# yifita/iso-points

Hardware: AMD Instinct MI355X
Metric: Mpoints/s full iso-point cycle (project+resample+splat), 1M pts (higher is better)
Workload: dtype f32-class (split-fp16 operands, 2^-22: hidden-layer products from two fp16 parts per f32 operand under exact power-of-two scales, 3 fp16-MFMA passes, f32 accumulate; everything else f32)

## Files before the change

### iso_points_amd/csrc/siren.hip

```cpp
#include <stdlib.h>
#include "siren_common.h"
#include "iso_newton.h"
#include "mlp_common.h"

namespace {

__global__ void k_siren_pack(const float* __restrict__ raw, float* __restrict__ packed,
                             int H, int L) {
  const int64_t total = off_hidden(H, L);
  const int64_t HH = (int64_t)H * H;
  const int NT = H / 16;
  for (int64_t o = (int64_t)blockIdx.x * blockDim.x + threadIdx.x; o < total;
       o += (int64_t)gridDim.x * blockDim.x) {
    float v = 0.f;
    if (o < off_wl(H)) {
      int64_t k = o;
      int c = (int)(k & 3);
      int e = (int)((k >> 2) % (H / 4));
      int g = (int)((k >> 2) / (H / 4));
      int f = 16 * (e >> 2) + 4 * g + (e & 3);
      v = (c < 3) ? raw[f * 3 + c] : raw[(int64_t)H * 3 + f];
    } else if (o < off_bl(H)) {
      int64_t k = o - off_wl(H);
      int e = (int)(k % (H / 4));
      int g = (int)(k / (H / 4));
      int f = 16 * (e >> 2) + 4 * g + (e & 3);
      const int64_t raw_wl = (int64_t)H * 4 + (int64_t)L * (HH + H);
      v = raw[raw_wl + f];
    } else if (o < off_hidden(H, 0)) {
      const int64_t raw_wl = (int64_t)H * 4 + (int64_t)L * (HH + H);
      v = (o == off_bl(H)) ? raw[raw_wl + H] : 0.f;
    } else {
      int64_t k = o - off_hidden(H, 0);
      const int64_t per = H + 2 * HH;
      int l = (int)(k / per);
      int64_t w = k % per;
      const float* Wl = raw + (int64_t)H * 4 + (int64_t)l * (HH + H);
      const float* bl = Wl + HH;
      if (w < H) {
        v = bl[w];
      } else {
        w -= H;
        bool bwd = w >= HH;
        if (bwd) w -= HH;
        int i = (int)(w & 3);
        int lane = (int)((w >> 2) & 63);
        int t = (int)((w >> 8) % NT);
        int q = (int)((w >> 8) / NT);
        int a = 16 * t + (lane & 15);
        int b = 16 * q + 4 * (lane >> 4) + i;
        v = bwd ? Wl[(int64_t)b * H + a]
                : Wl[(int64_t)a * H + b];
      }
    }
    packed[o] = v;
  }
}

#define ISO_GEMM_FWD(img, bias) gemm_pass<NT, true>(img, bias, hL, wbuf, acc, lane, g)
#define ISO_GEMM_BWD(img) gemm_pass<NT, false>(img, nullptr, hL, wbuf, acc, lane, g)

template <int NT, bool CODED>
__global__ __launch_bounds__(256, 2) void k_siren_step(typename SirenArgsOf<CODED>::type a) {
  constexpr int H = NT * 16;
  extern __shared__ __attribute__((aligned(16))) float smem[];
  const int tid = threadIdx.x;
  const int wave = tid >> 6, lane = tid & 63;
  const int g = lane >> 4, j = lane & 15;
  float* hL = smem + wave * (NT * 256);
  float* wbuf = smem + 4 * NT * 256;
  const float* W0img = a.packed + off_w0(H);
  const float* WLimg = a.packed + off_wl(H);
  const float bL = a.packed[off_bl(H)];
  float* stash = a.stash + ((int64_t)blockIdx.x * 4 + wave) * (int64_t)(a.L + 1) * NT * 256;

  const int64_t count = a.count_in ? (int64_t)(*a.count_in) : a.n;
  const int64_t n_tiles = (count + 63) / 64;
  for (int64_t tile = blockIdx.x; tile < n_tiles; tile += gridDim.x) {
    const int64_t slot = tile * 64 + wave * 16 + j;
    const bool valid = slot < count;
    int64_t idx = -1;
    float px = 0.f, py = 0.f, pz = 0.f;
    int row = 0;
    if (valid) {
      idx = a.idx_in ? (int64_t)a.idx_in[slot] : slot;
      px = a.pts[idx * 3]; py = a.pts[idx * 3 + 1]; pz = a.pts[idx * 3 + 2];
      if constexpr (CODED) row = a.code_of ? a.code_of[idx] : 0;
    }
    const f32x4* cb = nullptr;
    if constexpr (CODED) cb = reinterpret_cast<const f32x4*>(a.code_bias + (int64_t)row * H) + g;
    (void)cb;
    float f = 0.f;
    const bool top0 = (a.L == 0);
    for (int e4 = 0; e4 < NT; ++e4) {
      f32x4 h4, s4;
      f32x4 b4 = {0.f, 0.f, 0.f, 0.f};
      if constexpr (CODED) b4 = cb[4 * e4];
#pragma unroll
      for (int i = 0; i < 4; ++i) {
        const f32x4 w = reinterpret_cast<const f32x4*>(W0img)[g * (H / 4) + e4 * 4 + i];
        float z;
        if constexpr (CODED) z = ((w.x * px + w.y * py) + w.z * pz) + b4[i];
        else z = ((w.x * px + w.y * py) + w.z * pz) + w.w;
        float s, c;
        iso_sincos(a.w0 * z, s, c);
        h4[i] = s;
        s4[i] = a.w0 * c;
      }
      if (top0) {
        const f32x4 w4 = reinterpret_cast<const f32x4*>(WLimg)[g * NT + e4];
        f += (w4.x * h4.x + w4.y * h4.y) + (w4.z * h4.z + w4.w * h4.w);
        h4 = (f32x4){w4.x * s4.x, w4.y * s4.y, w4.z * s4.z, w4.w * s4.w};
      }
      reinterpret_cast<f32x4*>(hL)[e4 * 64 + lane] = h4;
      if (!top0) reinterpret_cast<f32x4*>(stash)[e4 * 64 + lane] = s4;
    }
    f32x4 acc[NT];
    for (int l = 0; l < a.L; ++l) {
      const float* base = a.packed + off_hidden(H, l);
      ISO_GEMM_FWD(base + H, base);
      float* st_l = stash + (int64_t)(l + 1) * NT * 256;
      const bool top = (l == a.L - 1);
#pragma unroll
      for (int t = 0; t < NT; ++t) reinterpret_cast<f32x4*>(hL)[t * 64 + lane] = acc[t];
      for (int e4 = 0; e4 < NT; ++e4) {
        const f32x4 z4 = reinterpret_cast<const f32x4*>(hL)[e4 * 64 + lane];
        f32x4 h4, s4;
#pragma unroll
        for (int i = 0; i < 4; ++i) {
          float s, c;
          iso_sincos(a.wh * z4[i], s, c);
          h4[i] = s;
          s4[i] = a.wh * c;
        }
        if (top) {
          const f32x4 w4 = reinterpret_cast<const f32x4*>(WLimg)[g * NT + e4];
          f += (w4.x * h4.x + w4.y * h4.y) + (w4.z * h4.z + w4.w * h4.w);
          h4 = (f32x4){w4.x * s4.x, w4.y * s4.y, w4.z * s4.z, w4.w * s4.w};
          reinterpret_cast<f32x4*>(hL)[e4 * 64 + lane] = h4;
        } else {
          reinterpret_cast<f32x4*>(hL)[e4 * 64 + lane] = h4;
          reinterpret_cast<f32x4*>(st_l)[e4 * 64 + lane] = s4;
        }
      }
    }
    f += __shfl_xor(f, 16);
    f += __shfl_xor(f, 32);
    f += bL;
    for (int l = a.L - 1; l >= 0; --l) {
      const float* base = a.packed + off_hidden(H, l);
      ISO_GEMM_BWD(base + H + (int64_t)H * H);
      const float* st_l = stash + (int64_t)l * NT * 256;
#pragma unroll
      for (int t = 0; t < NT; ++t) {
        const f32x4 s4 = reinterpret_cast<const f32x4*>(st_l)[t * 64 + lane];
        f32x4 gs = {acc[t].x * s4.x, acc[t].y * s4.y, acc[t].z * s4.z, acc[t].w * s4.w};
        reinterpret_cast<f32x4*>(hL)[t * 64 + lane] = gs;
      }
    }
    float gx = 0.f, gy = 0.f, gz = 0.f;
    for (int e4 = 0; e4 < NT; ++e4) {
      const f32x4 a4 = reinterpret_cast<const f32x4*>(hL)[e4 * 64 + lane];
#pragma unroll
      for (int i = 0; i < 4; ++i) {
        const f32x4 w = reinterpret_cast<const f32x4*>(W0img)[g * (H / 4) + e4 * 4 + i];
        gx += w.x * a4[i];
        gy += w.y * a4[i];
        gz += w.z * a4[i];
      }
    }
    gx += __shfl_xor(gx, 16); gx += __shfl_xor(gx, 32);
    gy += __shfl_xor(gy, 16); gy += __shfl_xor(gy, 32);
    gz += __shfl_xor(gz, 16); gz += __shfl_xor(gz, 32);

    bool survive = false;
    if (valid && g == 0) survive = iso_step_finish(a, idx, f, gx, gy, gz);
    if (!a.eval_only && a.do_move) {
      const unsigned long long bal = __ballot(survive);
      if (bal) {
        int base = 0;
        const int leader = __ffsll((long long)bal) - 1;
        if (lane == leader) base = atomicAdd(a.count_out, __popcll(bal));
        base = __shfl(base, leader);
        if (survive) {
          const int rank = __popcll(bal & ((1ull << lane) - 1ull));
          a.idx_out[base + rank] = (int32_t)idx;
        }
      }
    }
    __syncthreads();
  }
}

constexpr int kSirenBlocks = 512;

inline int64_t stash_floats(int H, int L) { return (int64_t)kSirenBlocks * 4 * (L + 1) * H * 16; }

template <int NT, bool CODED>
int launch_step(const typename SirenArgsOf<CODED>::type& a, int blocks, hipStream_t s) {
  const size_t lds = (size_t)(5 * NT * 256) * sizeof(float);
  static bool attr_done = false;
  if (!attr_done) {
    (void)hipFuncSetAttribute(reinterpret_cast<const void*>(&k_siren_step<NT, CODED>),
                        hipFuncAttributeMaxDynamicSharedMemorySize, (int)lds);
    attr_done = true;
  }
  hipLaunchKernelGGL((k_siren_step<NT, CODED>), dim3(blocks), dim3(256), lds, s, a);
  return 0;
}

template <bool CODED>
int dispatch_step(const typename SirenArgsOf<CODED>::type& a, int H, int blocks, hipStream_t s) {
  switch (H / 16) {
    case 4: return launch_step<4, CODED>(a, blocks, s);
    case 8: return launch_step<8, CODED>(a, blocks, s);
    case 16: return launch_step<16, CODED>(a, blocks, s);
    default: return -1;
  }
}

__global__ void k_zero_counts(int32_t* c, int n) {
  int i = blockIdx.x * blockDim.x + threadIdx.x;
  if (i < n) c[i] = 0;
}

bool siren_shape_ok(int H, int L) {
  return (H == 64 || H == 128 || H == 256) && L >= 0 && L <= 8;
}

int g_gemm_mode = -1;
int gemm_mode() {
  if (g_gemm_mode < 0) {
    const char* e = getenv("ISO_SIREN_GEMM");
    g_gemm_mode = (e && (!strcmp(e, "f32") || !strcmp(e, "0"))) ? 0 : 1;
  }
  return g_gemm_mode;
}
bool use_x3(int H, int L) { return gemm_mode() == 1 && siren_x3_supported(H, L); }

int64_t stash_floats_any(int H, int L) {
  int64_t a = stash_floats(H, L);
  int64_t b = siren_x3_supported(H, L) ? siren_x3_stash_floats(H, L) : 0;
  return a > b ? a : b;
}

int run_step(const SirenCodedArgs& a, int H, int64_t n, hipStream_t s) {
  if (use_x3(H, a.L)) return siren_x3_launch(a, H, n, s);
  int64_t tiles = (n + 63) / 64;
  int blocks = (int)(tiles < kSirenBlocks ? tiles : kSirenBlocks);
  return a.code_bias ? dispatch_step<true>(a, H, blocks, s) : dispatch_step<false>(a, H, blocks, s);
}

}

extern "C" int64_t iso_siren_raw_floats(int hidden, int n_hidden) {
  int64_t H = hidden;
  return H * 3 + H + (int64_t)n_hidden * (H * H + H) + H + 1;
}

extern "C" int64_t iso_siren_packed_floats(int hidden, int n_hidden) {
  return siren_packed_total(hidden, n_hidden);
}

extern "C" int iso_siren_set_gemm_mode(int mode) {
  ISO_REQUIRE(mode == 0 || mode == 1, ISO_ERR_INVALID, "iso_siren_set_gemm_mode: mode must be 0 (f32 MFMA) or 1 (split fp16)");
  g_gemm_mode = mode;
  return ISO_OK;
}

extern "C" int iso_siren_get_gemm_mode(void) { return gemm_mode(); }

extern "C" int iso_siren_pack_weights(const float* raw, float* packed, int hidden,
                                      int n_hidden, void* stream) {
  ISO_REQUIRE(siren_shape_ok(hidden, n_hidden), ISO_ERR_UNSUPPORTED,
              "iso_siren_pack_weights: hidden must be 64/128/256 and 0<=n_hidden<=8 (got %d, %d)",
              hidden, n_hidden);
  ISO_REQUIRE(raw && packed, ISO_ERR_INVALID, "iso_siren_pack_weights: null pointer");
  int64_t total = off_hidden(hidden, n_hidden);
  hipLaunchKernelGGL(k_siren_pack, dim3(iso_stream_grid(total, 256)), dim3(256), 0,
                     (hipStream_t)stream, raw, packed, hidden, n_hidden);
  if (hidden % 32 == 0) siren_x3_pack(raw, packed, hidden, n_hidden, (hipStream_t)stream);
  ISO_CHECK_LAUNCH("iso_siren_pack_weights");
  return ISO_OK;
}

static int64_t tail_cap_of(int64_t n) {
  const int64_t blocks = siren_x3_tail_blocks(), tiles = (n + 31) / 32;
  return ((tiles + blocks - 1) / blocks + 1) * 32;
}
static int64_t tail_ints(int64_t n) { return siren_x3_tail_blocks() * (2 * tail_cap_of(n) + 2); }

constexpr int kTileCtrInts = 128;
extern "C" int64_t iso_project_siren_workspace_bytes(int64_t n, int hidden, int n_hidden) {
  if (n < 0) n = 0;
  return stash_floats_any(hidden, n_hidden) * 4 + 2 * n * 4 + tail_ints(n) * 4 + (64 + kTileCtrInts) * 4 + 64;
}

extern "C" int64_t iso_project_siren_counts_offset(int64_t n, int hidden, int n_hidden) {
  if (n < 0) n = 0;
  return stash_floats_any(hidden, n_hidden) * 4 + 2 * n * 4 + tail_ints(n) * 4;
}

static int g_siren_dyn_tiles = -1;
static bool siren_dynamic_tiles_enabled() {
  return g_siren_dyn_tiles != 0;
}
extern "C" int iso_siren_set_drawn_tiles(int on) {
  ISO_REQUIRE(on >= -1 && on <= 1, ISO_ERR_INVALID, "iso_siren_set_drawn_tiles: -1 (default), 0 or 1");
  g_siren_dyn_tiles = on;
  return ISO_OK;
}

static int run_step_split(SirenCodedArgs a, int hidden, int64_t n, hipStream_t s) {
  if (hidden == 256 && !a.fwd_only && use_x3(hidden, a.L)) {
    a.split = 3;
    return run_step(a, hidden, n, s);
  }
  a.split = 0;
  a.tile_ctr = nullptr;
  return run_step(a, hidden, n, s);
}

static int g_tail_from = -1;
static int siren_tail_from(int max_iters) {
  if (g_tail_from == 0) return max_iters + 1;
  if (g_tail_from > 0) return g_tail_from;
  return max_iters >= 6 ? 4 : 2;
}
extern "C" int iso_siren_step_launches(int hidden, int n_hidden, int max_iters) {
  if (max_iters < 0) return 0;
  const bool can_tail = hidden == 256 && use_x3(hidden, n_hidden);
  const int from = can_tail ? siren_tail_from(max_iters) : max_iters + 1;
  return from <= max_iters && from > 0 ? from + 1 : max_iters + 1;
}
extern "C" int iso_siren_set_tail_from(int first_tail_iteration) {
  ISO_REQUIRE(first_tail_iteration >= -1, ISO_ERR_INVALID, "iso_siren_set_tail_from: -1 (default), 0 (never) or an iteration >= 1");
  g_tail_from = first_tail_iteration;
  return ISO_OK;
}

__global__ void k_zero_tail(int32_t* c, int n, int32_t* tc, int m) {
  const int i = blockIdx.x * blockDim.x + threadIdx.x;
  if (i < n) c[i] = 0;
  if (i < m) tc[i] = 0;
}

static int run_iterations(SirenCodedArgs a, int hidden, int64_t n, int max_iters, void* workspace,
                          hipStream_t s, const char* who) {
  float* stash = (float*)workspace;
  int32_t* idxA = (int32_t*)(stash + stash_floats_any(hidden, a.L));
  int32_t* idxB = idxA + n;
  int32_t* tail = idxB + n;
  int32_t* counts = tail + tail_ints(n);
  const int blocks = siren_x3_tail_blocks();
  const int64_t cap = tail_cap_of(n);
  int32_t* tail_counts = tail + (int64_t)blocks * 2 * cap;
  const bool can_tail = hidden == 256 && !a.dirs && !a.fwd_only && use_x3(hidden, a.L);
  const int tail_from = can_tail ? siren_tail_from(max_iters) : max_iters + 1;
  int32_t* tile_ctr = counts + 64;
  hipLaunchKernelGGL(k_zero_tail, dim3((2 * blocks + 255) / 256), dim3(256), 0, s, counts, 64 + kTileCtrInts, tail_counts,
                     tail_from <= max_iters ? 2 * blocks : 0);
  const bool dyn_tiles = siren_dynamic_tiles_enabled() && 2 * (max_iters + 1) <= kTileCtrInts;
  a.stash = stash; a.n = n; a.eval_only = 0; a.sdf_out = a.dirs ? a.sdf_out : nullptr; a.grad_out = nullptr;
  for (int it = 0; it <= max_iters; ++it) {
    a.idx_in = (it == 0) ? nullptr : ((it & 1) ? idxA : idxB);
    a.count_in = (it == 0) ? nullptr : counts + it;
    a.idx_out = (it & 1) ? idxB : idxA;
    a.count_out = counts + it + 1;
    a.do_move = (it < max_iters) ? 1 : 0;
    a.tile_ctr = dyn_tiles ? tile_ctr + 2 * it : nullptr;
    if (it >= tail_from && it > 0) {
      a.tail_lists = tail; a.tail_counts = tail_counts; a.iter_counts = counts; a.tail_cap = (int)cap;
      a.it_first = it; a.it_last = max_iters;
      ISO_REQUIRE(siren_x3_launch_tail(a, hidden, s) == 0, ISO_ERR_UNSUPPORTED, "%s: no tail kernel for hidden size %d", who, hidden);
      break;
    }
    ISO_REQUIRE(run_step_split(a, hidden, n, s) == 0, ISO_ERR_UNSUPPORTED, "%s: unsupported hidden size %d", who, hidden);
  }
  return ISO_OK;
}

__global__ void k_siren_fold_codes(const float* __restrict__ w0c, const float* __restrict__ b0,
                                   const float* __restrict__ codes, float* __restrict__ table, int H, int Hp, int C,
                                   int64_t U) {
  const int64_t total = U * Hp;
  for (int64_t o = (int64_t)blockIdx.x * blockDim.x + threadIdx.x; o < total; o += (int64_t)gridDim.x * blockDim.x) {
    const int64_t u = o / Hp;
    const int f = (int)(o - u * Hp);
    float v = 0.f;
    if (f < H) {
      double acc = (double)b0[f];
      const float* wr = w0c + (int64_t)f * C;
      const float* cu = codes + u * C;
      for (int k = 0; k < C; ++k) acc = fma((double)wr[k], (double)cu[k], acc);
      v = (float)acc;
    }
    table[o] = v;
  }
}

extern "C" int iso_siren_fold_codes(const float* w0c, const float* b0, const float* codes, float* table, int hidden,
                                    int padded_hidden, int c_dim, int64_t n_codes, void* stream) {
  ISO_REQUIRE(hidden >= 1 && padded_hidden >= hidden && c_dim >= 1 && n_codes >= 0, ISO_ERR_INVALID,
              "iso_siren_fold_codes: bad sizes (hidden %d, padded %d, c_dim %d, codes %lld)", hidden, padded_hidden,
              c_dim, (long long)n_codes);
  if (n_codes == 0) return ISO_OK;
  ISO_REQUIRE(w0c && b0 && codes && table, ISO_ERR_INVALID, "iso_siren_fold_codes: null pointer");
  const int64_t total = n_codes * padded_hidden;
  hipLaunchKernelGGL(k_siren_fold_codes, dim3(iso_stream_grid(total, 256)), dim3(256), 0, (hipStream_t)stream, w0c, b0,
                     codes, table, hidden, padded_hidden, c_dim, n_codes);
  ISO_CHECK_LAUNCH("iso_siren_fold_codes");
  return ISO_OK;
}

static int project_siren(const float* pts_in, float* pts_out, float* normals_out, uint8_t* mask_out, int64_t n,
                         const float* packed, int hidden, int n_hidden, float omega_first, float omega_hidden,
                         int max_iters, float tol, void* workspace, int64_t workspace_bytes, void* stream,
                         const float* code_bias, const int32_t* code_of) {
  ISO_REQUIRE(siren_shape_ok(hidden, n_hidden), ISO_ERR_UNSUPPORTED,
              "iso_project_siren: hidden must be 64/128/256 and 0<=n_hidden<=8 (got %d, %d)",
              hidden, n_hidden);
  ISO_REQUIRE(n >= 0 && max_iters >= 0 && max_iters <= 60, ISO_ERR_INVALID,
              "iso_project_siren: bad n / max_iters (max 60)");
  if (n == 0) return ISO_OK;
  ISO_REQUIRE(n < (1ll << 31), ISO_ERR_UNSUPPORTED, "iso_project_siren: n must fit int32");
  ISO_REQUIRE(pts_in && pts_out && normals_out && mask_out && packed && workspace,
              ISO_ERR_INVALID, "iso_project_siren: null pointer");
  ISO_REQUIRE(workspace_bytes >= iso_project_siren_workspace_bytes(n, hidden, n_hidden),
              ISO_ERR_WORKSPACE, "iso_project_siren: workspace too small");
  hipStream_t s = (hipStream_t)stream;
  if (pts_out != pts_in)
    (void)hipMemcpyAsync(pts_out, pts_in, (size_t)n * 12, hipMemcpyDeviceToDevice, s);
  SirenCodedArgs a;
  a.pts = pts_out; a.normals = normals_out; a.mask = mask_out;
  a.packed = packed; a.L = n_hidden;
  a.w0 = omega_first; a.wh = omega_hidden; a.tol = tol;
  a.code_bias = code_bias; a.code_of = code_of;
  int rc = run_iterations(a, hidden, n, max_iters, workspace, s, "iso_project_siren");
  if (rc != ISO_OK) return rc;
  ISO_CHECK_LAUNCH("iso_project_siren");
  return ISO_OK;
}

extern "C" int iso_project_siren(const float* pts_in, float* pts_out, float* normals_out,
                                 uint8_t* mask_out, int64_t n, const float* packed,
                                 int hidden, int n_hidden, float omega_first,
                                 float omega_hidden, int max_iters, float tol,
                                 void* workspace, int64_t workspace_bytes, void* stream) {
  return project_siren(pts_in, pts_out, normals_out, mask_out, n, packed, hidden, n_hidden, omega_first, omega_hidden,
                       max_iters, tol, workspace, workspace_bytes, stream, nullptr, nullptr);
}

extern "C" int iso_project_siren_coded(const float* pts_in, float* pts_out, float* normals_out,
                                       uint8_t* mask_out, int64_t n, const float* packed,
                                       int hidden, int n_hidden, float omega_first,
                                       float omega_hidden, int max_iters, float tol,
                                       void* workspace, int64_t workspace_bytes, void* stream,
                                       const float* code_bias, const int32_t* code_of, int64_t n_codes) {
  ISO_REQUIRE(code_bias && n_codes >= 1 && (code_of || n_codes == 1), ISO_ERR_INVALID,
              "iso_project_siren_coded: needs a bias table of n_codes >= 1 rows (and code_of when n_codes > 1)");
  return project_siren(pts_in, pts_out, normals_out, mask_out, n, packed, hidden, n_hidden, omega_first, omega_hidden,
                       max_iters, tol, workspace, workspace_bytes, stream, code_bias, code_of);
}

static int trace_siren(const float* ray0, const float* dirs, float* pts_out, float* sdf_out, uint8_t* mask_out,
                       int64_t n, const float* packed, int hidden, int n_hidden, float omega_first, float omega_hidden,
                       float alpha, float bound, int max_iters, float tol, void* workspace, int64_t workspace_bytes,
                       void* stream, const float* code_bias, const int32_t* code_of) {
  ISO_REQUIRE(siren_shape_ok(hidden, n_hidden), ISO_ERR_UNSUPPORTED,
              "iso_trace_siren: hidden must be 64/128/256 and 0<=n_hidden<=8 (got %d, %d)",
              hidden, n_hidden);
  ISO_REQUIRE(n >= 0 && max_iters >= 0 && max_iters <= 60, ISO_ERR_INVALID,
              "iso_trace_siren: bad n / max_iters (max 60)");
  if (n == 0) return ISO_OK;
  ISO_REQUIRE(n < (1ll << 31), ISO_ERR_UNSUPPORTED, "iso_trace_siren: n must fit int32");
  ISO_REQUIRE(ray0 && dirs && pts_out && sdf_out && mask_out && packed && workspace,
              ISO_ERR_INVALID, "iso_trace_siren: null pointer");
  ISO_REQUIRE(workspace_bytes >= iso_project_siren_workspace_bytes(n, hidden, n_hidden),
              ISO_ERR_WORKSPACE, "iso_trace_siren: workspace too small");
  hipStream_t s = (hipStream_t)stream;
  if (pts_out != ray0)
    (void)hipMemcpyAsync(pts_out, ray0, (size_t)n * 12, hipMemcpyDeviceToDevice, s);
  SirenCodedArgs a;
  a.pts = pts_out; a.normals = nullptr; a.mask = mask_out; a.sdf_out = sdf_out;
  a.packed = packed; a.L = n_hidden;
  a.w0 = omega_first; a.wh = omega_hidden;
  a.dirs = dirs; a.alpha = alpha; a.bound = bound;
  a.tol = 0.1f * tol;
  a.tol_valid = tol;
  a.fwd_only = 1;
  a.code_bias = code_bias; a.code_of = code_of;
  int rc = run_iterations(a, hidden, n, max_iters, workspace, s, "iso_trace_siren");
  if (rc != ISO_OK) return rc;
  ISO_CHECK_LAUNCH("iso_trace_siren");
  return ISO_OK;
}

extern "C" int iso_trace_siren(const float* ray0, const float* dirs, float* pts_out, float* sdf_out,
                               uint8_t* mask_out, int64_t n, const float* packed, int hidden,
                               int n_hidden, float omega_first, float omega_hidden, float alpha,
                               float bound, int max_iters, float tol, void* workspace,
                               int64_t workspace_bytes, void* stream) {
  return trace_siren(ray0, dirs, pts_out, sdf_out, mask_out, n, packed, hidden, n_hidden, omega_first, omega_hidden,
                     alpha, bound, max_iters, tol, workspace, workspace_bytes, stream, nullptr, nullptr);
}

extern "C" int iso_trace_siren_coded(const float* ray0, const float* dirs, float* pts_out, float* sdf_out,
                                     uint8_t* mask_out, int64_t n, const float* packed, int hidden,
                                     int n_hidden, float omega_first, float omega_hidden, float alpha,
                                     float bound, int max_iters, float tol, void* workspace,
                                     int64_t workspace_bytes, void* stream,
                                     const float* code_bias, const int32_t* code_of, int64_t n_codes) {
  ISO_REQUIRE(code_bias && n_codes >= 1 && (code_of || n_codes == 1), ISO_ERR_INVALID,
              "iso_trace_siren_coded: needs a bias table of n_codes >= 1 rows (and code_of when n_codes > 1)");
  return trace_siren(ray0, dirs, pts_out, sdf_out, mask_out, n, packed, hidden, n_hidden, omega_first, omega_hidden,
                     alpha, bound, max_iters, tol, workspace, workspace_bytes, stream, code_bias, code_of);
}

static int siren_sdf_grad(const float* pts, float* sdf_out, float* grad_out, int64_t n, const float* packed,
                          int hidden, int n_hidden, float omega_first, float omega_hidden, void* workspace,
                          int64_t workspace_bytes, void* stream, const float* code_bias, const int32_t* code_of) {
  ISO_REQUIRE(siren_shape_ok(hidden, n_hidden), ISO_ERR_UNSUPPORTED,
              "iso_siren_sdf_grad: hidden must be 64/128/256 and 0<=n_hidden<=8 (got %d, %d)",
              hidden, n_hidden);
  ISO_REQUIRE(n >= 0, ISO_ERR_INVALID, "iso_siren_sdf_grad: n < 0");
  ISO_REQUIRE(n < (1ll << 31), ISO_ERR_UNSUPPORTED, "iso_siren_sdf_grad: n must fit int32");
  if (n == 0) return ISO_OK;
  ISO_REQUIRE(pts && sdf_out && packed && workspace, ISO_ERR_INVALID,
              "iso_siren_sdf_grad: null pointer");
  ISO_REQUIRE(workspace_bytes >= stash_floats_any(hidden, n_hidden) * 4, ISO_ERR_WORKSPACE,
              "iso_siren_sdf_grad: workspace too small");
  SirenCodedArgs a;
  a.pts = const_cast<float*>(pts); a.normals = nullptr; a.mask = nullptr;
  a.sdf_out = sdf_out; a.grad_out = grad_out;
  a.idx_in = nullptr; a.count_in = nullptr; a.idx_out = nullptr; a.count_out = nullptr;
  a.packed = packed; a.stash = (float*)workspace; a.n = n; a.L = n_hidden;
  a.w0 = omega_first; a.wh = omega_hidden; a.tol = 0.f; a.do_move = 0; a.eval_only = 1;
  a.fwd_only = grad_out ? 0 : 1;
  a.code_bias = code_bias; a.code_of = code_of;
  if (hidden == 256 && !a.fwd_only && siren_dynamic_tiles_enabled() &&
      workspace_bytes >= iso_project_siren_workspace_bytes(n, hidden, n_hidden)) {
    int32_t* ctr = (int32_t*)((char*)workspace + iso_project_siren_counts_offset(n, hidden, n_hidden)) + 64;
    hipLaunchKernelGGL(k_zero_counts, dim3(1), dim3(64), 0, (hipStream_t)stream, ctr, 2);
    a.tile_ctr = ctr;
  }
  ISO_REQUIRE(run_step_split(a, hidden, n, (hipStream_t)stream) == 0, ISO_ERR_UNSUPPORTED,
              "iso_siren_sdf_grad: unsupported hidden size %d", hidden);
  ISO_CHECK_LAUNCH("iso_siren_sdf_grad");
  return ISO_OK;
}

extern "C" int iso_siren_sdf_grad(const float* pts, float* sdf_out, float* grad_out,
                                  int64_t n, const float* packed, int hidden,
                                  int n_hidden, float omega_first, float omega_hidden,
                                  void* workspace, int64_t workspace_bytes, void* stream) {
  return siren_sdf_grad(pts, sdf_out, grad_out, n, packed, hidden, n_hidden, omega_first, omega_hidden, workspace,
                        workspace_bytes, stream, nullptr, nullptr);
}

extern "C" int iso_siren_sdf_grad_coded(const float* pts, float* sdf_out, float* grad_out,
                                        int64_t n, const float* packed, int hidden,
                                        int n_hidden, float omega_first, float omega_hidden,
                                        void* workspace, int64_t workspace_bytes, void* stream,
                                        const float* code_bias, const int32_t* code_of, int64_t n_codes) {
  ISO_REQUIRE(code_bias && n_codes >= 1 && (code_of || n_codes == 1), ISO_ERR_INVALID,
              "iso_siren_sdf_grad_coded: needs a bias table of n_codes >= 1 rows (and code_of when n_codes > 1)");
  return siren_sdf_grad(pts, sdf_out, grad_out, n, packed, hidden, n_hidden, omega_first, omega_hidden, workspace,
                        workspace_bytes, stream, code_bias, code_of);
}
```

### iso_points_amd/csrc/siren_common.h

```cpp
#pragma once
#include "iso_common.h"

struct SirenArgs {
  float* pts;
  float* normals;
  uint8_t* mask;
  float* sdf_out;
  float* grad_out;
  const int32_t* idx_in;
  const int32_t* count_in;
  int32_t* idx_out;
  int32_t* count_out;
  const float* packed;
  float* stash;
  int64_t n;
  int L;
  float w0, wh, tol;
  int do_move;
  int eval_only;
  const float* dirs = nullptr;
  float alpha = 1.f, bound = 0.f, tol_valid = 0.f;
  int fwd_only = 0;
  int64_t cnt_lo = -1, cnt_hi = INT64_MAX;
  int small_tiles = 0;
  int split = 0;
  int big_blocks = 0;
  int32_t* tail_lists = nullptr;
  int32_t* tail_counts = nullptr;
  int32_t* iter_counts = nullptr;
  int tail_cap = 0, it_first = 0, it_last = 0;
  int32_t* tile_ctr = nullptr;
  int draw_first = 0;
  int ps_guard = 0;
};

struct SirenCodedArgs : SirenArgs {
  const float* code_bias = nullptr;
  const int32_t* code_of = nullptr;
};
template <bool CODED> struct SirenArgsOf { using type = SirenArgs; };
template <> struct SirenArgsOf<true> { using type = SirenCodedArgs; };

__host__ __device__ inline int64_t siren_split_point(int64_t count) {
  const int64_t big = 256 * 96, small = 256 * 32;
  const int64_t full = count / big * big, rem = count - full;
  if (rem == 0) return count;
  return (rem + small - 1) / small <= 2 ? full : count;
}

__host__ __device__ inline int64_t off_w0(int H) { (void)H; return 0; }
__host__ __device__ inline int64_t off_wl(int H) { return 4 * (int64_t)H; }
__host__ __device__ inline int64_t off_bl(int H) { return 5 * (int64_t)H; }
__host__ __device__ inline int64_t off_hidden(int H, int l) {
  return 5 * (int64_t)H + 4 + (int64_t)l * ((int64_t)H + 2 * (int64_t)H * H);
}

__host__ __device__ inline int x3_feat(int s, int kappa) {
  return 32 * (s >> 1) + 16 * (s & 1) + 8 * ((kappa & 7) >> 2) + 4 * (kappa >> 3) + (kappa & 3);
}
__host__ __device__ inline int64_t x3_base(int H, int L) { return off_hidden(H, L); }
__host__ __device__ inline int64_t x3_off_w0(int H, int L) { return x3_base(H, L); }
__host__ __device__ inline int64_t x3_off_wl(int H, int L) { return x3_base(H, L) + 4 * (int64_t)H; }
__host__ __device__ inline int64_t x3_off_layer(int H, int L, int l) {
  return x3_base(H, L) + 5 * (int64_t)H + (int64_t)l * (int64_t)H;
}
constexpr int kX16Header = 24;
__host__ __device__ inline int64_t x16_base(int H, int L) { return x3_off_layer(H, L, L); }
__host__ __device__ inline int64_t x16_off_layer(int H, int L, int l) { return x16_base(H, L) + kX16Header + (int64_t)l * H * H; }
__host__ __device__ inline int64_t x16_off_bw(int H, int L, int l) { return x16_off_layer(H, L, L) + (int64_t)l * H * H; }
__host__ __device__ inline int64_t siren_packed_total(int H, int L) { return x16_off_bw(H, L, L); }

bool siren_x3_supported(int H, int L);
int64_t siren_x3_stash_floats(int H, int L);
void siren_x3_pack(const float* raw, float* packed, int H, int L, hipStream_t s);
int siren_x3_launch(const SirenCodedArgs& a, int H, int64_t n_upper, hipStream_t s);
int siren_x3_tail_blocks();
int siren_x3_launch_tail(const SirenCodedArgs& a, int H, hipStream_t s);
constexpr int64_t kPsMinList = 3 * 256 * 128;
__host__ __device__ inline bool siren_ps_takes(int64_t count, int L, const float* hdr , float wh) {
  if (count < kPsMinList) return false;
  float r = 0.f;
  for (int l = 0; l < L; ++l) r = hdr[17 + l] > r ? hdr[17 + l] : r;
  return (wh * r) * 1.01f < 1.0e4f;
}
```

### iso_points_amd/csrc/siren_x3.hip

```cpp
#include <stdlib.h>
#include <type_traits>
#include "siren_common.h"
#include "iso_newton.h"
#include "mlp_common.h"

#include "mfma_split.h"

constexpr int kAD = 3;

namespace {

__device__ __forceinline__ void x3_sin_wcos8(float w_in, float w, const float (&z)[8], float (&s)[8], float (&c)[8]) {
  iso_sin_wcos8(w_in, w, z, s, c);
}


__global__ void k_siren_pack_x3(const float* __restrict__ raw, float* __restrict__ packed, int H, int L) {
  const int64_t base = x3_base(H, L), total = x16_base(H, L);
  const int64_t HH = (int64_t)H * H;
  const float* b0 = raw + (int64_t)H * 3;
  const float* WL = raw + (int64_t)H * 4 + (int64_t)L * (HH + H);
  for (int64_t o = base + (int64_t)blockIdx.x * blockDim.x + threadIdx.x; o < total;
       o += (int64_t)gridDim.x * blockDim.x) {
    const int64_t rel = o - base;
    auto feat_of = [](int64_t ko) { return x3_feat((int)(ko >> 4), 8 * (int)((ko >> 3) & 1) + (int)(ko & 7)); };
    if (rel < 4 * (int64_t)H) {
      const int f = feat_of(rel >> 2), c = (int)(rel & 3);
      packed[o] = (c < 3) ? raw[f * 3 + c] : b0[f];
    } else if (rel < 5 * (int64_t)H) {
      packed[o] = WL[feat_of(rel - 4 * (int64_t)H)];
    } else {
      const int64_t r2 = rel - 5 * (int64_t)H;
      const int l = (int)(r2 / H);
      const float* Wl = raw + (int64_t)H * 4 + (int64_t)l * (HH + H);
      packed[o] = Wl[HH + feat_of(r2 % H)];
    }
  }
}

__global__ void k_siren_wscale(const float* __restrict__ raw, float* __restrict__ packed, int H, int L) {
  __shared__ float s_m[256];
  const int l = blockIdx.x;
  const int64_t HH = (int64_t)H * H;
  const float* Wl = raw + (int64_t)H * 4 + (int64_t)l * (HH + H);
  float m = 0.f, cs = 0.f;
  for (int f = threadIdx.x; f < H; f += 256) {
    float t = 0.f;
#pragma unroll 32
    for (int k = 0; k < H; ++k) {
      const float a = fabsf(Wl[(int64_t)k * H + f]);
      m = (a == a && a > m) ? a : m;
      t += a;
    }
    cs = fmaxf(cs, t);
  }
  s_m[threadIdx.x] = m;
  __syncthreads();
  for (int o = 128; o > 0; o >>= 1) {
    if ((int)threadIdx.x < o) s_m[threadIdx.x] = fmaxf(s_m[threadIdx.x], s_m[threadIdx.x + o]);
    __syncthreads();
  }
  if (threadIdx.x == 0) {
    float mx = s_m[0];
    int e = 0;
    float sc = 1.0f;
    if (mx > 0.f && mx < 3.0e38f) {
      (void)frexpf(mx, &e);
      int k = 10 - e;
      k = k > 100 ? 100 : (k < -100 ? -100 : k);
      sc = ldexpf(1.0f, k);
    }
    packed[x16_base(H, L) + l] = sc;
  }
  __syncthreads();
  s_m[threadIdx.x] = cs;
  __syncthreads();
  for (int o = 128; o > 0; o >>= 1) {
    if ((int)threadIdx.x < o) s_m[threadIdx.x] = fmaxf(s_m[threadIdx.x], s_m[threadIdx.x + o]);
    __syncthreads();
  }
  if (threadIdx.x == 0) packed[x16_base(H, L) + 8 + l] = s_m[0];
  if (l == 0) {
    __syncthreads();
    const float* WLh = raw + (int64_t)H * 4 + (int64_t)L * (HH + H);
    float mh = 0.f;
    for (int f = threadIdx.x; f < H; f += 256) mh = fmaxf(mh, fabsf(WLh[f]));
    s_m[threadIdx.x] = mh;
    __syncthreads();
    for (int o = 128; o > 0; o >>= 1) {
      if ((int)threadIdx.x < o) s_m[threadIdx.x] = fmaxf(s_m[threadIdx.x], s_m[threadIdx.x + o]);
      __syncthreads();
    }
    if (threadIdx.x == 0) packed[x16_base(H, L) + 16] = s_m[0];
  }
}

__global__ void k_siren_pack_f16(const float* __restrict__ raw, float* __restrict__ packed, int H, int L) {
  const int64_t HH = (int64_t)H * H;
  const int NTO = H / 32;
  const int64_t total = 2 * (int64_t)L * HH;
  for (int64_t o = (int64_t)blockIdx.x * blockDim.x + threadIdx.x; o < total; o += (int64_t)gridDim.x * blockDim.x) {
    const bool bwd = o >= (int64_t)L * HH;
    const int l = (int)((o / HH) % L);
    const int64_t q = o % HH;
    const float* Wl = raw + (int64_t)H * 4 + (int64_t)l * (HH + H);
    const float sc = packed[x16_base(H, L) + l];
    const int d = (int)(q & 3), lane = (int)((q >> 2) & 63);
    const int64_t blk = q >> 8;
    const int part = (int)(blk & 1);
    const int To = (int)((blk >> 1) % NTO), s = (int)(blk / (2 * NTO));
    const int fo = 32 * To + (lane & 31);
    f32x2 v;
#pragma unroll
    for (int u = 0; u < 2; ++u) {
      const int fi = x3_feat(s, 8 * (lane >> 5) + 2 * d + u);
      v[u] = (bwd ? Wl[(int64_t)fi * H + fo] : Wl[(int64_t)fo * H + fi]) * sc;
    }
    const f16x2 h = __builtin_convertvector(v, f16x2);
    const f16x2 lo = __builtin_convertvector(v - __builtin_convertvector(h, f32x2), f16x2);
    reinterpret_cast<unsigned*>(packed + x16_off_layer(H, L, 0))[o] =
        part == 0 ? __builtin_bit_cast(unsigned, h) : __builtin_bit_cast(unsigned, lo);
  }
}

template <int H, int NW, int NB>
struct X3Shape {
  static constexpr int NS = H / 16;
  static constexpr int NTO = H / 32;
  static constexpr int TW = NTO / NW;
  static constexpr int SL = 2 * TW;
  static constexpr int NG = SL * NB;
  static constexpr int P = 32 * NB;
  static constexpr size_t kActBytes = (size_t)NS * NB * kAP * 1024;
  static constexpr size_t kRedBytes = (size_t)NW * P * 16;
  static constexpr size_t kPtsBytes = (size_t)P * 16;
  static constexpr int kLdsGroupsFit = (int)((163840 - (kActBytes + kRedBytes + kPtsBytes)) / ((size_t)NW * 2048));
  static constexpr int LG = kLdsGroupsFit < NG ? kLdsGroupsFit : NG;
  static constexpr size_t kLds = kActBytes + kRedBytes + kPtsBytes + (size_t)NW * LG * 2048;
  static constexpr int64_t kStashPerWg(int L) { return (int64_t)NW * (L > 1 ? L : 1) * NG * 512; }
  static_assert(NTO % NW == 0 && TW >= 1, "features must split evenly over the waves");
};

template <int H>
__device__ __forceinline__ void x3_code_bias8(const float* table, int row, int s, int h, float (&b)[8]) {
  const f32x4* t = reinterpret_cast<const f32x4*>(table + (int64_t)row * H + 16 * s + 4 * h);
  const f32x4 lo = t[0], hi = t[2];
#pragma unroll
  for (int e = 0; e < 4; ++e) { b[e] = lo[e]; b[4 + e] = hi[e]; }
}

template <int H, int NW, int NB, bool FWD, bool CODED>
__device__ __forceinline__ void x3_step_body(const typename SirenArgsOf<CODED>::type& a, const int bid, const int nblk,
                                             const int sid) {
  using S = X3Shape<H, NW, NB>;
  constexpr int NS = S::NS, NTO = S::NTO, TW = S::TW, SL = S::SL, NG = S::NG, P = S::P;
  extern __shared__ __attribute__((aligned(16))) unsigned char smem_raw[];
  u32x4* act = reinterpret_cast<u32x4*>(smem_raw);
  f32x4* red = reinterpret_cast<f32x4*>(smem_raw + S::kActBytes);
  f32x4* ptl = reinterpret_cast<f32x4*>(smem_raw + S::kActBytes + S::kRedBytes);
  constexpr int LG = S::LG;
  const int tid = threadIdx.x;
  const int w = __builtin_amdgcn_readfirstlane(tid >> 6);
  const int lane = tid & 63, h = lane >> 5, j = lane & 31;
  u32x4* own = act + (size_t)(SL * w) * NB * kAP * 64 + lane;
  u32x4* park = own + (size_t)(kAP - 2) * NG * 64;
  constexpr bool IL = (NW == 8);
  const int L = a.L;
  const float* X = a.packed + x3_base(H, L);
  const f32x4* W0u = reinterpret_cast<const f32x4*>(X) + SL * w * 16;
  const float* WLu = X + 4 * H + SL * w * 16;
  const int h8 = h * 8;
  const float bL = a.packed[off_bl(H)];
  f32x4* stash = reinterpret_cast<f32x4*>(a.stash) +
                 ((int64_t)sid * NW + w) * (int64_t)(L > 1 ? L : 1) * NG * 128;
  f32x4* lst = reinterpret_cast<f32x4*>(smem_raw + S::kActBytes + S::kRedBytes + S::kPtsBytes) + w * (LG * 128) + lane;

  constexpr int FP = 2, BP = 2;
  auto fwd_img = [&](int l) { return reinterpret_cast<const u32x4*>(a.packed + x16_off_layer(H, L, l)) + (TW * w * 2) * 64; };
  auto rev_img = [&](int l) { return reinterpret_cast<const u32x4*>(a.packed + x16_off_bw(H, L, l)) + (TW * w * 2) * 64; };
  auto fwd_scale = [&](int l) { return kActScale * a.packed[x16_base(H, L) + l]; };
  float* redm = reinterpret_cast<float*>(red);
  float bscale[NB];
  float amax[NB];
  auto put_amax = [&](int buf) {
#pragma unroll
    for (int n = 0; n < NB; ++n) {
      const float m = __builtin_fmaxf(amax[n], __shfl_xor(amax[n], 32));
      if (h == 0) redm[(buf * P + 32 * n + j) * NW + w] = m;
    }
  };
  u32x4 A[4][TW][3];
  x3_prefetch_a<kAD, TW, NTO, FP>(A, fwd_img(0), 0, lane);

  const int64_t total = a.count_in ? (int64_t)__hip_atomic_load(a.count_in, __ATOMIC_RELAXED, __HIP_MEMORY_SCOPE_AGENT) : a.n;
  if (total <= a.cnt_lo || total > a.cnt_hi) return;
  if (a.ps_guard && H == 256 && siren_ps_takes(total, L, a.packed + x16_base(H, L), a.wh)) return;
  const int64_t cut = a.split ? siren_split_point(total) : total;
  const int64_t slot0 = a.split == 2 ? cut : 0;
  const int64_t count = a.split == 1 ? cut : total;
  const int64_t n_tiles = (count - slot0 + P - 1) / P;
  __shared__ int s_next_tile, s_first_tile;
  int nidx[NB];
  float npx[NB], npy[NB], npz[NB];
  int nrow[NB];
  auto fetch_idx = [&](int64_t t) {
    int j_e = j;
    asm volatile("" : "+v"(j_e));
#pragma unroll
    for (int n = 0; n < NB; ++n) {
      const int64_t slot = slot0 + t * P + 32 * n + j_e;
      nidx[n] = -1;
      if (t < n_tiles && slot < count) nidx[n] = a.idx_in ? a.idx_in[slot] : (int)slot;
    }
  };
  auto fetch_pts = [&]() {
#pragma unroll
    for (int n = 0; n < NB; ++n) {
      npx[n] = npy[n] = npz[n] = 0.f;
      if constexpr (CODED) nrow[n] = 0;
      if (nidx[n] >= 0) {
        const int64_t idx = nidx[n];
        npx[n] = a.pts[idx * 3]; npy[n] = a.pts[idx * 3 + 1]; npz[n] = a.pts[idx * 3 + 2];
        if constexpr (CODED) nrow[n] = a.code_of ? a.code_of[idx] : 0;
      }
    }
  };
  int64_t first_tile = bid;
  if (!FWD && a.tile_ctr != nullptr && a.draw_first) {
    if (tid == 0) s_first_tile = atomicAdd(a.tile_ctr, 1);
    __syncthreads();
    first_tile = s_first_tile;
  }
  fetch_idx(first_tile);
  fetch_pts();
  const bool dyn = !FWD && a.tile_ctr != nullptr;
  const int draw_base = a.draw_first ? 0 : nblk;
  int64_t next_tile = 0;
  for (int64_t tile = first_tile; tile < n_tiles; tile = next_tile) {
    float px[NB], py[NB], pz[NB];
    int row[NB];
    int j_e = j;
    asm volatile("" : "+v"(j_e));
#pragma unroll
    for (int n = 0; n < NB; ++n) {
      px[n] = npx[n]; py[n] = npy[n]; pz[n] = npz[n];
      if constexpr (CODED) row[n] = nrow[n];
      if constexpr (!FWD) {
        if constexpr (CODED) {
          if (w == 0 && h == 0) ptl[32 * n + j_e] = (f32x4){px[n], py[n], pz[n], __int_as_float(row[n])};
        } else {
          if (w == 0 && h == 0) ptl[32 * n + j_e] = (f32x4){px[n], py[n], pz[n], 0.f};
        }
      }
    }
    for (int sl = 0; sl < SL; ++sl) {
      f32x4 wv[8];
#pragma unroll
      for (int e = 0; e < 8; ++e) wv[e] = W0u[sl * 16 + h8 + e];
#pragma unroll
      for (int n = 0; n < NB; ++n) {
        float zz[8], hv[8], sv[8];
        if constexpr (CODED) {
          float bz[8];
          x3_code_bias8<H>(a.code_bias, row[n], SL * w + sl, h, bz);
#pragma unroll
          for (int e = 0; e < 8; ++e) zz[e] = ((wv[e].x * px[n] + wv[e].y * py[n]) + wv[e].z * pz[n]) + bz[e];
        } else {
#pragma unroll
          for (int e = 0; e < 8; ++e) zz[e] = ((wv[e].x * px[n] + wv[e].y * py[n]) + wv[e].z * pz[n]) + wv[e].w;
        }
        x3_sin_wcos8(a.w0, a.w0, zz, hv, sv);
        const int k = sl * NB + n;
        {
          u32x4 p0, p1;
          split8_f16(hv, p0, p1);
          own[(k * kAP + 0) * 64] = p0; own[(k * kAP + 1) * 64] = p1;
        }
        (void)sv;
      }
    }
    __syncthreads();

    f32x16 acc[TW][NB];
    float fpart[NB];
#pragma unroll
    for (int n = 0; n < NB; ++n) fpart[n] = 0.f;
    for (int l = 0; l < L; ++l) {
      const float* lay = a.packed + x3_off_layer(H, L, l);
      const u32x4* img = fwd_img(l);
      const float zscale = fwd_scale(l);
      const float w_in = a.wh / zscale;
      if (l + 1 < L || FWD) {
        gemm_x3<kAD, TW, NB, NTO, NS, kBias, IL, FP, FP>(img, lay, act + lane, acc, w, 0, A,
                                                         l + 1 < L ? fwd_img(l + 1) : fwd_img(0), 0, lane, zscale);
      } else {
        gemm_x3<kAD, TW, NB, NTO, NS, kBias, IL, FP, BP>(img, lay, act + lane, acc, w, 0, A, rev_img(L - 1), 0, lane,
                                                         zscale);
      }
      __syncthreads();
      const bool top = (l == L - 1);
      f32x4* st_l = stash + (int64_t)l * NG * 128;
      const bool lds_slot = (l == 0);
      const float seed_scale = x3_scale_for(a.packed[x16_base(H, L) + 16] * a.wh * 1.01f);
      if (top) {
#pragma unroll
        for (int n = 0; n < NB; ++n) { amax[n] = 0.f; bscale[n] = seed_scale; }
      }
      auto act_group = [&](int k, int n, int sl, const float (&zz)[8], float& fp) {
        float hv[8], sv[8];
        x3_sin_wcos8(w_in, a.wh, zz, hv, sv);
        if (top) {
          const f32x4 wl0 = *reinterpret_cast<const f32x4*>(WLu + sl * 16 + h8);
          const f32x4 wl1 = *reinterpret_cast<const f32x4*>(WLu + sl * 16 + h8 + 4);
          const float f0 = (wl0.x * hv[0] + wl0.y * hv[1]) + (wl0.z * hv[2] + wl0.w * hv[3]);
          const float f1 = (wl1.x * hv[4] + wl1.y * hv[5]) + (wl1.z * hv[6] + wl1.w * hv[7]);
          fp += f0 + f1;
          if constexpr (FWD) return;
#pragma unroll
          for (int e = 0; e < 4; ++e) { hv[e] = wl0[e] * sv[e]; hv[4 + e] = wl1[e] * sv[4 + e]; }
          float m = amax[n];
#pragma unroll
          for (int e = 0; e < 8; e += 2) m = __builtin_fmaxf(m, __builtin_fmaxf(__builtin_fabsf(hv[e]), __builtin_fabsf(hv[e + 1])));
          amax[n] = m;
          u32x4 p0, p1;
          split8_f16(hv, p0, p1, seed_scale);
          own[(k * kAP + 0) * 64] = p0; own[(k * kAP + 1) * 64] = p1;
          return;
        } else {
          if constexpr (!FWD) {
            if (k < LG && lds_slot) {
              lst[(k * 2 + 0) * 64] = (f32x4){sv[0], sv[1], sv[2], sv[3]};
              lst[(k * 2 + 1) * 64] = (f32x4){sv[4], sv[5], sv[6], sv[7]};
            } else {
              st_l[(k * 2 + 0) * 64 + lane] = (f32x4){sv[0], sv[1], sv[2], sv[3]};
              st_l[(k * 2 + 1) * 64 + lane] = (f32x4){sv[4], sv[5], sv[6], sv[7]};
            }
          }
        }
        u32x4 p0, p1;
        split8_f16(hv, p0, p1);
        own[(k * kAP + 0) * 64] = p0; own[(k * kAP + 1) * 64] = p1;
      };
      if constexpr (NG <= 8) {
#pragma unroll
        for (int t = 0; t < TW; ++t)
#pragma unroll
          for (int p = 0; p < 2; ++p)
#pragma unroll
            for (int n = 0; n < NB; ++n) {
              float zz[8];
#pragma unroll
              for (int e = 0; e < 8; ++e) zz[e] = acc[t][n][8 * p + e];
              act_group((2 * t + p) * NB + n, n, 2 * t + p, zz, fpart[n]);
              __builtin_amdgcn_sched_barrier(0);
            }
      } else {
#pragma unroll
        for (int t = 0; t < TW; ++t)
#pragma unroll
          for (int n = 0; n < NB; ++n)
#pragma unroll
            for (int p = 0; p < 2; ++p) {
              const int k = (2 * t + p) * NB + n;
              const f32x16& v = acc[t][n];
              park[(k * 2 + 0) * 64] = as_u32x4((f32x4){v[8 * p], v[8 * p + 1], v[8 * p + 2], v[8 * p + 3]});
              park[(k * 2 + 1) * 64] = as_u32x4((f32x4){v[8 * p + 4], v[8 * p + 5], v[8 * p + 6], v[8 * p + 7]});
            }
        for (int sl = 0; sl < SL; ++sl) {
          f32x4 z[NB][2];
#pragma unroll
          for (int n = 0; n < NB; ++n) {
            z[n][0] = as_f32x4(park[((sl * NB + n) * 2 + 0) * 64]);
            z[n][1] = as_f32x4(park[((sl * NB + n) * 2 + 1) * 64]);
          }
#pragma unroll
          for (int n = 0; n < NB; ++n) {
            float zz[8];
#pragma unroll
            for (int e = 0; e < 8; ++e) zz[e] = z[n][e >> 2][e & 3];
            act_group(sl * NB + n, n, sl, zz, fpart[n]);
          }
        }
      }
      if constexpr (!FWD) { if (top) put_amax(0); }
      __syncthreads();
    }
    float gx[NB], gy[NB], gz[NB];
#pragma unroll
    for (int n = 0; n < NB; ++n) gx[n] = gy[n] = gz[n] = 0.f;
    int mbuf = 0;
    auto get_amax = [&](float (&Mp)[NB]) {
#pragma unroll
      for (int n = 0; n < NB; ++n) {
        float m = 0.f;
#pragma unroll
        for (int ww = 0; ww < NW; ++ww) m = __builtin_fmaxf(m, redm[(mbuf * P + 32 * n + j) * NW + ww]);
        Mp[n] = m;
      }
    };
    for (int l = FWD ? 0 : L - 1; l >= 1; --l) {
      const u32x4* img = rev_img(l);
      const f32x4* st_l = stash + (int64_t)(l - 1) * NG * 128;
      f32x4 sv[NG][2];
      auto ld_stash = [&]() {
#pragma unroll
        for (int k = 0; k < NG; ++k) {
          if (k < LG && l == 1) {
            sv[k][0] = lst[(k * 2) * 64]; sv[k][1] = lst[(k * 2 + 1) * 64];
          } else {
            sv[k][0] = st_l[(k * 2) * 64 + lane]; sv[k][1] = st_l[(k * 2 + 1) * 64 + lane];
          }
        }
      };
      float Mp[NB];
      get_amax(Mp);
      gemm_x3<kAD, TW, NB, NTO, NS, kZero, IL, BP, BP>(img, nullptr, act + lane, acc, w, 0, A, rev_img(l - 1), 0, lane);
      ld_stash();
      __syncthreads();
      float inv[NB], nscale[NB];
      {
        const float iw = 1.0f / a.packed[x16_base(H, L) + l];
        const float grow = a.packed[x16_base(H, L) + 8 + l] * a.wh * 1.01f;
#pragma unroll
        for (int n = 0; n < NB; ++n) {
          inv[n] = iw / bscale[n];
          nscale[n] = x3_scale_for(Mp[n] * grow);
          amax[n] = 0.f;
        }
      }
#pragma unroll
      for (int t = 0; t < TW; ++t)
#pragma unroll
        for (int p = 0; p < 2; ++p) {
#pragma unroll
          for (int n = 0; n < NB; ++n) {
            const int k = (2 * t + p) * NB + n;
            float av[8];
#pragma unroll
            for (int e = 0; e < 8; ++e) av[e] = (acc[t][n][8 * p + e] * inv[n]) * sv[k][e >> 2][e & 3];
            float m = amax[n];
#pragma unroll
            for (int e = 0; e < 8; e += 2) m = __builtin_fmaxf(m, __builtin_fmaxf(__builtin_fabsf(av[e]), __builtin_fabsf(av[e + 1])));
            amax[n] = m;
            u32x4 p0, p1;
            split8_f16(av, p0, p1, nscale[n]);
            own[(k * kAP + 0) * 64] = p0; own[(k * kAP + 1) * 64] = p1;
          }
        }
#pragma unroll
      for (int n = 0; n < NB; ++n) bscale[n] = nscale[n];
      put_amax(mbuf ^ 1);
      mbuf ^= 1;
      __syncthreads();
    }
    if constexpr (!FWD) {
      int drawn = 0;
      if (dyn && tid == 0) drawn = draw_base + atomicAdd(a.tile_ctr, 1);
      gemm_x3<kAD, TW, NB, NTO, NS, kZero, IL, BP, FP>(rev_img(0), nullptr, act + lane, acc, w, 0, A, fwd_img(0), 0, lane);
      if (dyn && tid == 0) s_next_tile = drawn;
      __syncthreads();
      next_tile = dyn ? (int64_t)s_next_tile : tile + nblk;
      fetch_idx(next_tile);
      float inv[NB];
      {
        const float iw = 1.0f / a.packed[x16_base(H, L)];
#pragma unroll
        for (int n = 0; n < NB; ++n) inv[n] = iw / bscale[n];
      }
      f32x4 q[NB];
#pragma unroll
      for (int n = 0; n < NB; ++n) q[n] = ptl[32 * n + j];
#pragma unroll
      for (int t = 0; t < TW; ++t)
#pragma unroll
        for (int p = 0; p < 2; ++p) {
          f32x4 wv[8];
#pragma unroll
          for (int e = 0; e < 8; ++e) wv[e] = W0u[(2 * t + p) * 16 + h8 + e];
#pragma unroll
          for (int n = 0; n < NB; ++n) {
            float zz[8], cv[8];
            if constexpr (CODED) {
              float bz[8];
              x3_code_bias8<H>(a.code_bias, __float_as_int(q[n].w), SL * w + 2 * t + p, h, bz);
#pragma unroll
              for (int e = 0; e < 8; ++e) zz[e] = ((wv[e].x * q[n].x + wv[e].y * q[n].y) + wv[e].z * q[n].z) + bz[e];
            } else {
#pragma unroll
              for (int e = 0; e < 8; ++e) zz[e] = ((wv[e].x * q[n].x + wv[e].y * q[n].y) + wv[e].z * q[n].z) + wv[e].w;
            }
            iso_wcos8(a.w0, a.w0, zz, cv);
#pragma unroll
            for (int e = 0; e < 8; ++e) {
              const float av = (acc[t][n][8 * p + e] * inv[n]) * cv[e];
              gx[n] += wv[e].x * av;
              gy[n] += wv[e].y * av;
              gz[n] += wv[e].z * av;
            }
            __builtin_amdgcn_sched_barrier(0);
          }
        }
    } else {
      next_tile = tile + nblk;
      fetch_idx(next_tile);
    }
#pragma unroll
    for (int n = 0; n < NB; ++n) {
      float f = fpart[n] + __shfl_xor(fpart[n], 32);
      float x = gx[n] + __shfl_xor(gx[n], 32);
      float y = gy[n] + __shfl_xor(gy[n], 32);
      float z = gz[n] + __shfl_xor(gz[n], 32);
      if (h == 0) red[w * P + 32 * n + j] = (f32x4){f, x, y, z};
    }
    int tid_e = tid, lane_e = lane;
    asm volatile("" : "+v"(tid_e), "+v"(lane_e));
    int eidx = -1;
    f32x4 qe = {0.f, 0.f, 0.f, 0.f};
    {
      const int64_t slot = slot0 + tile * P + tid_e;
      if (tid_e < P && slot < count) {
        eidx = a.idx_in ? a.idx_in[slot] : (int)slot;
        if constexpr (!FWD) qe = ptl[tid_e];
      }
      fetch_pts();
    }
    __syncthreads();
    bool survive = false;
    int64_t idx = -1;
    {
      const int64_t slot = slot0 + tile * P + tid_e;
      if (tid_e < P && slot < count) {
        f32x4 r = red[tid_e];
#pragma unroll
        for (int ww = 1; ww < NW; ++ww) {
          const f32x4 q = red[ww * P + tid_e];
          r.x += q.x; r.y += q.y; r.z += q.z; r.w += q.w;
        }
        const float f = r.x + bL;
        idx = eidx;
        if constexpr (!FWD) survive = iso_step_finish<SirenArgs, true>(a, idx, f, r.y, r.z, r.w, qe.x, qe.y, qe.z);
        else survive = iso_step_finish(a, idx, f, r.y, r.z, r.w);
      }
    }
    if (!a.eval_only && a.do_move) {
      const unsigned long long bal = __ballot(survive);
      if (bal) {
        int base = 0;
        const int leader = __ffsll((long long)bal) - 1;
        if (lane_e == leader) base = atomicAdd(a.count_out, __popcll(bal));
        base = __shfl(base, leader);
        if (survive) {
          const int rank = __popcll(bal & ((1ull << lane_e) - 1ull));
          a.idx_out[base + rank] = (int32_t)idx;
        }
      }
    }
  }
}

template <int H, int NW, int NB, int MINB, bool FWD, bool CODED>
__global__ __launch_bounds__(64 * NW, MINB) void k_siren_step_x3(typename SirenArgsOf<CODED>::type a) {
  x3_step_body<H, NW, NB, FWD, CODED>(a, (int)blockIdx.x, (int)gridDim.x, (int)blockIdx.x);
}

template <int H, int NW, int NB, int MINB, bool CODED>
__global__ __launch_bounds__(64 * NW, MINB) void k_siren_step_x3_both(typename SirenArgsOf<CODED>::type a) {
  const bool big = (int)blockIdx.x < a.big_blocks;
  const int small_blocks = (int)gridDim.x - a.big_blocks;
  if (big) {
    typename SirenArgsOf<CODED>::type b = a;
    b.split = 1;
    x3_step_body<H, NW, NB, false, CODED>(b, (int)blockIdx.x, a.big_blocks, (int)blockIdx.x);
  }
  if (!big || a.tile_ctr != nullptr) {
    if (big) __syncthreads();
    typename SirenArgsOf<CODED>::type b = a;
    b.split = 2;
    if (a.tile_ctr) b.tile_ctr = a.tile_ctr + 1;
    const bool joint = a.tile_ctr != nullptr;
    b.draw_first = joint ? 1 : 0;
    const int bid = big ? small_blocks + (int)blockIdx.x : (int)blockIdx.x - a.big_blocks;
    const int nblk = joint ? small_blocks + a.big_blocks : small_blocks;
    if (big) b.stash = a.stash + (int64_t)blockIdx.x * X3Shape<H, NW, NB>::kStashPerWg(a.L);
    else b.stash = a.stash + (int64_t)a.big_blocks * X3Shape<H, NW, NB>::kStashPerWg(a.L);
    x3_step_body<H, NW, 1, false, CODED>(b, bid, nblk, big ? 0 : bid);
  }
}

template <int H, int NW, int MINB, bool CODED>
__global__ __launch_bounds__(64 * NW, MINB) void k_siren_tail_x3(typename SirenArgsOf<CODED>::type a) {
  const int b = blockIdx.x, nblk = gridDim.x;
  int32_t* lists = a.tail_lists + (int64_t)b * 2 * a.tail_cap;
  int32_t* cnts = a.tail_counts + b * 2;
  typename SirenArgsOf<CODED>::type r = a;
  r.split = 0; r.small_tiles = 1; r.cnt_lo = -1; r.cnt_hi = INT64_MAX; r.tile_ctr = nullptr;
  r.idx_out = lists; r.count_out = cnts;
  r.do_move = a.it_first < a.it_last ? 1 : 0;
  x3_step_body<H, NW, 1, false, CODED>(r, b, nblk, b);
  int cur = 0;
  for (int it = a.it_first + 1; it <= a.it_last; ++it) {
    __syncthreads();
    const int m = __hip_atomic_load(&cnts[cur], __ATOMIC_RELAXED, __HIP_MEMORY_SCOPE_AGENT);
    if (m == 0) break;
    if (threadIdx.x == 0) {
      __hip_atomic_store(&cnts[cur ^ 1], 0, __ATOMIC_RELAXED, __HIP_MEMORY_SCOPE_AGENT);
      if (a.iter_counts) atomicAdd(&a.iter_counts[it], m);
    }
    __syncthreads();
    r.idx_in = lists + (int64_t)cur * a.tail_cap; r.count_in = cnts + cur;
    r.idx_out = lists + (int64_t)(cur ^ 1) * a.tail_cap; r.count_out = cnts + (cur ^ 1);
    r.do_move = it < a.it_last ? 1 : 0;
    x3_step_body<H, NW, 1, false, CODED>(r, 0, 1, b);
    cur ^= 1;
  }
  __syncthreads();
  if (threadIdx.x == 0) { cnts[0] = 0; cnts[1] = 0; }
}

template <int H, int NW, int NB, int MINB, bool FWD, bool CODED>
int launch_x3(const typename SirenArgsOf<CODED>::type& a, int64_t n_upper, hipStream_t s) {
  using S = X3Shape<H, NW, NB>;
  static bool attr_done = false;
  if (!attr_done) {
    (void)hipFuncSetAttribute(reinterpret_cast<const void*>(&k_siren_step_x3<H, NW, NB, MINB, FWD, CODED>),
                              hipFuncAttributeMaxDynamicSharedMemorySize, (int)S::kLds);
    attr_done = true;
  }
  const int64_t tiles = (n_upper + S::P - 1) / S::P;
  const int64_t cap = 256 * MINB;
  const int blocks = (int)(tiles < cap ? (tiles < 1 ? 1 : tiles) : cap);
  hipLaunchKernelGGL((k_siren_step_x3<H, NW, NB, MINB, FWD, CODED>), dim3(blocks), dim3(64 * NW), S::kLds, s, a);
  return 0;
}

template <int H, int NW, int NB, int MINB, bool CODED>
int launch_x3_both(typename SirenArgsOf<CODED>::type a, int64_t n_upper, hipStream_t s) {
  using SB = X3Shape<H, NW, NB>;
  using SS = X3Shape<H, NW, 1>;
  constexpr size_t lds = SB::kLds > SS::kLds ? SB::kLds : SS::kLds;
  static bool attr_done = false;
  if (!attr_done) {
    (void)hipFuncSetAttribute(reinterpret_cast<const void*>(&k_siren_step_x3_both<H, NW, NB, MINB, CODED>),
                              hipFuncAttributeMaxDynamicSharedMemorySize, (int)lds);
    attr_done = true;
  }
  const int64_t cap = 256 * MINB;
  const int64_t tb = (n_upper + SB::P - 1) / SB::P, ts = (n_upper + SS::P - 1) / SS::P;
  a.big_blocks = (int)(tb < cap ? (tb < 1 ? 1 : tb) : cap);
  const int small_blocks = (int)(ts < cap ? (ts < 1 ? 1 : ts) : cap);
  hipLaunchKernelGGL((k_siren_step_x3_both<H, NW, NB, MINB, CODED>), dim3(a.big_blocks + small_blocks), dim3(64 * NW), lds, s, a);
  return 0;
}

}

constexpr int kNW256 = 8;
constexpr int kMinB256 = 1;
constexpr int kNB256 = 3;
constexpr int kMinB128 = 1;
bool siren_x3_supported(int H, int L) { return (H == 256 || H == 128) && L >= 1 && L <= 8; }

int64_t siren_x3_stash_floats(int H, int L) {
  if (H == 256) {
    return 256 * kMinB256 * (X3Shape<256, kNW256, kNB256>::kStashPerWg(L) + X3Shape<256, kNW256, 1>::kStashPerWg(L));
  }
  if (H == 128) return 256 * kMinB128 * X3Shape<128, 4, 3>::kStashPerWg(L);
  return 0;
}

void siren_x3_pack(const float* raw, float* packed, int H, int L, hipStream_t s) {
  const int64_t words = x16_base(H, L) - x3_base(H, L);
  hipLaunchKernelGGL(k_siren_pack_x3, dim3(iso_stream_grid(words, 256)), dim3(256), 0, s, raw, packed, H, L);
  if (L > 0) {
    hipLaunchKernelGGL(k_siren_wscale, dim3(L), dim3(256), 0, s, raw, packed, H, L);
    hipLaunchKernelGGL(k_siren_pack_f16, dim3(iso_stream_grid(2 * (int64_t)L * H * H, 256)), dim3(256), 0, s, raw, packed, H, L);
  }
}

int siren_x3_tail_blocks() { return 256 * kMinB256; }

template <bool CODED>
static int launch_tail(const typename SirenArgsOf<CODED>::type& a, hipStream_t s) {
  using SS = X3Shape<256, kNW256, 1>;
  static bool attr_done = false;
  if (!attr_done) {
    (void)hipFuncSetAttribute(reinterpret_cast<const void*>(&k_siren_tail_x3<256, kNW256, kMinB256, CODED>),
                              hipFuncAttributeMaxDynamicSharedMemorySize, (int)SS::kLds);
    attr_done = true;
  }
  hipLaunchKernelGGL((k_siren_tail_x3<256, kNW256, kMinB256, CODED>), dim3(siren_x3_tail_blocks()), dim3(64 * kNW256), SS::kLds, s, a);
  return 0;
}

int siren_x3_launch_tail(const SirenCodedArgs& a, int H, hipStream_t s) {
  if (H != 256) return -1;
  return a.code_bias ? launch_tail<true>(a, s) : launch_tail<false>(a, s);
}

template <bool CODED>
static int launch_any(const typename SirenArgsOf<CODED>::type& a, int H, int64_t n_upper, hipStream_t s) {
  if (a.split == 3 && H == 256 && !a.fwd_only) return launch_x3_both<256, kNW256, kNB256, kMinB256, CODED>(a, n_upper, s);
  if (a.fwd_only) {
    if (H == 256) return launch_x3<256, kNW256, kNB256, kMinB256, true, CODED>(a, n_upper, s);
    if (H == 128) return launch_x3<128, 4, 3, kMinB128, true, CODED>(a, n_upper, s);
  }
  if constexpr (!CODED) {
    if (H == 256) return launch_x3<256, kNW256, kNB256, kMinB256, false, false>(a, n_upper, s);
  }
  if (H == 128) return launch_x3<128, 4, 3, kMinB128, false, CODED>(a, n_upper, s);
  return -1;
}

int siren_x3_launch(const SirenCodedArgs& a, int H, int64_t n_upper, hipStream_t s) {
  return a.code_bias ? launch_any<true>(a, H, n_upper, s) : launch_any<false>(a, H, n_upper, s);
}
```

### iso_points_amd/csrc/splat.hip

```cpp
#include <float.h>
#include "iso_common.h"
#include "splat_frame.h"
#include "pca_eig.h"

#pragma clang fp contract(off)

struct ZScale;
struct ZRider {
  const float* gz; int64_t n;
  ZScale* zs; int blocks;
  const long long* acc; float* grad; int terms_log2;
};
__device__ void z_absmax_body(const float* __restrict__ gz, int64_t n, ZScale* __restrict__ zs, int block, int nblocks);
__device__ void z_finish_body(const long long* __restrict__ acc, const ZScale* __restrict__ zs, const int64_t* __restrict__ first,
                              const int64_t* __restrict__ num, int n_clouds, float* __restrict__ grad, int terms_log2,
                              int block, int nblocks);

namespace {

__device__ __forceinline__ float esqrt_arg(float x) {
  float a = fabsf(x);
  return a < 1e-17f ? 1e-17f : a;
}

__global__ void k_view_flags(const float* __restrict__ pts, const float* __restrict__ nrm,
                             const float* __restrict__ views, int32_t* __restrict__ flags,
                             int64_t P, float znear, float zfar, int backface) {
  const int n = blockIdx.y;
  const float* V = views + n * 16;
  for (int64_t i = (int64_t)blockIdx.x * blockDim.x + threadIdx.x; i < P;
       i += (int64_t)gridDim.x * blockDim.x) {
    float x = pts[i * 3], y = pts[i * 3 + 1], z = pts[i * 3 + 2];
    float zv = ((x * V[2] + y * V[6]) + z * V[10]) + V[14];
    bool ok = (zv >= znear) && (zv <= zfar);
    if (backface) {
      float nx = nrm[i * 3], ny = nrm[i * 3 + 1], nz = nrm[i * 3 + 2];
      float nzv = (nx * V[2] + ny * V[6]) + nz * V[10];
      ok = ok && (nzv < 0.f);
    }
    flags[(int64_t)n * P + i] = ok ? 1 : 0;
  }
}

__global__ void k_compact_rows(const float* __restrict__ in, const int32_t* __restrict__ flags,
                               const int32_t* __restrict__ off, float* __restrict__ out,
                               int64_t P, int64_t total, int U) {
  for (int64_t e = (int64_t)blockIdx.x * blockDim.x + threadIdx.x; e < total;
       e += (int64_t)gridDim.x * blockDim.x) {
    if (flags[e]) {
      const float* s = in + (e % P) * U;
      float* d = out + (int64_t)off[e] * U;
      for (int u = 0; u < U; ++u) d[u] = s[u];
    }
  }
}

__global__ void k_vrk_h(const float* __restrict__ dists ,
                        const int64_t* __restrict__ first, const int64_t* __restrict__ num,
                        const int64_t* __restrict__ cloud_num, float* __restrict__ h, int64_t pmax) {
  const int n = blockIdx.y;
  const int64_t len = num[n];
  const int64_t clen = cloud_num ? cloud_num[n] : len;
  for (int64_t i = (int64_t)blockIdx.x * blockDim.x + threadIdx.x; i < len;
       i += (int64_t)gridDim.x * blockDim.x) {
    const float* d = dists + ((int64_t)n * pmax + i) * 7;
    float m = -FLT_MAX;
#pragma unroll
    for (int k = 1; k < 7; ++k) {
      float v = (clen < 7) ? 1e-3f : d[k];
      m = fmaxf(m, v);
    }
    float hv = 0.5f * m;
    hv = fminf(fmaxf(hv, 5e-5f), 0.01f);
    h[first[n] + i] = hv;
  }
}

struct SetupOut {
  float* ndc;
  float* ellipse;
  float* cutoff;
  float* radii;
  float* scaler;
};

struct SetupRes { float ndc[3], el[3], rad[2], scaler; };

__device__ __forceinline__ SetupRes splat_setup_point(float x, float y, float z, float nx, float ny, float nz,
                                                      float hk, const float* __restrict__ V,
                                                      const float* __restrict__ M, int S, float sigma,
                                                      float cutoffC) {
  const float xv = ((x * M[0] + y * M[4]) + z * M[8]) + M[12];
  const float yv = ((x * M[1] + y * M[5]) + z * M[9]) + M[13];
  const float t = ((x * M[3] + y * M[7]) + z * M[11]) + M[15];
  const float zv = ((x * V[2] + y * V[6]) + z * V[10]) + V[14];
  const float t2 = iso_eps_denom(t * t, 1e-17f);
  const float td = iso_eps_denom(t, 1e-17f);
  const float j00 = 1.0f / td;
  const float j30 = -1.0f / t2 * xv, j31 = -1.0f / t2 * yv;
  float w0[3], w1[3];
#pragma unroll
  for (int r = 0; r < 3; ++r) {
    w0[r] = M[r * 4 + 0] * j00 + M[r * 4 + 3] * j30;
    w1[r] = M[r * 4 + 1] * j00 + M[r * 4 + 3] * j31;
  }
  float ex = 0.f, ey = 0.f, ez = 0.f;
  const float ax = fabsf(nx), ay = fabsf(ny), az = fabsf(nz);
  if (ax <= ay && ax <= az) ex = 1.f; else if (ay <= az) ey = 1.f; else ez = 1.f;
  const float mx = nx + ex, my = ny + ey, mz = nz + ez;
  float ux = ny * mz - nz * my, uy = nz * mx - nx * mz, uz = nx * my - ny * mx;
  float un = sqrtf((ux * ux + uy * uy) + uz * uz);
  un = un > 1e-12f ? un : 1e-12f;
  ux /= un; uy /= un; uz /= un;
  float vx = ny * uz - nz * uy, vy = nz * ux - nx * uz, vz = nx * uy - ny * ux;
  float vn = sqrtf((vx * vx + vy * vy) + vz * vz);
  vn = vn > 1e-12f ? vn : 1e-12f;
  vx /= vn; vy /= vn; vz /= vn;
  const float m00 = (ux * w0[0] + uy * w0[1]) + uz * w0[2];
  const float m01 = (ux * w1[0] + uy * w1[1]) + uz * w1[2];
  const float m10 = (vx * w0[0] + vy * w0[1]) + vz * w0[2];
  const float m11 = (vx * w1[0] + vy * w1[1]) + vz * w1[2];
  const float ps = 2.0f / (float)S;
  const float lp = sigma * (ps * ps);
  const float g00 = hk * (m00 * m00 + m10 * m10) + lp;
  const float g01 = hk * (m00 * m01 + m10 * m11);
  const float g11 = hk * (m01 * m01 + m11 * m11) + lp;
  const float detM = m00 * m11 - m01 * m10;
  const float fro = (m00 * m00 + m10 * m10) + (m01 * m01 + m11 * m11);
  const float detG = (hk * hk) * (detM * detM) + (lp * hk * fro + lp * lp);
  const float a = g11 / detG, c = g00 / detG, b = (-g01 / detG) + (-g01 / detG);
  const float den = iso_eps_denom(4.0f * a * c - b * b, 1e-17f);
  SetupRes o;
  o.rad[1] = sqrtf(esqrt_arg(4.0f * a * cutoffC / den));
  o.rad[0] = sqrtf(esqrt_arg(4.0f * c * cutoffC / den));
  o.scaler = fabsf(detM) / iso_eps_denom(sqrtf(esqrt_arg(detG * 4.0f * 3.14159265358979323846f * 3.14159265358979323846f)), 1e-17f);
  o.ndc[0] = xv / t; o.ndc[1] = yv / t; o.ndc[2] = zv;
  o.el[0] = a; o.el[1] = b; o.el[2] = c;
  return o;
}

__device__ __forceinline__ void splat_tangent_frame(float nx, float ny, float nz, float& ux, float& uy, float& uz,
                                                    float& vx, float& vy, float& vz) {
  float ex = 0.f, ey = 0.f, ez = 0.f;
  const float ax = fabsf(nx), ay = fabsf(ny), az = fabsf(nz);
  if (ax <= ay && ax <= az) ex = 1.f; else if (ay <= az) ey = 1.f; else ez = 1.f;
  const float mx = nx + ex, my = ny + ey, mz = nz + ez;
  ux = ny * mz - nz * my;
  uy = nz * mx - nx * mz;
  uz = nx * my - ny * mx;
  float un = sqrtf((ux * ux + uy * uy) + uz * uz);
  un = un > 1e-12f ? un : 1e-12f;
  ux /= un; uy /= un; uz /= un;
  vx = ny * uz - nz * uy;
  vy = nz * ux - nx * uz;
  vz = nx * uy - ny * ux;
  float vn = sqrtf((vx * vx + vy * vy) + vz * vz);
  vn = vn > 1e-12f ? vn : 1e-12f;
  vx /= vn; vy /= vn; vz /= vn;
}

__global__ void k_tangent_frame(const float* __restrict__ nrm, int64_t n, float* __restrict__ u, float* __restrict__ v) {
  for (int64_t i = (int64_t)blockIdx.x * blockDim.x + threadIdx.x; i < n; i += (int64_t)gridDim.x * blockDim.x) {
    float ux, uy, uz, vx, vy, vz;
    splat_tangent_frame(nrm[i * 3], nrm[i * 3 + 1], nrm[i * 3 + 2], ux, uy, uz, vx, vy, vz);
    u[i * 3] = ux; u[i * 3 + 1] = uy; u[i * 3 + 2] = uz;
    v[i * 3] = vx; v[i * 3 + 1] = vy; v[i * 3 + 2] = vz;
  }
}

struct SetupProj { float xv, yv, t, zv, w0[3], w1[3]; };

__device__ __forceinline__ SetupProj splat_setup_project(float x, float y, float z, const float* __restrict__ V,
                                                         const float* __restrict__ M) {
  SetupProj pj;
  pj.xv = ((x * M[0] + y * M[4]) + z * M[8]) + M[12];
  pj.yv = ((x * M[1] + y * M[5]) + z * M[9]) + M[13];
  pj.t = ((x * M[3] + y * M[7]) + z * M[11]) + M[15];
  pj.zv = ((x * V[2] + y * V[6]) + z * V[10]) + V[14];
  const float t2 = iso_eps_denom(pj.t * pj.t, 1e-17f);
  const float td = iso_eps_denom(pj.t, 1e-17f);
  const float j00 = 1.0f / td;
  const float j30 = -1.0f / t2 * pj.xv, j31 = -1.0f / t2 * pj.yv;
#pragma unroll
  for (int r = 0; r < 3; ++r) {
    pj.w0[r] = M[r * 4 + 0] * j00 + M[r * 4 + 3] * j30;
    pj.w1[r] = M[r * 4 + 1] * j00 + M[r * 4 + 3] * j31;
  }
  return pj;
}

__device__ __forceinline__ SetupRes splat_setup_frame(const SetupProj& pj, float ux, float uy, float uz, float vx, float vy,
                                                      float vz, float c1, float c2, int S, float sigma, float cutoffC) {
  const float* w0 = pj.w0;
  const float* w1 = pj.w1;
  const float m00 = (ux * w0[0] + uy * w0[1]) + uz * w0[2];
  const float m01 = (ux * w1[0] + uy * w1[1]) + uz * w1[2];
  const float m10 = (vx * w0[0] + vy * w0[1]) + vz * w0[2];
  const float m11 = (vx * w1[0] + vy * w1[1]) + vz * w1[2];
  const float ps = 2.0f / (float)S;
  const float lp = sigma * (ps * ps);
  const float hk = c1;
  float g00 = hk * (m00 * m00 + m10 * m10) + lp;
  float g01 = hk * (m00 * m01 + m10 * m11);
  float g11 = hk * (m01 * m01 + m11 * m11) + lp;
  const float detM = m00 * m11 - m01 * m10;
  const float fro = (m00 * m00 + m10 * m10) + (m01 * m01 + m11 * m11);
  float detG = (hk * hk) * (detM * detM) + (lp * hk * fro + lp * lp);
  {
    const bool same = c1 == c2;
    const float a00 = (c1 * (m00 * m00) + c2 * (m10 * m10)) + lp;
    const float a01 = c1 * (m00 * m01) + c2 * (m10 * m11);
    const float a11 = (c1 * (m01 * m01) + c2 * (m11 * m11)) + lp;
    const float adet = (c1 * c2) * (detM * detM) +
                       (lp * (c1 * (m00 * m00 + m01 * m01) + c2 * (m10 * m10 + m11 * m11)) + lp * lp);
    g00 = same ? g00 : a00;
    g01 = same ? g01 : a01;
    g11 = same ? g11 : a11;
    detG = same ? detG : adet;
  }
  const float a = g11 / detG, c = g00 / detG, b = (-g01 / detG) + (-g01 / detG);
  const float den = iso_eps_denom(4.0f * a * c - b * b, 1e-17f);
  SetupRes o;
  o.rad[1] = sqrtf(esqrt_arg(4.0f * a * cutoffC / den));
  o.rad[0] = sqrtf(esqrt_arg(4.0f * c * cutoffC / den));
  o.scaler = fabsf(detM) / iso_eps_denom(sqrtf(esqrt_arg(detG * 4.0f * 3.14159265358979323846f * 3.14159265358979323846f)), 1e-17f);
  o.ndc[0] = pj.xv / pj.t; o.ndc[1] = pj.yv / pj.t; o.ndc[2] = pj.zv;
  o.el[0] = a; o.el[1] = b; o.el[2] = c;
  return o;
}

__global__ void k_splat_setup(const float* __restrict__ pts, const float* __restrict__ nrm,
                              const float* __restrict__ h, const int64_t* __restrict__ first,
                              const int64_t* __restrict__ num, const float* __restrict__ views,
                              const float* __restrict__ projs, int S, float sigma, float cutoffC,
                              SetupOut o) {
  const int n = blockIdx.y;
  const float* V = views + n * 16;
  const float* M = projs + n * 16;
  const int64_t len = num[n], base = first[n];
  for (int64_t i = (int64_t)blockIdx.x * blockDim.x + threadIdx.x; i < len;
       i += (int64_t)gridDim.x * blockDim.x) {
    const int64_t p = base + i;
    const SetupRes r = splat_setup_point(pts[p * 3], pts[p * 3 + 1], pts[p * 3 + 2], nrm[p * 3], nrm[p * 3 + 1],
                                         nrm[p * 3 + 2], h[p], V, M, S, sigma, cutoffC);
    o.ndc[p * 3] = r.ndc[0]; o.ndc[p * 3 + 1] = r.ndc[1]; o.ndc[p * 3 + 2] = r.ndc[2];
    o.ellipse[p * 3] = r.el[0]; o.ellipse[p * 3 + 1] = r.el[1]; o.ellipse[p * 3 + 2] = r.el[2];
    o.cutoff[p] = cutoffC;
    o.radii[p * 2] = r.rad[0]; o.radii[p * 2 + 1] = r.rad[1];
    o.scaler[p] = r.scaler;
  }
}

__global__ void k_splat_setup_vrk(const float* __restrict__ pts, const float* __restrict__ frames,
                                  const float* __restrict__ curv, const int64_t* __restrict__ first,
                                  const int64_t* __restrict__ num, const float* __restrict__ views,
                                  const float* __restrict__ projs, int S, float sigma, float cutoffC, SetupOut o) {
  const int n = blockIdx.y;
  const float* V = views + n * 16;
  const float* M = projs + n * 16;
  const int64_t len = num[n], base = first[n];
  for (int64_t i = (int64_t)blockIdx.x * blockDim.x + threadIdx.x; i < len;
       i += (int64_t)gridDim.x * blockDim.x) {
    const int64_t p = base + i;
    const float* f = frames + p * 9;
    const SetupProj pj = splat_setup_project(pts[p * 3], pts[p * 3 + 1], pts[p * 3 + 2], V, M);
    const SetupRes r = splat_setup_frame(pj, f[1], f[4], f[7], f[2], f[5], f[8], curv[p * 3 + 1], curv[p * 3 + 2], S, sigma,
                                         cutoffC);
    o.ndc[p * 3] = r.ndc[0]; o.ndc[p * 3 + 1] = r.ndc[1]; o.ndc[p * 3 + 2] = r.ndc[2];
    o.ellipse[p * 3] = r.el[0]; o.ellipse[p * 3 + 1] = r.el[1]; o.ellipse[p * 3 + 2] = r.el[2];
    o.cutoff[p] = cutoffC;
    o.radii[p * 2] = r.rad[0]; o.radii[p * 2 + 1] = r.rad[1];
    o.scaler[p] = r.scaler;
  }
}

constexpr int kVrkK = 8;
__global__ void __launch_bounds__(256) k_splat_setup_aniso(const float* __restrict__ pts, const int64_t* __restrict__ idx,
                                                           int64_t p_stride, const int64_t* __restrict__ first,
                                                           const int64_t* __restrict__ num,
                                                           const float* __restrict__ views,
                                                           const float* __restrict__ projs, int S, float sigma,
                                                           float cutoffC, SetupOut o) {
  const int n = blockIdx.y;
  const float* V = views + n * 16;
  const float* M = projs + n * 16;
  const int64_t base = first[n];
  const int64_t len = min(num[n], p_stride);
  const float* cloud = pts + base * 3;
  for (int64_t i = (int64_t)blockIdx.x * blockDim.x + threadIdx.x; i < len;
       i += (int64_t)gridDim.x * blockDim.x) {
    const int64_t p = base + i;
    float l[3], v[3][3];
    pca_neighbourhood_eig(cloud, idx + ((int64_t)n * p_stride + i) * kVrkK, kVrkK, len, l, v);
    const SetupProj pj = splat_setup_project(pts[p * 3], pts[p * 3 + 1], pts[p * 3 + 2], V, M);
    const SetupRes r = splat_setup_frame(pj, v[0][1], v[1][1], v[2][1], v[0][2], v[1][2], v[2][2], l[1], l[2], S, sigma,
                                         cutoffC);
    o.ndc[p * 3] = r.ndc[0]; o.ndc[p * 3 + 1] = r.ndc[1]; o.ndc[p * 3 + 2] = r.ndc[2];
    o.ellipse[p * 3] = r.el[0]; o.ellipse[p * 3 + 1] = r.el[1]; o.ellipse[p * 3 + 2] = r.el[2];
    o.cutoff[p] = cutoffC;
    o.radii[p * 2] = r.rad[0]; o.radii[p * 2 + 1] = r.rad[1];
    o.scaler[p] = r.scaler;
  }
}

constexpr int kHSlices = 64;
constexpr int kHBlock = 256;
__global__ void __launch_bounds__(kHBlock) k_vrk_h_partial(const float* __restrict__ dists ,
                                                           const int64_t* __restrict__ num, int64_t p_stride, int64_t pmax,
                                                           double* __restrict__ part) {
  __shared__ double s_sum[kHBlock];
  const int n = blockIdx.y, s = blockIdx.x;
  const int64_t clen = num[n];
  const int64_t len = min(max(clen, (int64_t)0), p_stride);
  const int64_t chunk = (pmax + kHSlices - 1) / kHSlices;
  const int64_t lo = s * chunk, hi = min(lo + chunk, pmax);
  double acc = 0.0;
  for (int64_t i = lo + threadIdx.x; i < hi; i += kHBlock) {
    float m = -1.0f;
    if (clen < 7) {
// ... 923 lines not shown
    cc[k] = i < tiles ? count_of(tile_of(i)) : 0;
  }
  auto visit = [&](auto&& f) {
#pragma unroll
    for (int k = 0; k < 4; ++k) {
      const int i = threadIdx.x + k * (int)blockDim.x;
      if (i < tiles) f(i, tile_of(i), cc[k]);
    }
    for (int i = threadIdx.x + 4 * (int)blockDim.x; i < tiles; i += blockDim.x) f(i, tile_of(i), count_of(tile_of(i)));
  };
  if (threadIdx.x == 0) s_slots = 0;
  __syncthreads();
  {
    int mine = 0;
    visit([&](int, int, int c) { mine += c; });
    mine = wave_sum_i(mine);
    if ((threadIdx.x & 63) == 0 && mine) atomicAdd(&s_slots, mine);
  }
  __syncthreads();
  if (threadIdx.x == 0) {
    int sl0 = (s_slots / target_items + 255) / 256 * 256;
    s_slice = sl0 < 256 ? 256 : (sl0 > kSlice ? kSlice : sl0);
  }
  __syncthreads();
  for (int round = 0; round < 16; ++round) {
    if (threadIdx.x == 0) s_slots = 0;
    __syncthreads();
    const int sl = s_slice;
    int mine = 0;
    visit([&](int, int, int c) { if (2 * c > 3 * sl) mine += (c + sl - 1) / sl; });
    mine = wave_sum_i(mine);
    if ((threadIdx.x & 63) == 0 && mine) atomicAdd(&s_slots, mine);
    __syncthreads();
    const bool fits = s_slots <= max_slots;
    __syncthreads();
    if (fits) break;
    if (threadIdx.x == 0) s_slice = sl * 2;
    __syncthreads();
  }
  const int sl = s_slice;
  auto slices_of = [&](int c) { return (2 * c > 3 * sl && max_slots > 0) ? (c + sl - 1) / sl : 1; };
  if (threadIdx.x < 64) hist[threadIdx.x] = 0;
  if (threadIdx.x == 0) { s_slots = 0; s_heavy = 0; }
  __syncthreads();
  auto bucket_of = [&](int c) { return min(c >> 6, 63); };
  visit([&](int, int tile, int c) {
    const int ns = slices_of(c);
    if (ns > 1) {
      const int b0 = atomicAdd(&s_slots, ns);
      heavy[atomicAdd(&s_heavy, 1)] = make_int4(tile, b0, ns, 0);
      for (int k = 0; k < ns; ++k) items[b0 + k] = make_int4(tile, k, ns, b0 + k);
    } else {
      atomicAdd(&hist[bucket_of(c)], 1);
    }
  });
  __syncthreads();
  if (threadIdx.x == 0) {
    int run = s_slots;
    for (int b = 63; b >= 0; --b) { base[b] = run; run += hist[b]; }
    counters[0] = run;
    counters[1] = s_heavy;
  }
  __syncthreads();
  visit([&](int, int tile, int c) {
    if (slices_of(c) == 1) items[atomicAdd(&base[bucket_of(c)], 1)] = make_int4(tile, 0, 1, 0);
  });
}
__global__ __launch_bounds__(1024) void k_tile_items(const int32_t* __restrict__ tile_off, Frame F, int ty_begin,
                                                     int ty_rows, int n_clouds, int max_slots, int target_items,
                                                     int4* __restrict__ items, int4* __restrict__ heavy,
                                                     int32_t* __restrict__ counters) {
  tile_items_body(tile_off, F, ty_begin, ty_rows, n_clouds, max_slots, target_items, items, heavy, counters);
}

template <int KMAX, bool KFULL = false>
__global__ __launch_bounds__(256) void k_raster_merge(const int4* __restrict__ heavy, const int32_t* __restrict__ counters,
                                                      const float* __restrict__ scratch, Frame F, int K_arg,
                                                      float depth_thres, int32_t* __restrict__ idx_out,
                                                      float* __restrict__ zbuf_out, float* __restrict__ q_out,
                                                      float* __restrict__ occ_out, CompositeArgs ca) {
  const int K = KFULL ? KMAX : K_arg;
  const int nh = counters[1];
  for (int hI = blockIdx.x; hI < nh; hI += gridDim.x) {
    const int4 hv = heavy[hI];
    const int tile = hv.x;
    const int tx = tile % F.Tx, ty = (tile / F.Tx) % F.Ty, n = tile / (F.Tx * F.Ty);
    const int lx = threadIdx.x % TILE, ly = threadIdx.x / TILE;
    const int xi = tx * TILE + lx, yi = ty * TILE + ly;
    PixK<KMAX> best;
    best.init();
    for (int sI = 0; sI < hv.z; ++sI) {
      const float* sc = scratch + (int64_t)(hv.y + sI) * 3 * KMAX * 256;
      float zz[KMAX], qq[KMAX];
      int ii[KMAX];
#pragma unroll
      for (int j = 0; j < KMAX; ++j) {
        zz[j] = sc[j * 256 + threadIdx.x];
        qq[j] = sc[(KMAX + j) * 256 + threadIdx.x];
        ii[j] = __float_as_int(sc[(2 * KMAX + j) * 256 + threadIdx.x]);
      }
      if (sI == 0) {
#pragma unroll
        for (int j = 0; j < KMAX; ++j) { best.z[j] = zz[j]; best.q[j] = qq[j]; best.id[j] = ii[j]; }
      } else {
#pragma unroll
        for (int j = 0; j < KMAX; ++j)
          if (j < K && zz[j] < FLT_MAX) best.push_q(zz[j], ii[j], qq[j], K);
      }
    }
    if (xi >= F.W || yi >= F.H) continue;
    const int yo = F.H - 1 - yi, xo = F.W - 1 - xi;
    const int64_t pix = ((int64_t)n * F.H + yo) * F.W + xo;
    const float z0 = best.z[0];
    const bool hit = z0 < FLT_MAX;
    occ_out[pix] = hit ? 1.0f : 0.0f;
#pragma unroll
    for (int j = 0; j < KMAX; ++j) {
      if (j < K) {
        const bool ok = best.z[j] < FLT_MAX && !((best.z[j] - z0) > depth_thres);
        idx_out[pix * K + j] = ok ? best.id[j] : -1;
        zbuf_out[pix * K + j] = ok ? best.z[j] : -1.0f;
        q_out[pix * K + j] = ok ? best.q[j] : -1.0f;
        if (ok && ca.vis) ca.vis[best.id[j]] = 1;
      }
    }
    if (ca.scaler) composite_pixel<KMAX>(best, K, z0, depth_thres, hit, ca, pix);
  }
}

template <int K>
__global__ __launch_bounds__(256) void k_composite_k(const int32_t* __restrict__ idx, const float* __restrict__ qv,
                                                     const float* __restrict__ occ, const float* __restrict__ scaler,
                                                     const float* __restrict__ feat, int C, int norm, float eps,
                                                     int64_t npix, float* __restrict__ frag_scaler, float* __restrict__ out) {
  const int64_t i = (int64_t)blockIdx.x * blockDim.x + threadIdx.x;
  if (i >= npix) return;
  int p[K];
  float q[K];
#pragma unroll
  for (int v = 0; v < K / 4; ++v) {
    const int4 a = reinterpret_cast<const int4*>(idx + i * K)[v];
    const float4 b = reinterpret_cast<const float4*>(qv + i * K)[v];
    p[4 * v] = a.x; p[4 * v + 1] = a.y; p[4 * v + 2] = a.z; p[4 * v + 3] = a.w;
    q[4 * v] = b.x; q[4 * v + 1] = b.y; q[4 * v + 2] = b.z; q[4 * v + 3] = b.w;
  }
  float s[K], f[K][3];
#pragma unroll
  for (int k = 0; k < K; ++k) {
    const int64_t pc = p[k] >= 0 ? p[k] : 0;
    s[k] = p[k] >= 0 ? scaler[pc] : 0.f;
#pragma unroll
    for (int c = 0; c < 3; ++c) f[k][c] = (c < C && p[k] >= 0) ? feat[pc * C + c] : 0.f;
  }
  float sw = 0.f, acc[3] = {0.f, 0.f, 0.f};
#pragma unroll
  for (int k = 0; k < K; ++k) {
    if (p[k] >= 0) {
      const float w = expf(-0.5f * q[k]) * s[k];
#pragma unroll
      for (int c = 0; c < 3; ++c) if (c < C) acc[c] += w * f[k][c];
      sw += w;
    }
  }
  if (frag_scaler) {
#pragma unroll
    for (int v = 0; v < K / 4; ++v)
      reinterpret_cast<float4*>(frag_scaler + i * K)[v] = make_float4(s[4 * v], s[4 * v + 1], s[4 * v + 2], s[4 * v + 3]);
  }
  float d = 1.0f;
  if (norm) d = sw > eps ? sw : eps;
#pragma unroll
  for (int c = 0; c < 3; ++c) if (c < C) out[i * (C + 1) + c] = norm ? acc[c] / d : acc[c];
  out[i * (C + 1) + C] = occ[i];
}

__global__ void k_composite(const int32_t* __restrict__ idx, const float* __restrict__ qv,
                            const float* __restrict__ occ, const float* __restrict__ scaler,
                            const float* __restrict__ feat, int K, int C, int norm, float eps,
                            int64_t npix, float* __restrict__ frag_scaler ,
                            float* __restrict__ out) {
  for (int64_t i = (int64_t)blockIdx.x * blockDim.x + threadIdx.x; i < npix;
       i += (int64_t)gridDim.x * blockDim.x) {
    float sw = 0.f;
    float acc[8];
    for (int c = 0; c < C; ++c) acc[c] = 0.f;
    for (int k = 0; k < K; ++k) {
      const int p = idx[i * K + k];
      float s = 0.f, w = 0.f;
      if (p >= 0) {
        s = scaler[p];
        w = expf(-0.5f * qv[i * K + k]) * s;
        for (int c = 0; c < C; ++c) acc[c] += w * feat[(int64_t)p * C + c];
        sw += w;
      }
      if (frag_scaler) frag_scaler[i * K + k] = s;
    }
    float d = 1.0f;
    if (norm) d = sw > eps ? sw : eps;
    for (int c = 0; c < C; ++c) out[i * (C + 1) + c] = norm ? acc[c] / d : acc[c];
    out[i * (C + 1) + C] = occ[i];
  }
}

__global__ void k_composite_backward(const int32_t* __restrict__ idx, const float* __restrict__ qv,
                                     const float* __restrict__ scaler, const float* __restrict__ feat,
                                     const float* __restrict__ grad_img, int K, int C, int norm, float eps, int64_t npix,
                                     float* __restrict__ grad_feat, float* __restrict__ grad_q,
                                     float* __restrict__ grad_scaler, float* __restrict__ grad_occ) {
  for (int64_t i = (int64_t)blockIdx.x * blockDim.x + threadIdx.x; i < npix; i += (int64_t)gridDim.x * blockDim.x) {
    float g[8], acc[8];
#pragma unroll
    for (int c = 0; c < 8; ++c) { g[c] = c < C ? grad_img[i * (C + 1) + c] : 0.f; acc[c] = 0.f; }
    if (grad_occ) grad_occ[i] = grad_img[i * (C + 1) + C];
    float sw = 0.f;
    for (int k = 0; k < K; ++k) {
      const int p = idx[i * K + k];
      if (p >= 0) {
        const float w = expf(-0.5f * qv[i * K + k]) * scaler[p];
#pragma unroll
        for (int c = 0; c < 8; ++c) if (c < C) acc[c] += w * feat[(int64_t)p * C + c];
        sw += w;
      }
    }
    const float d = norm ? (sw > eps ? sw : eps) : 1.0f;
    const bool through = norm && sw > eps;
    float go = 0.f;
#pragma unroll
    for (int c = 0; c < 8; ++c) if (c < C) go += g[c] * (acc[c] / d);
    for (int k = 0; k < K; ++k) {
      const int p = idx[i * K + k];
      float gq = 0.f;
      if (p >= 0) {
        const float e = expf(-0.5f * qv[i * K + k]);
        const float sc = scaler[p];
        const float w = e * sc;
        float gw = 0.f;
#pragma unroll
        for (int c = 0; c < 8; ++c)
          if (c < C) {
            const float f = feat[(int64_t)p * C + c];
            gw += g[c] * f;
            if (grad_feat && g[c] != 0.f) atomicAdd(&grad_feat[(int64_t)p * C + c], g[c] * w / d);
          }
        gw = (gw - (through ? go : 0.f)) / d;
        gq = -0.5f * w * gw;
        if (grad_scaler && gw != 0.f) atomicAdd(&grad_scaler[p], e * gw);
      }
      if (grad_q) grad_q[i * K + k] = gq;
    }
  }
}

__global__ void k_mark_visible(const int32_t* __restrict__ idx0, int K, int64_t npix,
                               uint8_t* __restrict__ visible, int64_t view_stride = 0) {
  const int32_t* __restrict__ idx = idx0 + (int64_t)blockIdx.y * view_stride * K;
  if ((K & 3) == 0 && ((uintptr_t)idx & 15) == 0) {
    const int4* __restrict__ idx4 = reinterpret_cast<const int4*>(idx);
    const int64_t nq = npix * (K / 4);
    for (int64_t i = (int64_t)blockIdx.x * blockDim.x + threadIdx.x; i < nq; i += (int64_t)gridDim.x * blockDim.x) {
      const int4 p = idx4[i];
      if (p.x >= 0) visible[p.x] = 1;
      if (p.y >= 0) visible[p.y] = 1;
      if (p.z >= 0) visible[p.z] = 1;
      if (p.w >= 0) visible[p.w] = 1;
    }
    return;
  }
  for (int64_t i = (int64_t)blockIdx.x * blockDim.x + threadIdx.x; i < npix;
       i += (int64_t)gridDim.x * blockDim.x) {
    if (idx[i * K] < 0) continue;
    for (int k = 0; k < K; ++k) {
      const int p = idx[i * K + k];
      if (p >= 0) visible[p] = 1;
    }
  }
}

__global__ void k_zbuf_scatter(const int32_t* __restrict__ idx, const float* __restrict__ gz,
                               int K, int64_t npix, float* __restrict__ z_grad) {
  for (int64_t i = (int64_t)blockIdx.x * blockDim.x + threadIdx.x; i < npix;
       i += (int64_t)gridDim.x * blockDim.x) {
    for (int k = 0; k < K; ++k) {
      const float g = gz[i * K + k];
      if (g == 0.0f) continue;
      const int p = idx[i * K + k];
      if (p < 0) break;
      atomicAdd(&z_grad[p], g);
    }
  }
}

constexpr int GB = 8;
struct BlkGeo { int NBx, NBy, NB2x, NB2y; };
static inline BlkGeo make_blk(int H, int W) {
  BlkGeo g;
  g.NBx = (W + GB - 1) / GB; g.NBy = (H + GB - 1) / GB; g.NB2x = (g.NBx + 7) / 8; g.NB2y = (g.NBy + 7) / 8;
  return g;
}

__global__ __launch_bounds__(256) void k_grad_maps(const float* __restrict__ grad_occ, Frame F, BlkGeo G, int N,
                                                   unsigned long long* __restrict__ pixmask ,
                                                   uint8_t* __restrict__ rowbytes ,
                                                   uint8_t* __restrict__ blk2 ,
                                                   int32_t* __restrict__ clear_a, int n_clear_a,
                                                   int32_t* __restrict__ clear_b, int n_clear_b) {
  if (blockIdx.x == 0) {
    if ((int)threadIdx.x < n_clear_a) clear_a[threadIdx.x] = 0;
    if (clear_b && (int)threadIdx.x < n_clear_b) clear_b[threadIdx.x] = 0;
  }
  const int lane = threadIdx.x & 63;
  const int64_t total = (int64_t)N * G.NB2x * G.NB2y;
  for (int64_t sb = (int64_t)blockIdx.x * 4 + (threadIdx.x >> 6); sb < total; sb += (int64_t)gridDim.x * 4) {
    const int sx = sb % G.NB2x, sy = (sb / G.NB2x) % G.NB2y, n = sb / ((int64_t)G.NB2x * G.NB2y);
    const int bx = sx * 8 + (lane & 7), by = sy * 8 + (lane >> 3);
    unsigned long long m = 0ull;
    if (bx < G.NBx && by < G.NBy) {
      const int x0 = bx * GB, x1 = min(F.W, x0 + GB);
      for (int y = by * GB; y < min(F.H, (by + 1) * GB); ++y) {
        const float* row = grad_occ + ((int64_t)n * F.H + y) * F.W;
        unsigned bits = 0u;
        if (x1 - x0 == GB && (((uintptr_t)(row + x0)) & 15) == 0) {
          const float4 a = *reinterpret_cast<const float4*>(row + x0), c = *reinterpret_cast<const float4*>(row + x0 + 4);
          bits = (unsigned)(a.x != 0.f) | ((unsigned)(a.y != 0.f) << 1) | ((unsigned)(a.z != 0.f) << 2) | ((unsigned)(a.w != 0.f) << 3) |
                 ((unsigned)(c.x != 0.f) << 4) | ((unsigned)(c.y != 0.f) << 5) | ((unsigned)(c.z != 0.f) << 6) | ((unsigned)(c.w != 0.f) << 7);
        } else {
          for (int x = x0; x < x1; ++x) bits |= (unsigned)(row[x] != 0.0f) << (x - x0);
        }
        m |= (unsigned long long)bits << (8 * (y - by * GB));
      }
      pixmask[((int64_t)n * G.NBy + by) * G.NBx + bx] = m;
    }
    const unsigned long long bal = __ballot(m != 0ull);
    if ((lane & 7) == 0 && by < G.NBy) rowbytes[((int64_t)n * G.NBy + by) * G.NB2x + sx] = (uint8_t)((bal >> (8 * (lane >> 3))) & 0xffull);
    if (lane == 0) blk2[sb] = bal ? 1 : 0;
  }
}



__device__ __forceinline__ bool out_range(float c, float r, int n, float e, int m, int& lo, int& hi) {
  int a, b;
  if (!pixel_range(c, r, n, e, m, a, b)) return false;
  lo = n - 1 - b;
  hi = n - 1 - a;
  return true;
}

__device__ __forceinline__ void occ_term(float g, float dx, float dy, float rx, float ry, float sx,
                                         float sy, float r2, int rect_mode, float radii_s, float& gx,
                                         float& gy) {
  if (g == 0.0f) return;
  const float dist2 = dx * dx + dy * dy;
  bool outside;
  if (rect_mode) {
    if (fabsf(dx) > sx || fabsf(dy) > sy) return;
    outside = (fabsf(dx) > sx / radii_s) || (fabsf(dy) > sy / radii_s);
  } else {
    if (dist2 > r2) return;
    outside = (fabsf(dx) > rx) || (fabsf(dy) > ry);
  }
  if (g > 0.0f && outside) return;
  const float denom = iso_eps_denom(dist2, 1e-10f);
  gx += dx / denom * g;
  gy += dy / denom * g;
}

__global__ __launch_bounds__(256) void k_splat_backward(
    const float* __restrict__ pts, const float* __restrict__ radii,
    const uint8_t* __restrict__ visible, const float* __restrict__ rs,
    const int64_t* __restrict__ first, const int64_t* __restrict__ num,
    const uint8_t* __restrict__ blk2, BlkGeo G, Frame F, int rect_mode, float radii_s,
    int32_t* __restrict__ heavy, int32_t* __restrict__ heavy_count, float* __restrict__ grad,
    long long* __restrict__ zacc ,
    ZRider rider, int own_blocks) {
  if ((int)blockIdx.x >= own_blocks) {
    if (blockIdx.y == 0) z_absmax_body(rider.gz, rider.n, rider.zs, blockIdx.x - own_blocks, rider.blocks);
    return;
  }
  const int n = blockIdx.y;
  const int64_t len = num[n], base = first[n];
  const float r = rect_mode ? 0.f : rs[n];
  const int lane = threadIdx.x & 63, wv = threadIdx.x >> 6;
  __shared__ int s_wcnt[4][4], s_base;
  const int64_t span = (int64_t)own_blocks * 1024;
  for (int64_t i0 = (int64_t)blockIdx.x * 1024; i0 < len; i0 += span) {
    bool is_heavy[4];
    int64_t pp[4];
    unsigned long long bal[4];
#pragma unroll
    for (int k = 0; k < 4; ++k) {
      const int64_t i = i0 + k * 256 + threadIdx.x;
      is_heavy[k] = false;
      pp[k] = -1;
      if (i < len) {
        const int64_t p = base + i;
        pp[k] = p;
        const float px = pts[p * 3], py = pts[p * 3 + 1], pz = pts[p * 3 + 2];
        const float rx = radii[p * 2], ry = radii[p * 2 + 1];
        const bool vis = (!visible || visible[p]);
        grad[p * 3] = 0.f; grad[p * 3 + 1] = 0.f; grad[p * 3 + 2] = 0.f;
        if (zacc) zacc[p] = 0;
        const float sx = rect_mode ? rx * radii_s : r, sy = rect_mode ? ry * radii_s : r;
        if (vis && !(pz < 0.f || fabsf(py) > F.ey || fabsf(px) > F.ex) && sx > 0.f && sy > 0.f) {
          int x0, x1, y0, y1;
          if (out_range(px, sx, F.W, F.ex, F.m, x0, x1) && out_range(py, sy, F.H, F.ey, F.m, y0, y1)) {
            for (int sy2 = y0 / 64; sy2 <= y1 / 64 && !is_heavy[k]; ++sy2)
              for (int sx2 = x0 / 64; sx2 <= x1 / 64; ++sx2)
                if (blk2[((int64_t)n * G.NB2y + sy2) * G.NB2x + sx2]) { is_heavy[k] = true; break; }
          }
        }
      }
      bal[k] = __ballot(is_heavy[k]);
      if (lane == 0) s_wcnt[k][wv] = __popcll(bal[k]);
    }
    __syncthreads();
    if (threadIdx.x == 0) {
      int tot = 0;
#pragma unroll
      for (int q = 0; q < 16; ++q) tot += s_wcnt[q >> 2][q & 3];
      s_base = tot ? atomicAdd(heavy_count, tot) : 0;
    }
    __syncthreads();
    int b0 = s_base;
#pragma unroll
    for (int k = 0; k < 4; ++k) {
#pragma unroll
      for (int q = 0; q < 4; ++q) {
        if (q == wv && is_heavy[k]) heavy[b0 + __popcll(bal[k] & ((1ull << lane) - 1ull))] = (int32_t)pp[k];
        b0 += s_wcnt[k][q];
      }
    }
    __syncthreads();
  }
}

__global__ __launch_bounds__(256) void k_splat_backward_heavy(
    const float* __restrict__ pts, const float* __restrict__ radii, const float* __restrict__ rs,
    const int64_t* __restrict__ first, const int64_t* __restrict__ num, int n_clouds,
    const float* __restrict__ grad_occ, const unsigned long long* __restrict__ pixmask,
    const uint8_t* __restrict__ rowbytes, BlkGeo G, Frame F,
    int rect_mode, float radii_s, const int32_t* __restrict__ heavy,
    const int32_t* __restrict__ heavy_count, float* __restrict__ grad, ZRider rider, int own_blocks) {
  if ((int)blockIdx.x >= own_blocks) {
    z_finish_body(rider.acc, rider.zs, first, num, n_clouds, rider.grad, rider.terms_log2, blockIdx.x - own_blocks, rider.blocks);
    return;
  }
  const int count = *heavy_count;
  constexpr int LP = 8;
  const int j = threadIdx.x & (LP - 1);
  unsigned long long diag = 0ull;
  for (int ry = 0; ry < 8; ++ry) diag |= 1ull << (8 * ry + ((j - ry) & 7));
  for (int w = (blockIdx.x * blockDim.x + threadIdx.x) / LP; w < (count + 63) / 64 * 64; w += own_blocks * blockDim.x / LP) {
    const bool live = w < count;
    const int64_t p = live ? heavy[w] : 0;
    int n = 0;
    for (int c = 1; c < n_clouds; ++c) if (p >= first[c]) n = c;
    const float r = rect_mode ? 0.f : rs[n], r2 = r * r;
    const float px = pts[p * 3], py = pts[p * 3 + 1];
    const float rx = radii[p * 2], ry = radii[p * 2 + 1];
    const float sx = rect_mode ? rx * radii_s : r, sy = rect_mode ? ry * radii_s : r;
    int x0, x1, y0, y1;
    float gx = 0.f, gy = 0.f;
    if (live && out_range(px, sx, F.W, F.ex, F.m, x0, x1) && out_range(py, sy, F.H, F.ey, F.m, y0, y1)) {
      const float* __restrict__ gimg = grad_occ + (int64_t)n * F.H * F.W;
      const int bx0 = x0 / GB, bx1 = x1 / GB, by0 = y0 / GB, by1 = y1 / GB;
      constexpr int RY = 4;
      for (int cx = bx0 >> 3; cx <= bx1 >> 3; cx += 4) {
        const int ka = max(bx0 - cx * 8, 0), kb = min(bx1 - cx * 8, 31);
        const unsigned colwin = (0xffffffffu >> (31 - kb)) & (0xffffffffu << ka);
        for (int byc = by0; byc <= by1; byc += RY) {
          unsigned fl[RY];
#pragma unroll
          for (int t = 0; t < RY; ++t) {
            fl[t] = 0u;
            if (byc + t <= by1) {
              const uint8_t* rp = rowbytes + ((int64_t)n * G.NBy + byc + t) * G.NB2x + cx;
              unsigned wv;
              __builtin_memcpy(&wv, rp, 4);
              fl[t] = wv & colwin;
            }
          }
#pragma unroll
          for (int t = 0; t < RY; ++t) {
            const int by = byc + t;
            unsigned flags = fl[t];
            if (!flags) continue;
            const int ra = max(y0 - by * GB, 0), rb = min(y1 - by * GB, GB - 1);
            const unsigned long long rowsel = (rb == 7 ? ~0ull : ((1ull << (8 * (rb + 1))) - 1ull)) & ~((1ull << (8 * ra)) - 1ull);
            while (flags) {
              const int k = __ffs((int)flags) - 1;
              flags &= flags - 1;
              const int bx = cx * 8 + k;
              const int ca = max(x0 - bx * GB, 0), cb = min(x1 - bx * GB, GB - 1);
              const unsigned long long colsel = (unsigned long long)((0xffu >> (7 - cb)) & (0xffu << ca)) * 0x0101010101010101ull;
              const unsigned long long win = rowsel & colsel;
              unsigned long long m = pixmask[((int64_t)n * G.NBy + by) * G.NBx + bx] & win;
              if (m == win && bx * GB + GB <= F.W && (F.W & 3) == 0 && (((uintptr_t)gimg) & 15) == 0) {
                if (j >= ra && j <= rb) {
                  const int yo = by * GB + j;
                  const float4* rowp = reinterpret_cast<const float4*>(gimg + (int64_t)yo * F.W + bx * GB);
                  const float4 ga = rowp[0], gb = rowp[1];
                  const float gv[8] = {ga.x, ga.y, ga.z, ga.w, gb.x, gb.y, gb.z, gb.w};
                  const float dy = ndc_y(F.H - 1 - yo, F) - py;
#pragma unroll
                  for (int rxx = 0; rxx < GB; ++rxx)
                    if (rxx >= ca && rxx <= cb)
                      occ_term(gv[rxx], ndc_x(F.W - 1 - (bx * GB + rxx), F) - px, dy, rx, ry, sx, sy, r2, rect_mode, radii_s, gx, gy);
                }
                continue;
              }
              m &= diag;
              while (m) {
                const int b = __ffsll((long long)m) - 1;
                m &= m - 1;
                const int yo = by * GB + (b >> 3), xo = bx * GB + (b & 7);
                const float g = gimg[(int64_t)yo * F.W + xo];
                occ_term(g, ndc_x(F.W - 1 - xo, F) - px, ndc_y(F.H - 1 - yo, F) - py, rx, ry, sx, sy, r2, rect_mode, radii_s, gx, gy);
              }
            }
          }
        }
      }
    }
#pragma unroll
    for (int o = 1; o < LP; o <<= 1) {
      gx += __shfl_xor(gx, o);
      gy += __shfl_xor(gy, o);
    }
    if (live && j == 0) { grad[p * 3] = gx; grad[p * 3 + 1] = gy; }
  }
}

constexpr int kRselBins = 2048;
constexpr int kRselShift[3] = {21, 10, 0};
constexpr int kRselBits[3] = {11, 11, 10};

__device__ bool rsel_resolve(const unsigned* __restrict__ hist, int n, int n_clouds, int passes, unsigned& prefix,
                             long long& k, long long& cnt, long long* s_w , long long* s_pub ) {
  prefix = 0u; k = 0; cnt = 0;
  const int t = threadIdx.x, lane = t & 63, w = t >> 6;
  for (int q = 0; q < passes; ++q) {
    const unsigned* hq = hist + ((int64_t)q * n_clouds + n) * kRselBins;
    long long v[8], sum = 0;
#pragma unroll
    for (int e = 0; e < 8; ++e) { v[e] = hq[t * 8 + e]; sum += v[e]; }
    long long inc = sum;
#pragma unroll
    for (int o = 1; o < 64; o <<= 1) { const long long u = __shfl_up(inc, o); if (lane >= o) inc += u; }
    if (lane == 63) s_w[w] = inc;
    __syncthreads();
    long long base = 0, tot = 0;
#pragma unroll
    for (int j = 0; j < 4; ++j) { if (j < w) base += s_w[j]; tot += s_w[j]; }
    if (q == 0) { cnt = tot; k = tot > 0 ? (tot - 1) / 2 : 0; }
    if (cnt == 0) { __syncthreads(); return false; }
    long long ex = base + inc - sum;
    if (k >= ex && k < ex + sum) {
      int bsel = 0;
#pragma unroll
      for (int e = 0; e < 8; ++e) { if (k >= ex + v[e] && e < 7 && bsel == e) { ex += v[e]; bsel = e + 1; } }
      s_pub[0] = t * 8 + bsel; s_pub[1] = ex;
    }
    __syncthreads();
    prefix |= ((unsigned)s_pub[0]) << kRselShift[q];
    k -= s_pub[1];
    __syncthreads();
  }
  return true;
}

template <int PASS>
__global__ __launch_bounds__(256) void k_rsel_hist(const float* __restrict__ radii,
                                                   const uint8_t* __restrict__ visible,
                                                   const int64_t* __restrict__ first,
                                                   const int64_t* __restrict__ num,
                                                   unsigned* __restrict__ hist ) {
  __shared__ unsigned lh[kRselBins];
  __shared__ long long s_w[4], s_pub[2];
  const int n = blockIdx.y, n_clouds = gridDim.y;
  unsigned prefix = 0u;
  long long k, cnt;
  if (PASS > 0 && !rsel_resolve(hist, n, n_clouds, PASS, prefix, k, cnt, s_w, s_pub)) return;
  for (int j = threadIdx.x; j < kRselBins; j += 256) lh[j] = 0u;
  __syncthreads();
  constexpr int shift = kRselShift[PASS];
  constexpr unsigned dmask = (1u << kRselBits[PASS]) - 1u;
  const unsigned hi_mask = PASS == 0 ? 0u : (0xffffffffu << (shift + kRselBits[PASS]));
  const int64_t len = num[n], base = first[n];
  for (int64_t i = (int64_t)blockIdx.x * blockDim.x + threadIdx.x; i < len;
       i += (int64_t)gridDim.x * blockDim.x) {
    const int64_t p = base + i;
    if (!visible[p]) continue;
    const float2 r2 = *reinterpret_cast<const float2*>(radii + p * 2);
    const unsigned k0 = __float_as_uint(r2.x), k1 = __float_as_uint(r2.y);
    if ((k0 & hi_mask) == prefix) atomicAdd(&lh[(k0 >> shift) & dmask], 1u);
    if ((k1 & hi_mask) == prefix) atomicAdd(&lh[(k1 >> shift) & dmask], 1u);
  }
  __syncthreads();
  unsigned* hp = hist + ((int64_t)PASS * n_clouds + n) * kRselBins;
  for (int j = threadIdx.x; j < kRselBins; j += 256)
    if (lh[j]) atomicAdd(&hp[j], lh[j]);
}

__global__ __launch_bounds__(256) void k_rsel_final(unsigned* __restrict__ hist, int n_clouds, float radii_s,
                                                    float* __restrict__ out) {
  __shared__ long long s_w[4], s_pub[2];
  const int n = blockIdx.x;
  if (n >= n_clouds) return;
  unsigned prefix;
  long long k, cnt;
  const bool any = rsel_resolve(hist, n, n_clouds, 3, prefix, k, cnt, s_w, s_pub);
  if (threadIdx.x == 0) out[n] = any ? __uint_as_float(prefix) * radii_s : 0.0f;
  __syncthreads();
  for (int q = 0; q < 3; ++q)
    for (int j = threadIdx.x; j < kRselBins; j += 256) hist[((int64_t)q * n_clouds + n) * kRselBins + j] = 0u;
}

}

extern "C" int iso_splat_view_flags(const float* points, const float* normals,
                                    const float* views, int32_t* flags, int64_t P, int n_views,
                                    float znear, float zfar, int backface_culling, void* stream) {
  ISO_REQUIRE(P >= 0 && n_views >= 0, ISO_ERR_INVALID, "iso_splat_view_flags: bad sizes");
  if (P == 0 || n_views == 0) return ISO_OK;
  ISO_REQUIRE(points && views && flags && (normals || !backface_culling), ISO_ERR_INVALID,
              "iso_splat_view_flags: null pointer");
  int gx = iso_div_up(P, 256); if (gx > 4096) gx = 4096;
  hipLaunchKernelGGL(k_view_flags, dim3(gx, n_views), dim3(256), 0, (hipStream_t)stream, points,
                     normals, views, flags, P, znear, zfar, backface_culling);
  ISO_CHECK_LAUNCH("iso_splat_view_flags");
  return ISO_OK;
}

extern "C" int iso_compact_rows(const float* in, const int32_t* flags, const int32_t* offsets,
                                float* out, int64_t P, int64_t total, int U, void* stream) {
  ISO_REQUIRE(P >= 0 && total >= 0 && U >= 0, ISO_ERR_INVALID, "iso_compact_rows: bad sizes");
  if (total == 0 || U == 0) return ISO_OK;
  ISO_REQUIRE(in && flags && offsets && out && P > 0, ISO_ERR_INVALID, "iso_compact_rows: null pointer");
  hipLaunchKernelGGL(k_compact_rows, dim3(iso_stream_grid(total, 256)), dim3(256), 0,
                     (hipStream_t)stream, in, flags, offsets, out, P, total, U);
  ISO_CHECK_LAUNCH("iso_compact_rows");
  return ISO_OK;
}

extern "C" int iso_splat_vrk_h(const float* dists, const int64_t* first_idx, const int64_t* num_pts,
                               const int64_t* cloud_num_pts, float* h, int n_clouds,
                               int64_t p_stride, void* stream) {
  ISO_REQUIRE(n_clouds >= 0 && p_stride >= 0, ISO_ERR_INVALID, "iso_splat_vrk_h: bad sizes");
  if (n_clouds == 0 || p_stride == 0) return ISO_OK;
  ISO_REQUIRE(dists && first_idx && num_pts && h, ISO_ERR_INVALID, "iso_splat_vrk_h: null pointer");
  int gx = iso_div_up(p_stride, 256); if (gx > 4096) gx = 4096;
  hipLaunchKernelGGL(k_vrk_h, dim3(gx, n_clouds), dim3(256), 0, (hipStream_t)stream, dists,
                     first_idx, num_pts, cloud_num_pts, h, p_stride);
  ISO_CHECK_LAUNCH("iso_splat_vrk_h");
  return ISO_OK;
}

extern "C" int iso_splat_setup(const float* points, const float* normals, const float* h,
                               const int64_t* first_idx, const int64_t* num_pts,
                               const float* views, const float* projs, int n_views,
                               int64_t max_pts, int image_size, float sigma, float cutoff,
                               float* ndc_out, float* ellipse_out, float* cutoff_out,
                               float* radii_out, float* scaler_out, void* stream) {
  ISO_REQUIRE(n_views >= 0 && max_pts >= 0 && image_size > 0, ISO_ERR_INVALID, "iso_splat_setup: bad sizes");
  if (n_views == 0 || max_pts == 0) return ISO_OK;
  ISO_REQUIRE(points && normals && h && first_idx && num_pts && views && projs && ndc_out &&
                  ellipse_out && cutoff_out && radii_out && scaler_out,
              ISO_ERR_INVALID, "iso_splat_setup: null pointer");
  SetupOut o{ndc_out, ellipse_out, cutoff_out, radii_out, scaler_out};
  int gx = iso_div_up(max_pts, 256); if (gx > 4096) gx = 4096;
  hipLaunchKernelGGL(k_splat_setup, dim3(gx, n_views), dim3(256), 0, (hipStream_t)stream, points,
                     normals, h, first_idx, num_pts, views, projs, image_size, sigma, cutoff, o);
  ISO_CHECK_LAUNCH("iso_splat_setup");
  return ISO_OK;
}

extern "C" int64_t iso_splat_vrk_h_global_work_bytes(int n_clouds) {
  return n_clouds > 0 ? (int64_t)n_clouds * kHSlices * (int64_t)sizeof(double) : 0;
}

extern "C" int iso_splat_vrk_h_global(const float* dists, const int64_t* first_idx, const int64_t* num_pts, float* h,
                                      int n_clouds, int64_t p_stride, int64_t padded_len, void* work, void* stream) {
  ISO_REQUIRE(n_clouds >= 0 && p_stride >= 0 && padded_len >= p_stride, ISO_ERR_INVALID,
              "iso_splat_vrk_h_global: bad sizes (padded_len must be >= p_stride)");
  if (n_clouds == 0 || p_stride == 0) return ISO_OK;
  ISO_REQUIRE(dists && first_idx && num_pts && h && work, ISO_ERR_INVALID, "iso_splat_vrk_h_global: null pointer");
  hipLaunchKernelGGL(k_vrk_h_partial, dim3(kHSlices, n_clouds), dim3(kHBlock), 0, (hipStream_t)stream, dists, num_pts,
                     p_stride, padded_len, (double*)work);
  ISO_CHECK_LAUNCH("iso_splat_vrk_h_global (partial sums)");
  int gx = iso_div_up(p_stride, 256); if (gx > 4096) gx = 4096;
  hipLaunchKernelGGL(k_vrk_h_finish, dim3(gx, n_clouds), dim3(256), 0, (hipStream_t)stream, (const double*)work, first_idx,
                     num_pts, padded_len, h);
  ISO_CHECK_LAUNCH("iso_splat_vrk_h_global");
  return ISO_OK;
}

extern "C" int iso_splat_tangent_frame(const float* normals, int64_t n, float* u_out, float* v_out, void* stream) {
  ISO_REQUIRE(n >= 0, ISO_ERR_INVALID, "iso_splat_tangent_frame: bad sizes");
  if (n == 0) return ISO_OK;
  ISO_REQUIRE(normals && u_out && v_out, ISO_ERR_INVALID, "iso_splat_tangent_frame: null pointer");
  hipLaunchKernelGGL(k_tangent_frame, dim3(iso_stream_grid(n, 256)), dim3(256), 0, (hipStream_t)stream, normals, n, u_out,
                     v_out);
  ISO_CHECK_LAUNCH("iso_splat_tangent_frame");
  return ISO_OK;
}

extern "C" int iso_splat_setup_vrk(const float* points, const float* frames, const float* curvature,
                                   const int64_t* first_idx, const int64_t* num_pts, const float* views, const float* projs,
                                   int n_views, int64_t max_pts, int image_size, float sigma, float cutoff, float* ndc_out,
                                   float* ellipse_out, float* cutoff_out, float* radii_out, float* scaler_out, void* stream) {
  ISO_REQUIRE(n_views >= 0 && max_pts >= 0 && image_size > 0, ISO_ERR_INVALID, "iso_splat_setup_vrk: bad sizes");
  if (n_views == 0 || max_pts == 0) return ISO_OK;
  ISO_REQUIRE(points && frames && curvature && first_idx && num_pts && views && projs && ndc_out && ellipse_out &&
                  cutoff_out && radii_out && scaler_out,
              ISO_ERR_INVALID, "iso_splat_setup_vrk: null pointer");
  SetupOut o{ndc_out, ellipse_out, cutoff_out, radii_out, scaler_out};
  int gx = iso_div_up(max_pts, 256); if (gx > 4096) gx = 4096;
  hipLaunchKernelGGL(k_splat_setup_vrk, dim3(gx, n_views), dim3(256), 0, (hipStream_t)stream, points, frames, curvature,
                     first_idx, num_pts, views, projs, image_size, sigma, cutoff, o);
  ISO_CHECK_LAUNCH("iso_splat_setup_vrk");
  return ISO_OK;
}

extern "C" int iso_splat_setup_aniso(const float* points, const int64_t* knn_idx, int64_t p_stride,
                                     const int64_t* first_idx, const int64_t* num_pts, const float* views,
                                     const float* projs, int n_views, int image_size, float sigma, float cutoff,
                                     float* ndc_out, float* ellipse_out, float* cutoff_out, float* radii_out,
                                     float* scaler_out, void* stream) {
  ISO_REQUIRE(n_views >= 0 && p_stride >= 0 && image_size > 0, ISO_ERR_INVALID, "iso_splat_setup_aniso: bad sizes");
  if (n_views == 0 || p_stride == 0) return ISO_OK;
  ISO_REQUIRE(points && knn_idx && first_idx && num_pts && views && projs && ndc_out && ellipse_out && cutoff_out &&
                  radii_out && scaler_out,
              ISO_ERR_INVALID, "iso_splat_setup_aniso: null pointer");
  SetupOut o{ndc_out, ellipse_out, cutoff_out, radii_out, scaler_out};
  int gx = iso_div_up(p_stride, 256); if (gx > 4096) gx = 4096;
  hipLaunchKernelGGL(k_splat_setup_aniso, dim3(gx, n_views), dim3(256), 0, (hipStream_t)stream, points, knn_idx, p_stride,
                     first_idx, num_pts, views, projs, image_size, sigma, cutoff, o);
  ISO_CHECK_LAUNCH("iso_splat_setup_aniso");
  return ISO_OK;
}

extern "C" int64_t iso_splat_front_workspace_bytes(int64_t n_points) {
  if (n_points < 0) n_points = 0;
  const int64_t n_chunks = (n_points + kChunk - 1) / kChunk;
  return 8 * 4 * (n_chunks + 1) + 8 * 4 * (4 * n_chunks + 4);
}

// ... 243 lines not shown
  }
  bool items_done = false;
  if (max_pts > 0) {
    ISO_REQUIRE(points && ellipse && cutoff && radii, ISO_ERR_INVALID, "iso_splat_forward: null pointer");
    items_done = launch_bin<true>(points, radii, first_idx, num_pts, n_clouds, max_pts, F, tile_row_begin,
                                  tile_row_end, tile_cursor, tile_off, pairs, pair_capacity, overflow_flag, s,
                                  TileItemsJob{ty_rows, n_clouds, max_slots, kTargetItems, items, heavy, counters});
  }
  if (K > 32) {
    hipLaunchKernelGGL(k_tile_order, dim3(1), dim3(1024), 0, s, tile_off, F, tile_row_begin, ty_rows, n_clouds, tile_cursor);
    hipLaunchKernelGGL(k_raster_deep, dim3(tiles), dim3(256), 0, s, points, ellipse, cutoff, radii, tile_cursor, tile_off, pairs,
                       pair_capacity, F, K, depth_merging_thres, idx_out, zbuf_out, qvalue_out, occ_out, ca);
    ISO_CHECK_LAUNCH("iso_splat_forward");
    return ISO_OK;
  }
  if (items) {
    if (!items_done)
      hipLaunchKernelGGL(k_tile_items, dim3(1), dim3(1024), 0, s, tile_off, F, tile_row_begin, ty_rows, n_clouds, max_slots,
                         kTargetItems, items, heavy, counters);
  } else {
    hipLaunchKernelGGL(k_tile_order, dim3(1), dim3(1024), 0, s, tile_off, F, tile_row_begin, ty_rows, n_clouds,
                       tile_cursor);
  }
#define ISO_LAUNCH_R(KM_)                                                                            \
  if (K == KM_)                                                                                      \
    hipLaunchKernelGGL((k_raster<KM_, true>), dim3(tiles + max_slots), dim3(256), 0, s, points, ellipse, cutoff, radii, \
                       tile_cursor, items, counters, scratch, tile_off, pairs, pair_capacity, F,                \
                       K, depth_merging_thres, idx_out, zbuf_out, qvalue_out, occ_out, ca);             \
  else                                                                                               \
    hipLaunchKernelGGL((k_raster<KM_>), dim3(tiles + max_slots), dim3(256), 0, s, points, ellipse, cutoff, radii, \
                       tile_cursor, items, counters, scratch, tile_off, pairs, pair_capacity, F,                \
                       K, depth_merging_thres, idx_out, zbuf_out, qvalue_out, occ_out, ca);             \
  if (items && K == KM_)                                                                              \
    hipLaunchKernelGGL((k_raster_merge<KM_, true>), dim3(tiles < 1024 ? tiles : 1024), dim3(256), 0, s, heavy, counters, scratch, \
                       F, K, depth_merging_thres, idx_out, zbuf_out, qvalue_out, occ_out, ca);              \
  else if (items)                                                                                     \
    hipLaunchKernelGGL(k_raster_merge<KM_>, dim3(tiles < 1024 ? tiles : 1024), dim3(256), 0, s, heavy, counters, scratch, \
                       F, K, depth_merging_thres, idx_out, zbuf_out, qvalue_out, occ_out, ca)
  if (K <= 4) { ISO_LAUNCH_R(4); }
  else if (K <= 8) { ISO_LAUNCH_R(8); }
  else if (K <= 16) { ISO_LAUNCH_R(16); }
  else { ISO_LAUNCH_R(32); }
#undef ISO_LAUNCH_R
  ISO_CHECK_LAUNCH("iso_splat_forward");
  return ISO_OK;
}

extern "C" int iso_splat_forward(const float* points, const float* ellipse, const float* cutoff,
                                 const float* radii, const int64_t* first_idx,
                                 const int64_t* num_pts, int n_clouds, int64_t max_pts,
                                 float depth_merging_thres, int image_size, int image_width, int points_per_pixel,
                                 int tile_row_begin, int tile_row_end, int32_t* tile_cursor,
                                 const int32_t* tile_off, int32_t* pairs,
                                 int64_t pair_capacity, int32_t* overflow_flag, int32_t* idx_out,
                                 float* zbuf_out, float* qvalue_out, float* occ_out, void* workspace,
                                 int64_t workspace_bytes, void* stream) {
  CompositeArgs ca{nullptr, nullptr, nullptr, 0, 0, 0.f, nullptr};
  return splat_forward_impl(ca, points, ellipse, cutoff, radii, first_idx, num_pts, n_clouds, max_pts, depth_merging_thres,
                            image_size, image_width, points_per_pixel, tile_row_begin, tile_row_end, tile_cursor, tile_off, pairs,
                            pair_capacity, overflow_flag, idx_out, zbuf_out, qvalue_out, occ_out, workspace,
                            workspace_bytes, stream);
}

extern "C" int iso_splat_render(const float* points, const float* ellipse, const float* cutoff,
                                const float* radii, const int64_t* first_idx,
                                const int64_t* num_pts, int n_clouds, int64_t max_pts,
                                float depth_merging_thres, int image_size, int image_width, int points_per_pixel,
                                int tile_row_begin, int tile_row_end, int32_t* tile_cursor,
                                const int32_t* tile_off, int32_t* pairs,
                                int64_t pair_capacity, int32_t* overflow_flag, int32_t* idx_out,
                                float* zbuf_out, float* qvalue_out, float* occ_out, void* workspace,
                                int64_t workspace_bytes, const float* scaler, const float* features, int channels,
                                int norm_weighted, float eps, float* image_out, void* stream) {
  return iso_splat_render_visible(points, ellipse, cutoff, radii, first_idx, num_pts, n_clouds, max_pts, depth_merging_thres,
                                  image_size, image_width, points_per_pixel, tile_row_begin, tile_row_end, tile_cursor, tile_off,
                                  pairs, pair_capacity, overflow_flag, idx_out, zbuf_out, qvalue_out, occ_out, workspace,
                                  workspace_bytes, scaler, features, channels, norm_weighted, eps, image_out, nullptr, stream);
}

extern "C" int iso_splat_render_visible(const float* points, const float* ellipse, const float* cutoff,
                                        const float* radii, const int64_t* first_idx,
                                        const int64_t* num_pts, int n_clouds, int64_t max_pts,
                                        float depth_merging_thres, int image_size, int image_width, int points_per_pixel,
                                        int tile_row_begin, int tile_row_end, int32_t* tile_cursor,
                                        const int32_t* tile_off, int32_t* pairs,
                                        int64_t pair_capacity, int32_t* overflow_flag, int32_t* idx_out,
                                        float* zbuf_out, float* qvalue_out, float* occ_out, void* workspace,
                                        int64_t workspace_bytes, const float* scaler, const float* features, int channels,
                                        int norm_weighted, float eps, float* image_out, uint8_t* visible_out, void* stream) {
  ISO_REQUIRE(channels >= 0 && channels <= 8, ISO_ERR_UNSUPPORTED, "iso_splat_render: channels must be <= 8");
  ISO_REQUIRE(scaler && image_out && (features || channels == 0), ISO_ERR_INVALID, "iso_splat_render: null pointer");
  CompositeArgs ca{scaler, features, image_out, channels, norm_weighted, eps, visible_out};
  return splat_forward_impl(ca, points, ellipse, cutoff, radii, first_idx, num_pts, n_clouds, max_pts, depth_merging_thres,
                            image_size, image_width, points_per_pixel, tile_row_begin, tile_row_end, tile_cursor, tile_off, pairs,
                            pair_capacity, overflow_flag, idx_out, zbuf_out, qvalue_out, occ_out, workspace,
                            workspace_bytes, stream);
}

extern "C" int iso_rasterize_coarse(const float* points, const float* radii, const int64_t* first_idx,
                                    const int64_t* num_pts, int n_clouds, int image_size, int bin_size,
                                    int max_points_per_bin, int32_t* bin_points_out, int32_t* overflow_out, void* stream) {
  ISO_REQUIRE(n_clouds >= 0 && image_size > 0 && bin_size > 0 && max_points_per_bin >= 0, ISO_ERR_INVALID,
              "iso_rasterize_coarse: bad sizes");
  const int B = 1 + (image_size - 1) / bin_size;
  if (n_clouds == 0 || max_points_per_bin == 0) return ISO_OK;
  ISO_REQUIRE(points && radii && first_idx && num_pts && bin_points_out && overflow_out, ISO_ERR_INVALID,
              "iso_rasterize_coarse: null pointer");
  hipLaunchKernelGGL(k_coarse_bins, dim3(B * B, n_clouds), dim3(256), 0, (hipStream_t)stream, points, radii, first_idx,
                     num_pts, image_size, bin_size, B, max_points_per_bin, bin_points_out, overflow_out);
  ISO_CHECK_LAUNCH("iso_rasterize_coarse");
  return ISO_OK;
}

extern "C" int iso_rasterize_fine(const float* points, const float* ellipse, const float* cutoff, const float* radii,
                                  int64_t n_points, const int32_t* bin_points, int n_clouds, int max_points_per_bin,
                                  float depth_merging_thres, int image_size, int bin_size, int points_per_pixel,
                                  int32_t* idx_out, float* zbuf_out, float* qvalue_out, float* occ_out, void* stream) {
  ISO_REQUIRE(n_clouds >= 0 && image_size > 0 && bin_size > 0 && max_points_per_bin >= 0 && n_points >= 0, ISO_ERR_INVALID,
              "iso_rasterize_fine: bad sizes");
  ISO_REQUIRE(points_per_pixel >= 1 && points_per_pixel <= 150, ISO_ERR_UNSUPPORTED,
              "iso_rasterize_fine: points_per_pixel must be in [1,150] (rasterization_utils.cuh:18), got %d", points_per_pixel);
  if (n_clouds == 0) return ISO_OK;
  ISO_REQUIRE(idx_out && zbuf_out && qvalue_out && occ_out && (max_points_per_bin == 0 || bin_points) &&
                  (n_points == 0 || (points && ellipse && cutoff && radii)),
              ISO_ERR_INVALID, "iso_rasterize_fine: null pointer");
  const Frame F = make_frame(image_size, image_size);
  const int B = 1 + (image_size - 1) / bin_size;
  const int64_t npix = (int64_t)n_clouds * image_size * image_size;
  const int K = points_per_pixel;
  hipStream_t s = (hipStream_t)stream;
#define ISO_FINE(KM_)                                                                                               \
  hipLaunchKernelGGL(k_fine_bins<KM_>, dim3(iso_stream_grid(npix, 256)), dim3(256), 0, s, points, ellipse, cutoff, radii, \
                     bin_points, n_clouds, B, max_points_per_bin, bin_size, F, K, depth_merging_thres, n_points, idx_out,  \
                     zbuf_out, qvalue_out, occ_out)
  if (K <= 4) ISO_FINE(4);
  else if (K <= 8) ISO_FINE(8);
  else if (K <= 16) ISO_FINE(16);
  else if (K <= 32) ISO_FINE(32);
  else
    hipLaunchKernelGGL(k_fine_bins_deep, dim3(iso_stream_grid(npix, 256)), dim3(256), 0, s, points, ellipse, cutoff, radii,
                       bin_points, n_clouds, B, max_points_per_bin, bin_size, F, K, depth_merging_thres, n_points, idx_out,
                       zbuf_out, qvalue_out, occ_out);
#undef ISO_FINE
  ISO_CHECK_LAUNCH("iso_rasterize_fine");
  return ISO_OK;
}

namespace {
__global__ __launch_bounds__(256) void k_gather_neg_idx(const float* __restrict__ values, const int32_t* __restrict__ idx,
                                                        int64_t n, float* __restrict__ out) {
  const int64_t i0 = ((int64_t)blockIdx.x * 256 + threadIdx.x) * 4;
  if (i0 + 3 < n) {
    const int4 k = *reinterpret_cast<const int4*>(idx + i0);
    float4 r;
    r.x = k.x >= 0 ? values[k.x] : 0.f;
    r.y = k.y >= 0 ? values[k.y] : 0.f;
    r.z = k.z >= 0 ? values[k.z] : 0.f;
    r.w = k.w >= 0 ? values[k.w] : 0.f;
    *reinterpret_cast<float4*>(out + i0) = r;
  } else {
    for (int64_t i = i0; i < n; ++i) { const int k = idx[i]; out[i] = k >= 0 ? values[k] : 0.f; }
  }
}
}

extern "C" int iso_gather_neg_idx(const float* values, const int32_t* idx, int64_t n, float* out, void* stream) {
  ISO_REQUIRE(n >= 0, ISO_ERR_INVALID, "iso_gather_neg_idx: bad size");
  if (n == 0) return ISO_OK;
  ISO_REQUIRE(values && idx && out, ISO_ERR_INVALID, "iso_gather_neg_idx: null pointer");
  ISO_REQUIRE((((uintptr_t)idx | (uintptr_t)out) & 15) == 0, ISO_ERR_INVALID, "iso_gather_neg_idx: idx / out must be 16-byte aligned");
  hipLaunchKernelGGL(k_gather_neg_idx, dim3((unsigned)((n + 1023) / 1024)), dim3(256), 0, (hipStream_t)stream, values, idx, n, out);
  ISO_CHECK_LAUNCH("iso_gather_neg_idx");
  return ISO_OK;
}

extern "C" int iso_splat_composite(const int32_t* idx, const float* qvalue, const float* occ,
                                   const float* scaler, const float* features, int64_t n_pixels,
                                   int points_per_pixel, int channels, int norm_weighted, float eps,
                                   float* frag_scaler_out, float* image_out, void* stream) {
  ISO_REQUIRE(channels >= 0 && channels <= 8, ISO_ERR_UNSUPPORTED, "iso_splat_composite: channels must be <= 8");
  ISO_REQUIRE(n_pixels >= 0 && points_per_pixel >= 1, ISO_ERR_INVALID, "iso_splat_composite: bad sizes");
  if (n_pixels == 0) return ISO_OK;
  ISO_REQUIRE(idx && qvalue && occ && scaler && image_out && (features || channels == 0),
              ISO_ERR_INVALID, "iso_splat_composite: null pointer");
  const bool aligned = (((uintptr_t)idx | (uintptr_t)qvalue | (uintptr_t)frag_scaler_out) & 15) == 0;
  if (aligned && channels <= 3 && points_per_pixel == 8)
    hipLaunchKernelGGL(k_composite_k<8>, dim3((unsigned)((n_pixels + 255) / 256)), dim3(256), 0, (hipStream_t)stream, idx, qvalue,
                       occ, scaler, features, channels, norm_weighted, eps, n_pixels, frag_scaler_out, image_out);
  else if (aligned && channels <= 3 && points_per_pixel == 4)
    hipLaunchKernelGGL(k_composite_k<4>, dim3((unsigned)((n_pixels + 255) / 256)), dim3(256), 0, (hipStream_t)stream, idx, qvalue,
                       occ, scaler, features, channels, norm_weighted, eps, n_pixels, frag_scaler_out, image_out);
  else
  hipLaunchKernelGGL(k_composite, dim3(iso_stream_grid(n_pixels, 256)), dim3(256), 0,
                     (hipStream_t)stream, idx, qvalue, occ, scaler, features, points_per_pixel,
                     channels, norm_weighted, eps, n_pixels, frag_scaler_out, image_out);
  ISO_CHECK_LAUNCH("iso_splat_composite");
  return ISO_OK;
}

extern "C" int iso_splat_composite_backward(const int32_t* idx, const float* qvalue, const float* scaler,
                                            const float* features, const float* grad_image, int64_t n_pixels,
                                            int points_per_pixel, int channels, int norm_weighted, float eps,
                                            float* grad_features, float* grad_qvalue, float* grad_scaler,
                                            float* grad_occ, void* stream) {
  ISO_REQUIRE(channels >= 0 && channels <= 8, ISO_ERR_UNSUPPORTED, "iso_splat_composite_backward: channels must be <= 8");
  ISO_REQUIRE(n_pixels >= 0 && points_per_pixel >= 1, ISO_ERR_INVALID, "iso_splat_composite_backward: bad sizes");
  if (n_pixels == 0) return ISO_OK;
  ISO_REQUIRE(idx && qvalue && scaler && grad_image && (features || channels == 0), ISO_ERR_INVALID,
              "iso_splat_composite_backward: null pointer");
  hipLaunchKernelGGL(k_composite_backward, dim3(iso_stream_grid(n_pixels, 256)), dim3(256), 0, (hipStream_t)stream, idx,
                     qvalue, scaler, features, grad_image, points_per_pixel, channels, norm_weighted, eps, n_pixels,
                     grad_features, grad_qvalue, grad_scaler, grad_occ);
  ISO_CHECK_LAUNCH("iso_splat_composite_backward");
  return ISO_OK;
}

extern "C" int iso_splat_mark_visible(const int32_t* idx, int64_t n_pixels, int points_per_pixel,
                                      uint8_t* visible, void* stream) {
  ISO_REQUIRE(n_pixels >= 0 && points_per_pixel >= 1, ISO_ERR_INVALID, "iso_splat_mark_visible: bad sizes");
  if (n_pixels == 0) return ISO_OK;
  ISO_REQUIRE(idx && visible, ISO_ERR_INVALID, "iso_splat_mark_visible: null pointer");
  hipLaunchKernelGGL(k_mark_visible, dim3(iso_stream_grid(n_pixels, 256)), dim3(256), 0,
                     (hipStream_t)stream, idx, points_per_pixel, n_pixels, visible);
  ISO_CHECK_LAUNCH("iso_splat_mark_visible");
  return ISO_OK;
}

extern "C" int64_t iso_splat_median_radius_workspace_bytes(int n_clouds) {
  if (n_clouds < 0) n_clouds = 0;
  return (int64_t)n_clouds * 3 * kRselBins * 4 + 64;
}

extern "C" int iso_splat_median_radius(const float* radii, const uint8_t* visible,
                                       const int64_t* first_idx, const int64_t* num_pts,
                                       int n_clouds, int64_t max_pts, float radii_s,
                                       void* workspace, int64_t workspace_bytes,
                                       float* search_radius_out, void* stream) {
  ISO_REQUIRE(n_clouds >= 0 && max_pts >= 0, ISO_ERR_INVALID, "iso_splat_median_radius: bad sizes");
  if (n_clouds == 0) return ISO_OK;
  ISO_REQUIRE(first_idx && num_pts && workspace && search_radius_out && (max_pts == 0 || (radii && visible)),
              ISO_ERR_INVALID, "iso_splat_median_radius: null pointer");
  ISO_REQUIRE(workspace_bytes >= iso_splat_median_radius_workspace_bytes(n_clouds), ISO_ERR_WORKSPACE,
              "iso_splat_median_radius: workspace too small");
  ISO_REQUIRE(((uintptr_t)radii & 7) == 0, ISO_ERR_INVALID, "iso_splat_median_radius: radii must be 8-byte aligned");
  hipStream_t s = (hipStream_t)stream;
  unsigned* hist = (unsigned*)workspace;
  int gx = iso_div_up(max_pts > 0 ? max_pts : 1, 256 * 8);
  if (gx > 512) gx = 512;
  if (max_pts > 0) {
    hipLaunchKernelGGL(k_rsel_hist<0>, dim3(gx, n_clouds), dim3(256), 0, s, radii, visible, first_idx, num_pts, hist);
    hipLaunchKernelGGL(k_rsel_hist<1>, dim3(gx, n_clouds), dim3(256), 0, s, radii, visible, first_idx, num_pts, hist);
    hipLaunchKernelGGL(k_rsel_hist<2>, dim3(gx, n_clouds), dim3(256), 0, s, radii, visible, first_idx, num_pts, hist);
  }
  hipLaunchKernelGGL(k_rsel_final, dim3(n_clouds), dim3(256), 0, s, hist, n_clouds, radii_s, search_radius_out);
  ISO_CHECK_LAUNCH("iso_splat_median_radius");
  return ISO_OK;
}

extern "C" int64_t iso_splat_median_pass_words(int n_clouds) { return (int64_t)(n_clouds < 0 ? 0 : n_clouds) * kRselBins; }

extern "C" int iso_splat_median_pass(int pass, const float* radii, const uint8_t* visible, const int64_t* first_idx,
                                     const int64_t* num_pts, int n_clouds, int64_t max_pts, void* workspace,
                                     int64_t workspace_bytes, void* stream) {
  ISO_REQUIRE(pass >= 0 && pass <= 2 && n_clouds >= 0 && max_pts >= 0, ISO_ERR_INVALID, "iso_splat_median_pass: bad arguments");
  if (n_clouds == 0 || max_pts == 0) return ISO_OK;
  ISO_REQUIRE(radii && visible && first_idx && num_pts && workspace, ISO_ERR_INVALID, "iso_splat_median_pass: null pointer");
  ISO_REQUIRE(workspace_bytes >= iso_splat_median_radius_workspace_bytes(n_clouds), ISO_ERR_WORKSPACE,
              "iso_splat_median_pass: workspace too small");
  hipStream_t s = (hipStream_t)stream;
  unsigned* hist = (unsigned*)workspace;
  int gx = iso_div_up(max_pts, 256 * 8);
  if (gx > 512) gx = 512;
  if (pass == 0) hipLaunchKernelGGL(k_rsel_hist<0>, dim3(gx, n_clouds), dim3(256), 0, s, radii, visible, first_idx, num_pts, hist);
  else if (pass == 1) hipLaunchKernelGGL(k_rsel_hist<1>, dim3(gx, n_clouds), dim3(256), 0, s, radii, visible, first_idx, num_pts, hist);
  else hipLaunchKernelGGL(k_rsel_hist<2>, dim3(gx, n_clouds), dim3(256), 0, s, radii, visible, first_idx, num_pts, hist);
  ISO_CHECK_LAUNCH("iso_splat_median_pass");
  return ISO_OK;
}

extern "C" int iso_splat_median_final(void* workspace, int n_clouds, float radii_s, float* search_radius_out, void* stream) {
  ISO_REQUIRE(n_clouds >= 0 && (n_clouds == 0 || (workspace && search_radius_out)), ISO_ERR_INVALID,
              "iso_splat_median_final: bad arguments");
  if (n_clouds == 0) return ISO_OK;
  hipLaunchKernelGGL(k_rsel_final, dim3(n_clouds), dim3(256), 0, (hipStream_t)stream, (unsigned*)workspace, n_clouds, radii_s,
                     search_radius_out);
  ISO_CHECK_LAUNCH("iso_splat_median_final");
  return ISO_OK;
}

extern "C" int iso_splat_zbuf_backward(const int32_t* idx, const float* grad_zbuf,
                                       int64_t n_pixels, int points_per_pixel, float* z_grad,
                                       void* stream) {
  ISO_REQUIRE(n_pixels >= 0 && points_per_pixel >= 1, ISO_ERR_INVALID, "iso_splat_zbuf_backward: bad sizes");
  if (n_pixels == 0) return ISO_OK;
  ISO_REQUIRE(idx && grad_zbuf && z_grad, ISO_ERR_INVALID, "iso_splat_zbuf_backward: null pointer");
  hipLaunchKernelGGL(k_zbuf_scatter, dim3(iso_stream_grid(n_pixels, 256)), dim3(256), 0,
                     (hipStream_t)stream, idx, grad_zbuf, points_per_pixel, n_pixels, z_grad);
  ISO_CHECK_LAUNCH("iso_splat_zbuf_backward");
  return ISO_OK;
}

struct ZScale { unsigned max_bits; int exp2; };

__device__ void z_absmax_body(const float* __restrict__ gz, int64_t n, ZScale* __restrict__ zs, int block, int nblocks) {
  __shared__ unsigned sm[4];
  unsigned m = 0u;
  const int64_t n4 = n / 4;
  const uint4* g4 = reinterpret_cast<const uint4*>(gz);
  const int64_t stride = (int64_t)nblocks * blockDim.x;
  int64_t i = (int64_t)block * blockDim.x + threadIdx.x;
  for (; i + 3 * stride < n4; i += 4 * stride) {
    const uint4 v0 = g4[i], v1 = g4[i + stride], v2 = g4[i + 2 * stride], v3 = g4[i + 3 * stride];
    const unsigned a = max(max(v0.x & 0x7fffffffu, v0.y & 0x7fffffffu), max(v0.z & 0x7fffffffu, v0.w & 0x7fffffffu));
    const unsigned b = max(max(v1.x & 0x7fffffffu, v1.y & 0x7fffffffu), max(v1.z & 0x7fffffffu, v1.w & 0x7fffffffu));
    const unsigned c = max(max(v2.x & 0x7fffffffu, v2.y & 0x7fffffffu), max(v2.z & 0x7fffffffu, v2.w & 0x7fffffffu));
    const unsigned d = max(max(v3.x & 0x7fffffffu, v3.y & 0x7fffffffu), max(v3.z & 0x7fffffffu, v3.w & 0x7fffffffu));
    m = max(m, max(max(a, b), max(c, d)));
  }
  for (; i < n4; i += stride) {
    const uint4 v = g4[i];
    const unsigned a = max(v.x & 0x7fffffffu, v.y & 0x7fffffffu), b = max(v.z & 0x7fffffffu, v.w & 0x7fffffffu);
    m = max(m, max(a, b));
  }
  for (int64_t t = n4 * 4 + (int64_t)block * blockDim.x + threadIdx.x; t < n; t += stride)
    m = max(m, __float_as_uint(gz[t]) & 0x7fffffffu);
#pragma unroll
  for (int o = 32; o > 0; o >>= 1) m = max(m, (unsigned)__shfl_xor((int)m, o));
  if ((threadIdx.x & 63) == 0) sm[threadIdx.x >> 6] = m;
  __syncthreads();
  if (threadIdx.x == 0) {
    m = max(max(sm[0], sm[1]), max(sm[2], sm[3]));
    if (m) atomicMax(&zs->max_bits, m);
  }
}

__global__ __launch_bounds__(256) void k_z_absmax(const float* __restrict__ gz0, int64_t n, ZScale* __restrict__ zs,
                                                  int64_t view_stride = 0) {
  z_absmax_body(gz0 + (int64_t)blockIdx.y * view_stride, n, zs, blockIdx.x, gridDim.x);
}

__device__ __forceinline__ int z_exponent(unsigned max_bits, int terms_log2) {
  int e = 0;
  if (max_bits != 0u && max_bits < 0x7f800000u) {
    int ex;
    (void)frexpf(__uint_as_float(max_bits), &ex);
    e = 61 - terms_log2 - ex;
  }
  return e;
}
__global__ void k_z_scale(ZScale* zs, int terms_log2) { zs->exp2 = z_exponent(zs->max_bits, terms_log2); }

__device__ __forceinline__ void z_scatter_one(int p, float g, int e, long long* __restrict__ acc) {
  if (g == 0.0f) return;
  if (g != g || fabsf(g) > 3.0e38f) {
    atomicMax(&acc[p], 1ll << 62);
    return;
  }
  const long long q = __double2ll_rn(ldexp((double)g, e));
  atomicAdd(reinterpret_cast<unsigned long long*>(&acc[p]), (unsigned long long)q);
}

__global__ void k_z_scatter(const int32_t* __restrict__ idx0, const float* __restrict__ gz0, int K, int64_t npix,
                            const ZScale* __restrict__ zs, long long* __restrict__ acc, int64_t view_stride = 0,
                            int terms_log2 = -1) {
  const int32_t* __restrict__ idx = idx0 + (int64_t)blockIdx.y * view_stride * K;
  const float* __restrict__ gz = gz0 + (int64_t)blockIdx.y * view_stride * K;
  const int e = terms_log2 >= 0 ? z_exponent(zs->max_bits, terms_log2) : zs->exp2;
  if ((K & 3) == 0 && (((uintptr_t)idx | (uintptr_t)gz) & 15) == 0) {
    const int4* __restrict__ idx4 = reinterpret_cast<const int4*>(idx);
    const float4* __restrict__ gz4 = reinterpret_cast<const float4*>(gz);
    const int64_t nq = npix * (K / 4);
    for (int64_t i = (int64_t)blockIdx.x * blockDim.x + threadIdx.x; i < nq; i += (int64_t)gridDim.x * blockDim.x) {
      const float4 g = gz4[i];
      if (g.x == 0.0f && g.y == 0.0f && g.z == 0.0f && g.w == 0.0f) continue;
      const int4 p = idx4[i];
      if (p.x < 0) continue;
      z_scatter_one(p.x, g.x, e, acc);
      if (p.y >= 0) z_scatter_one(p.y, g.y, e, acc);
      if (p.z >= 0) z_scatter_one(p.z, g.z, e, acc);
      if (p.w >= 0) z_scatter_one(p.w, g.w, e, acc);
    }
    return;
  }
  for (int64_t i = (int64_t)blockIdx.x * blockDim.x + threadIdx.x; i < npix; i += (int64_t)gridDim.x * blockDim.x) {
    for (int k = 0; k < K; ++k) {
      const int p = idx[i * K + k];
      if (p < 0) break;
      z_scatter_one(p, gz[i * K + k], e, acc);
    }
  }
}

__global__ void k_z_finish(const long long* __restrict__ acc, const ZScale* __restrict__ zs, int64_t n,
                           float* __restrict__ grad, int terms_log2 = -1) {
  const int e = terms_log2 >= 0 ? z_exponent(zs->max_bits, terms_log2) : zs->exp2;
  for (int64_t p = (int64_t)blockIdx.x * blockDim.x + threadIdx.x; p < n; p += (int64_t)gridDim.x * blockDim.x) {
    const long long a = acc[p];
    float z = (float)ldexp((double)a, -e);
    if (a >= (1ll << 61) || a <= -(1ll << 61)) z = __builtin_nanf("");
    grad[p * 3 + 2] = z;
  }
}

__device__ void z_finish_body(const long long* __restrict__ acc, const ZScale* __restrict__ zs, const int64_t* __restrict__ first,
                              const int64_t* __restrict__ num, int n_clouds, float* __restrict__ grad, int terms_log2,
                              int block, int nblocks) {
  const int e = z_exponent(zs->max_bits, terms_log2);
  for (int c = 0; c < n_clouds; ++c) {
    const int64_t len = num[c], base = first[c];
    for (int64_t i = (int64_t)block * blockDim.x + threadIdx.x; i < len; i += (int64_t)nblocks * blockDim.x) {
      const int64_t p = base + i;
      const long long a = acc[p];
      float z = (float)ldexp((double)a, -e);
      if (a >= (1ll << 61) || a <= -(1ll << 61)) z = __builtin_nanf("");
      grad[p * 3 + 2] = z;
    }
  }
}

__global__ void k_z_finish_clouds(const long long* __restrict__ acc, const ZScale* __restrict__ zs,
                                  const int64_t* __restrict__ first, const int64_t* __restrict__ num,
                                  float* __restrict__ grad, int terms_log2) {
  z_finish_body(acc, zs, first + blockIdx.y, num + blockIdx.y, 1, grad, terms_log2, blockIdx.x, gridDim.x);
}

static int64_t bwd_maps_bytes(int n_clouds, int image_size, int image_width) {
  const BlkGeo G = make_blk(image_size, image_width > 0 ? image_width : image_size);
  return (((int64_t)n_clouds * ((int64_t)G.NBx * G.NBy * 8 + (int64_t)G.NB2x * G.NBy + (int64_t)G.NB2x * G.NB2y)) + 63) / 64 * 64;
}
extern "C" int64_t iso_splat_backward_workspace_bytes(int n_clouds, int image_size, int image_width,
                                                      int64_t total_points) {
  if (total_points < 0) total_points = 0;
  return bwd_maps_bytes(n_clouds, image_size, image_width) + 64 + (4 * total_points + 15) / 16 * 16 + 16 + 8 * total_points;
}

extern "C" int iso_splat_backward(const float* points, const float* radii, const uint8_t* visible,
                                  const float* search_radius, const int64_t* first_idx,
                                  const int64_t* num_pts, int n_clouds, int64_t max_pts,
                                  const float* grad_occ, const int32_t* idx,
                                  const float* grad_zbuf, int image_size, int image_width, int points_per_pixel,
                                  int rect_mode, float radii_s, int64_t total_points,
                                  void* workspace, int64_t workspace_bytes, float* grad_points,
                                  void* stream) {
  ISO_REQUIRE(n_clouds >= 0 && max_pts >= 0 && image_size > 0, ISO_ERR_INVALID, "iso_splat_backward: bad sizes");
  if (n_clouds == 0 || max_pts == 0) return ISO_OK;
  ISO_REQUIRE(points && radii && (search_radius || rect_mode) && first_idx && num_pts && grad_occ &&
                  grad_points && workspace && (!grad_zbuf || idx),
              ISO_ERR_INVALID, "iso_splat_backward: null pointer");
  ISO_REQUIRE(workspace_bytes >= iso_splat_backward_workspace_bytes(n_clouds, image_size, image_width, total_points),
              ISO_ERR_WORKSPACE, "iso_splat_backward: workspace too small");
  const Frame F = make_frame(image_size, image_width > 0 ? image_width : image_size);
  const BlkGeo G = make_blk(F.H, F.W);
  ISO_REQUIRE(F.H <= 2048 && F.W <= 2048, ISO_ERR_UNSUPPORTED, "iso_splat_backward: image sides must be <= 2048");
  hipStream_t s = (hipStream_t)stream;
  unsigned long long* pixmask = (unsigned long long*)workspace;
  uint8_t* rowbytes = (uint8_t*)(pixmask + (int64_t)n_clouds * G.NBx * G.NBy);
  uint8_t* blk2 = rowbytes + (int64_t)n_clouds * G.NB2x * G.NBy;
  int32_t* heavy_count = (int32_t*)((uint8_t*)workspace + bwd_maps_bytes(n_clouds, image_size, image_width));
  int32_t* heavy = heavy_count + 16;
  const bool with_z = grad_zbuf && total_points > 0;
  ZScale* zs = reinterpret_cast<ZScale*>((char*)(heavy_count) + 64 + (4 * total_points + 15) / 16 * 16);
  long long* zacc = reinterpret_cast<long long*>((char*)zs + 16);
  {
    int gmaps = iso_div_up((int64_t)n_clouds * G.NB2x * G.NB2y, 4);
    hipLaunchKernelGGL(k_grad_maps, dim3(gmaps < 1 ? 1 : gmaps), dim3(256), 0, s, grad_occ, F, G, n_clouds, pixmask, rowbytes, blk2,
                       heavy_count, 16, with_z ? reinterpret_cast<int32_t*>(zs) : nullptr, 4);
  }
  int gx = iso_div_up(max_pts, 1024); if (gx > 8192) gx = 8192;
  const int64_t npix = (int64_t)n_clouds * F.H * F.W;
  int terms_log2 = 0;
  while ((1ll << terms_log2) < (int64_t)F.H * F.W) ++terms_log2;
  ZRider r1{nullptr, 0, zs, 0, nullptr, nullptr, 0}, r2 = r1;
  if (with_z) {
    int gm = iso_div_up(npix * points_per_pixel, 256 * 16); if (gm > 1024) gm = 1024; if (gm < 1) gm = 1;
    r1 = ZRider{grad_zbuf, npix * points_per_pixel, zs, gm, nullptr, nullptr, 0};
    r2 = ZRider{nullptr, 0, zs, iso_stream_grid(total_points, 256), zacc, grad_points, terms_log2};
  }
  hipLaunchKernelGGL(k_splat_backward, dim3(gx + r1.blocks, n_clouds), dim3(256), 0, s, points, radii, visible,
                     search_radius, first_idx, num_pts, blk2, G, F, rect_mode, radii_s, heavy,
                     heavy_count, grad_points, with_z ? zacc : nullptr, r1, gx);
  if (with_z)
    hipLaunchKernelGGL(k_z_scatter, dim3(iso_stream_grid(npix, 256)), dim3(256), 0, s, idx, grad_zbuf,
                       points_per_pixel, npix, zs, zacc, (int64_t)0, terms_log2);
  constexpr int heavy_grid = 4096;
  hipLaunchKernelGGL(k_splat_backward_heavy, dim3(heavy_grid + r2.blocks), dim3(256), 0, s, points, radii, search_radius,
                     first_idx, num_pts, n_clouds, grad_occ, pixmask, rowbytes, G, F, rect_mode, radii_s,
                     heavy, heavy_count, grad_points, r2, heavy_grid);
  ISO_CHECK_LAUNCH("iso_splat_backward");
  return ISO_OK;
}

extern "C" int iso_splat_z_absmax(const float* grad_zbuf, int64_t n, int32_t* zscale, void* stream) {
  ISO_REQUIRE(zscale && n >= 0 && (grad_zbuf || n == 0), ISO_ERR_INVALID, "iso_splat_z_absmax: bad arguments");
  hipStream_t s = (hipStream_t)stream;
  iso_zero_words(zscale, 2, s);
  if (n > 0) {
    int gm = iso_div_up(n, 256 * 16); if (gm > 1024) gm = 1024; if (gm < 1) gm = 1;
    hipLaunchKernelGGL(k_z_absmax, dim3(gm), dim3(256), 0, s, grad_zbuf, n, reinterpret_cast<ZScale*>(zscale));
  }
  ISO_CHECK_LAUNCH("iso_splat_z_absmax");
  return ISO_OK;
}

extern "C" int iso_splat_z_scatter(const int32_t* idx, const float* grad_zbuf, int64_t n_pixels, int points_per_pixel,
                                   int64_t pixels_per_view, int32_t* zscale, int64_t* acc, void* stream) {
  ISO_REQUIRE(zscale && acc && n_pixels >= 0 && points_per_pixel >= 1 && pixels_per_view > 0 && ((idx && grad_zbuf) || n_pixels == 0),
              ISO_ERR_INVALID, "iso_splat_z_scatter: bad arguments");
  hipStream_t s = (hipStream_t)stream;
  int terms_log2 = 0;
  while ((1ll << terms_log2) < pixels_per_view) ++terms_log2;
  hipLaunchKernelGGL(k_z_scale, dim3(1), dim3(1), 0, s, reinterpret_cast<ZScale*>(zscale), terms_log2);
  if (n_pixels > 0)
    hipLaunchKernelGGL(k_z_scatter, dim3(iso_stream_grid(n_pixels, 256)), dim3(256), 0, s, idx, grad_zbuf, points_per_pixel,
                       n_pixels, reinterpret_cast<const ZScale*>(zscale), reinterpret_cast<long long*>(acc));
  ISO_CHECK_LAUNCH("iso_splat_z_scatter");
  return ISO_OK;
}

extern "C" int iso_splat_band_marks(const int32_t* idx, const float* grad_zbuf, int n_views, int64_t view_pixels,
                                    int64_t band_pixels, int points_per_pixel, uint8_t* visible, int32_t* zscale,
                                    void* stream) {
  ISO_REQUIRE(zscale && n_views >= 0 && view_pixels >= band_pixels && band_pixels >= 0 && points_per_pixel >= 1,
              ISO_ERR_INVALID, "iso_splat_band_marks: bad arguments");
  hipStream_t s = (hipStream_t)stream;
  iso_zero_words(zscale, 2, s);
  if (band_pixels == 0 || n_views == 0) return ISO_OK;
  ISO_REQUIRE(idx && grad_zbuf && visible, ISO_ERR_INVALID, "iso_splat_band_marks: null pointer");
  ISO_REQUIRE((((uintptr_t)grad_zbuf) & 15) == 0 && ((view_pixels * points_per_pixel) & 3) == 0 &&
                  ((band_pixels * points_per_pixel) & 3) == 0,
              ISO_ERR_UNSUPPORTED, "iso_splat_band_marks: grad_zbuf slices must be 16-byte aligned");
  hipLaunchKernelGGL(k_mark_visible, dim3(iso_stream_grid(band_pixels, 256), n_views), dim3(256), 0, s, idx,
                     points_per_pixel, band_pixels, visible, view_pixels);
  const int64_t n = band_pixels * points_per_pixel;
  int gm = iso_div_up(n, 256 * 16); if (gm > 1024) gm = 1024; if (gm < 1) gm = 1;
  hipLaunchKernelGGL(k_z_absmax, dim3(gm, n_views), dim3(256), 0, s, grad_zbuf, n, reinterpret_cast<ZScale*>(zscale),
                     view_pixels * points_per_pixel);
  ISO_CHECK_LAUNCH("iso_splat_band_marks");
  return ISO_OK;
}

extern "C" int iso_splat_band_z_scatter(const int32_t* idx, const float* grad_zbuf, int n_views, int64_t view_pixels,
                                        int64_t band_pixels, int points_per_pixel, int32_t* zscale, int64_t* acc,
                                        void* stream) {
  ISO_REQUIRE(zscale && acc && n_views >= 0 && view_pixels > 0 && band_pixels >= 0 && points_per_pixel >= 1 &&
                  ((idx && grad_zbuf) || band_pixels == 0),
              ISO_ERR_INVALID, "iso_splat_band_z_scatter: bad arguments");
  hipStream_t s = (hipStream_t)stream;
  int terms_log2 = 0;
  while ((1ll << terms_log2) < view_pixels) ++terms_log2;
  hipLaunchKernelGGL(k_z_scale, dim3(1), dim3(1), 0, s, reinterpret_cast<ZScale*>(zscale), terms_log2);
  if (band_pixels > 0 && n_views > 0)
    hipLaunchKernelGGL(k_z_scatter, dim3(iso_stream_grid(band_pixels, 256), n_views), dim3(256), 0, s, idx, grad_zbuf,
                       points_per_pixel, band_pixels, reinterpret_cast<const ZScale*>(zscale),
                       reinterpret_cast<long long*>(acc), view_pixels);
  ISO_CHECK_LAUNCH("iso_splat_band_z_scatter");
  return ISO_OK;
}

namespace {
__global__ void k_z_finish_rows(const long long* __restrict__ acc, const ZScale* __restrict__ zs, int64_t row0, int64_t n,
                                float* __restrict__ grad) {
  const int e = zs->exp2;
  for (int64_t j = (int64_t)blockIdx.x * blockDim.x + threadIdx.x; j < n; j += (int64_t)gridDim.x * blockDim.x) {
    const long long a = acc[row0 + j];
    float z = (float)ldexp((double)a, -e);
    if (a >= (1ll << 61) || a <= -(1ll << 61)) z = __builtin_nanf("");
    grad[(row0 + j) * 3 + 2] = z;
  }
}

__global__ __launch_bounds__(256) void k_repack_records(const float* __restrict__ gathered, int64_t cap, int world,
                                                        int n_views, const int32_t* __restrict__ counts, float cutoffC,
                                                        int64_t max_rows, float* __restrict__ ndc, float* __restrict__ ellipse,
                                                        float* __restrict__ cutoff, float* __restrict__ radii,
                                                        float* __restrict__ scaler, float* __restrict__ feat) {
  const int s = blockIdx.y, v = blockIdx.z;
  int64_t g0 = 0, l0 = 0;
  for (int vv = 0; vv < n_views; ++vv)
    for (int ss = 0; ss < world; ++ss) {
      const int c = counts[ss * 8 + vv];
      if (vv < v || (vv == v && ss < s)) g0 += c;
      if (ss == s && vv < v) l0 += c;
    }
  int64_t n = counts[s * 8 + v];
  if (l0 + n > cap) n = cap > l0 ? cap - l0 : 0;
  if (g0 + n > max_rows) n = max_rows > g0 ? max_rows - g0 : 0;
  const float* blk = gathered + (int64_t)s * 12 * cap;
  const int64_t t0 = (int64_t)blockIdx.x * blockDim.x + threadIdx.x, step = (int64_t)gridDim.x * blockDim.x;
  for (int64_t j = t0; j < 3 * n; j += step) {
    ndc[g0 * 3 + j] = blk[l0 * 3 + j];
    ellipse[g0 * 3 + j] = blk[3 * cap + l0 * 3 + j];
    feat[g0 * 3 + j] = blk[9 * cap + l0 * 3 + j];
  }
  for (int64_t j = t0; j < 2 * n; j += step) radii[g0 * 2 + j] = blk[6 * cap + l0 * 2 + j];
  for (int64_t j = t0; j < n; j += step) {
    scaler[g0 + j] = blk[8 * cap + l0 + j];
    cutoff[g0 + j] = cutoffC;
  }
}

__global__ void k_repack_offsets(const int32_t* __restrict__ counts, int world, int n_views, int rank, int64_t max_rows,
                                 int64_t* __restrict__ first_g, int64_t* __restrict__ num_g,
                                 int64_t* __restrict__ first_own, int64_t* __restrict__ num_own) {
  if (threadIdx.x != 0 || blockIdx.x != 0) return;
  int64_t run = 0;
  for (int v = 0; v < n_views; ++v) {
    first_g[v] = run < max_rows ? run : max_rows;
    for (int s = 0; s < world; ++s) {
      const int64_t c = counts[s * 8 + v];
      if (s == rank) { first_own[v] = run < max_rows ? run : max_rows; num_own[v] = run + c <= max_rows ? c : (max_rows > run ? max_rows - run : 0); }
      run += c;
    }
    num_g[v] = (run < max_rows ? run : max_rows) - first_g[v];
  }
}
}

extern "C" int iso_splat_z_finish(const int64_t* acc, const int32_t* zscale, int64_t row0, int64_t n_rows,
                                  float* grad_points, void* stream) {
  ISO_REQUIRE(acc && zscale && grad_points && row0 >= 0 && n_rows >= 0, ISO_ERR_INVALID, "iso_splat_z_finish: bad arguments");
  if (n_rows > 0)
    hipLaunchKernelGGL(k_z_finish_rows, dim3(iso_stream_grid(n_rows, 256)), dim3(256), 0, (hipStream_t)stream,
                       reinterpret_cast<const long long*>(acc), reinterpret_cast<const ZScale*>(zscale), row0, n_rows,
                       grad_points);
  ISO_CHECK_LAUNCH("iso_splat_z_finish");
  return ISO_OK;
}

extern "C" int iso_splat_repack(const float* gathered, int64_t capacity, int world, int rank, int n_views,
                                const int32_t* counts, float cutoff, int64_t max_rows, float* ndc_out,
                                float* ellipse_out, float* cutoff_out, float* radii_out, float* scaler_out,
                                float* features_out, int64_t* first_idx_out, int64_t* num_pts_out,
                                int64_t* own_first_out, int64_t* own_num_out, void* stream) {
  ISO_REQUIRE(gathered && counts && world >= 1 && rank >= 0 && rank < world && n_views >= 1 && n_views <= 8 &&
                  capacity >= 0 && ndc_out && ellipse_out && cutoff_out && radii_out && scaler_out && features_out &&
                  first_idx_out && num_pts_out && own_first_out && own_num_out,
              ISO_ERR_INVALID, "iso_splat_repack: bad arguments");
  hipStream_t s = (hipStream_t)stream;
  hipLaunchKernelGGL(k_repack_offsets, dim3(1), dim3(64), 0, s, counts, world, n_views, rank, max_rows, first_idx_out,
                     num_pts_out, own_first_out, own_num_out);
  int gx = iso_div_up(max_rows > 0 ? 3 * max_rows / (world * n_views) + 1 : 1, 256); if (gx > 256) gx = 256;
  hipLaunchKernelGGL(k_repack_records, dim3(gx, world, n_views), dim3(256), 0, s, gathered, capacity, world, n_views, counts,
                     cutoff, max_rows, ndc_out, ellipse_out, cutoff_out, radii_out, scaler_out, features_out);
  ISO_CHECK_LAUNCH("iso_splat_repack");
  return ISO_OK;
}
```

Before: 74.61.

## Fuse SIREN weight packing and splat-backward z-gradient passes into fewer launches

The SIREN weight-packing path now runs as one multi-role kernel that writes the f32, x3 and split-fp16 images together, after a column-parallel scale/stat kernel that publishes per-group partial maxima to a device global. In splat backward, the z-gradient absmax now produces per-block partial maxima and rides inside the grad-maps kernel along with accumulator clearing. The scatter rides inside the main backward kernel, and the finish step rides inside the heavy kernel, which removes a separate scatter launch and the ZScale atomic reduction. The intent is to cut launch count and serialization. In exchange the code gains global scratch state, more complex block-role dispatch, and rider blocks that compete with the main work.

```diff
diff --git a/iso_points_amd/csrc/siren.hip b/iso_points_amd/csrc/siren.hip
--- a/iso_points_amd/csrc/siren.hip
+++ b/iso_points_amd/csrc/siren.hip
@@ -4,58 +4,6 @@
 #include "mlp_common.h"
 
 namespace {
-
-__global__ void k_siren_pack(const float* __restrict__ raw, float* __restrict__ packed,
-                             int H, int L) {
-  const int64_t total = off_hidden(H, L);
-  const int64_t HH = (int64_t)H * H;
-  const int NT = H / 16;
-  for (int64_t o = (int64_t)blockIdx.x * blockDim.x + threadIdx.x; o < total;
-       o += (int64_t)gridDim.x * blockDim.x) {
-    float v = 0.f;
-    if (o < off_wl(H)) {
-      int64_t k = o;
-      int c = (int)(k & 3);
-      int e = (int)((k >> 2) % (H / 4));
-      int g = (int)((k >> 2) / (H / 4));
-      int f = 16 * (e >> 2) + 4 * g + (e & 3);
-      v = (c < 3) ? raw[f * 3 + c] : raw[(int64_t)H * 3 + f];
-    } else if (o < off_bl(H)) {
-      int64_t k = o - off_wl(H);
-      int e = (int)(k % (H / 4));
-      int g = (int)(k / (H / 4));
-      int f = 16 * (e >> 2) + 4 * g + (e & 3);
-      const int64_t raw_wl = (int64_t)H * 4 + (int64_t)L * (HH + H);
-      v = raw[raw_wl + f];
-    } else if (o < off_hidden(H, 0)) {
-      const int64_t raw_wl = (int64_t)H * 4 + (int64_t)L * (HH + H);
-      v = (o == off_bl(H)) ? raw[raw_wl + H] : 0.f;
-    } else {
-      int64_t k = o - off_hidden(H, 0);
-      const int64_t per = H + 2 * HH;
-      int l = (int)(k / per);
-      int64_t w = k % per;
-      const float* Wl = raw + (int64_t)H * 4 + (int64_t)l * (HH + H);
-      const float* bl = Wl + HH;
-      if (w < H) {
-        v = bl[w];
-      } else {
-        w -= H;
-        bool bwd = w >= HH;
-        if (bwd) w -= HH;
-        int i = (int)(w & 3);
-        int lane = (int)((w >> 2) & 63);
-        int t = (int)((w >> 8) % NT);
-        int q = (int)((w >> 8) / NT);
-        int a = 16 * t + (lane & 15);
-        int b = 16 * q + 4 * (lane >> 4) + i;
-        v = bwd ? Wl[(int64_t)b * H + a]
-                : Wl[(int64_t)a * H + b];
-      }
-    }
-    packed[o] = v;
-  }
-}
 
 #define ISO_GEMM_FWD(img, bias) gemm_pass<NT, true>(img, bias, hL, wbuf, acc, lane, g)
 #define ISO_GEMM_BWD(img) gemm_pass<NT, false>(img, nullptr, hL, wbuf, acc, lane, g)
@@ -276,10 +224,7 @@
               "iso_siren_pack_weights: hidden must be 64/128/256 and 0<=n_hidden<=8 (got %d, %d)",
               hidden, n_hidden);
   ISO_REQUIRE(raw && packed, ISO_ERR_INVALID, "iso_siren_pack_weights: null pointer");
-  int64_t total = off_hidden(hidden, n_hidden);
-  hipLaunchKernelGGL(k_siren_pack, dim3(iso_stream_grid(total, 256)), dim3(256), 0,
-                     (hipStream_t)stream, raw, packed, hidden, n_hidden);
-  if (hidden % 32 == 0) siren_x3_pack(raw, packed, hidden, n_hidden, (hipStream_t)stream);
+  siren_x3_pack(raw, packed, hidden, n_hidden, (hipStream_t)stream);
   ISO_CHECK_LAUNCH("iso_siren_pack_weights");
   return ISO_OK;
 }
diff --git a/iso_points_amd/csrc/siren_common.h b/iso_points_amd/csrc/siren_common.h
--- a/iso_points_amd/csrc/siren_common.h
+++ b/iso_points_amd/csrc/siren_common.h
@@ -55,6 +55,57 @@
   return 5 * (int64_t)H + 4 + (int64_t)l * ((int64_t)H + 2 * (int64_t)H * H);
 }
 
+__device__ inline void siren_pack_f32_body(const float* __restrict__ raw, float* __restrict__ packed, int H, int L,
+                                           int block, int nblocks) {
+  const int64_t total = off_hidden(H, L);
+  const int64_t HH = (int64_t)H * H;
+  const int NT = H / 16;
+  for (int64_t o = (int64_t)block * blockDim.x + threadIdx.x; o < total; o += (int64_t)nblocks * blockDim.x) {
+    float v = 0.f;
+    if (o < off_wl(H)) {
+      int64_t k = o;
+      int c = (int)(k & 3);
+      int e = (int)((k >> 2) % (H / 4));
+      int g = (int)((k >> 2) / (H / 4));
+      int f = 16 * (e >> 2) + 4 * g + (e & 3);
+      v = (c < 3) ? raw[f * 3 + c] : raw[(int64_t)H * 3 + f];
+    } else if (o < off_bl(H)) {
+      int64_t k = o - off_wl(H);
+      int e = (int)(k % (H / 4));
+      int g = (int)(k / (H / 4));
+      int f = 16 * (e >> 2) + 4 * g + (e & 3);
+      const int64_t raw_wl = (int64_t)H * 4 + (int64_t)L * (HH + H);
+      v = raw[raw_wl + f];
+    } else if (o < off_hidden(H, 0)) {
+      const int64_t raw_wl = (int64_t)H * 4 + (int64_t)L * (HH + H);
+      v = (o == off_bl(H)) ? raw[raw_wl + H] : 0.f;
+    } else {
+      int64_t k = o - off_hidden(H, 0);
+      const int64_t per = H + 2 * HH;
+      int l = (int)(k / per);
+      int64_t w = k % per;
+      const float* Wl = raw + (int64_t)H * 4 + (int64_t)l * (HH + H);
+      const float* bl = Wl + HH;
+      if (w < H) {
+        v = bl[w];
+      } else {
+        w -= H;
+        bool bwd = w >= HH;
+        if (bwd) w -= HH;
+        int i = (int)(w & 3);
+        int lane = (int)((w >> 2) & 63);
+        int t = (int)((w >> 8) % NT);
+        int q = (int)((w >> 8) / NT);
+        int a = 16 * t + (lane & 15);
+        int b = 16 * q + 4 * (lane >> 4) + i;
+        v = bwd ? Wl[(int64_t)b * H + a]
+                : Wl[(int64_t)a * H + b];
+      }
+    }
+    packed[o] = v;
+  }
+}
+
 __host__ __device__ inline int x3_feat(int s, int kappa) {
   return 32 * (s >> 1) + 16 * (s & 1) + 8 * ((kappa & 7) >> 2) + 4 * (kappa >> 3) + (kappa & 3);
 }
diff --git a/iso_points_amd/csrc/siren_x3.hip b/iso_points_amd/csrc/siren_x3.hip
--- a/iso_points_amd/csrc/siren_x3.hip
+++ b/iso_points_amd/csrc/siren_x3.hip
@@ -15,13 +15,13 @@
 }
 
 
-__global__ void k_siren_pack_x3(const float* __restrict__ raw, float* __restrict__ packed, int H, int L) {
+__device__ __forceinline__ void pack_x3_body(const float* __restrict__ raw, float* __restrict__ packed, int H, int L,
+                                             int block, int nblocks) {
   const int64_t base = x3_base(H, L), total = x16_base(H, L);
   const int64_t HH = (int64_t)H * H;
   const float* b0 = raw + (int64_t)H * 3;
   const float* WL = raw + (int64_t)H * 4 + (int64_t)L * (HH + H);
-  for (int64_t o = base + (int64_t)blockIdx.x * blockDim.x + threadIdx.x; o < total;
-       o += (int64_t)gridDim.x * blockDim.x) {
+  for (int64_t o = base + (int64_t)block * blockDim.x + threadIdx.x; o < total; o += (int64_t)nblocks * blockDim.x) {
     const int64_t rel = o - base;
     auto feat_of = [](int64_t ko) { return x3_feat((int)(ko >> 4), 8 * (int)((ko >> 3) & 1) + (int)(ko & 7)); };
     if (rel < 4 * (int64_t)H) {
@@ -38,50 +38,15 @@
   }
 }
 
-__global__ void k_siren_wscale(const float* __restrict__ raw, float* __restrict__ packed, int H, int L) {
+constexpr int kWCols = 16;
+__device__ unsigned g_wstat[2][8][256 / kWCols];
+
+__global__ __launch_bounds__(256) void k_siren_wscale(const float* __restrict__ raw, float* __restrict__ packed, int H, int L) {
+  __shared__ float s_a[256 * kWCols];
   __shared__ float s_m[256];
-  const int l = blockIdx.x;
   const int64_t HH = (int64_t)H * H;
-  const float* Wl = raw + (int64_t)H * 4 + (int64_t)l * (HH + H);
-  float m = 0.f, cs = 0.f;
-  for (int f = threadIdx.x; f < H; f += 256) {
-    float t = 0.f;
-#pragma unroll 32
-    for (int k = 0; k < H; ++k) {
-      const float a = fabsf(Wl[(int64_t)k * H + f]);
-      m = (a == a && a > m) ? a : m;
-      t += a;
-    }
-    cs = fmaxf(cs, t);
-  }
-  s_m[threadIdx.x] = m;
-  __syncthreads();
-  for (int o = 128; o > 0; o >>= 1) {
-    if ((int)threadIdx.x < o) s_m[threadIdx.x] = fmaxf(s_m[threadIdx.x], s_m[threadIdx.x + o]);
-    __syncthreads();
-  }
-  if (threadIdx.x == 0) {
-    float mx = s_m[0];
-    int e = 0;
-    float sc = 1.0f;
-    if (mx > 0.f && mx < 3.0e38f) {
-      (void)frexpf(mx, &e);
-      int k = 10 - e;
-      k = k > 100 ? 100 : (k < -100 ? -100 : k);
-      sc = ldexpf(1.0f, k);
-    }
-    packed[x16_base(H, L) + l] = sc;
-  }
-  __syncthreads();
-  s_m[threadIdx.x] = cs;
-  __syncthreads();
-  for (int o = 128; o > 0; o >>= 1) {
-    if ((int)threadIdx.x < o) s_m[threadIdx.x] = fmaxf(s_m[threadIdx.x], s_m[threadIdx.x + o]);
-    __syncthreads();
-  }
-  if (threadIdx.x == 0) packed[x16_base(H, L) + 8 + l] = s_m[0];
-  if (l == 0) {
-    __syncthreads();
+  const int groups = H / kWCols;
+  if ((int)blockIdx.x == L * groups) {
     const float* WLh = raw + (int64_t)H * 4 + (int64_t)L * (HH + H);
     float mh = 0.f;
     for (int f = threadIdx.x; f < H; f += 256) mh = fmaxf(mh, fabsf(WLh[f]));
@@ -92,19 +57,61 @@
       __syncthreads();
     }
     if (threadIdx.x == 0) packed[x16_base(H, L) + 16] = s_m[0];
-  }
-}
-
-__global__ void k_siren_pack_f16(const float* __restrict__ raw, float* __restrict__ packed, int H, int L) {
+    return;
+  }
+  const int l = blockIdx.x / groups, cg = blockIdx.x % groups;
+  const float* Wl = raw + (int64_t)H * 4 + (int64_t)l * (HH + H) + cg * kWCols;
+  const int c = threadIdx.x % kWCols, r0 = threadIdx.x / kWCols;
+  float m = 0.f;
+#pragma unroll 16
+  for (int k = r0; k < H; k += 256 / kWCols) {
+    const float a = fabsf(Wl[(int64_t)k * H + c]);
+    s_a[k * kWCols + c] = a;
+    m = (a == a && a > m) ? a : m;
+  }
+  s_m[threadIdx.x] = m;
+  __syncthreads();
+  for (int o = 128; o > 0; o >>= 1) {
+    if ((int)threadIdx.x < o) s_m[threadIdx.x] = fmaxf(s_m[threadIdx.x], s_m[threadIdx.x + o]);
+    __syncthreads();
+  }
+  if (threadIdx.x == 0) g_wstat[0][l][cg] = __float_as_uint(s_m[0]);
+  if (threadIdx.x < 64) {
+    float t = 0.f;
+    if ((int)threadIdx.x < kWCols) {
+#pragma unroll 32
+      for (int k = 0; k < H; ++k) t += s_a[k * kWCols + threadIdx.x];
+    }
+    float cs = fmaxf(0.f, t);
+#pragma unroll
+    for (int o = kWCols / 2; o > 0; o >>= 1) cs = fmaxf(cs, __shfl_xor(cs, o));
+    if (threadIdx.x == 0) g_wstat[1][l][cg] = __float_as_uint(cs);
+  }
+}
+
+__device__ __forceinline__ float x3_scale_of_max(float mx) {
+  int e = 0;
+  float sc = 1.0f;
+  if (mx > 0.f && mx < 3.0e38f) {
+    (void)frexpf(mx, &e);
+    int k = 10 - e;
+    k = k > 100 ? 100 : (k < -100 ? -100 : k);
+    sc = ldexpf(1.0f, k);
+  }
+  return sc;
+}
+
+__device__ __forceinline__ void pack_f16_body(const float* __restrict__ raw, float* __restrict__ packed, int H, int L,
+                                              const float* __restrict__ s_sc , int block, int nblocks) {
   const int64_t HH = (int64_t)H * H;
   const int NTO = H / 32;
   const int64_t total = 2 * (int64_t)L * HH;
-  for (int64_t o = (int64_t)blockIdx.x * blockDim.x + threadIdx.x; o < total; o += (int64_t)gridDim.x * blockDim.x) {
+  for (int64_t o = (int64_t)block * blockDim.x + threadIdx.x; o < total; o += (int64_t)nblocks * blockDim.x) {
     const bool bwd = o >= (int64_t)L * HH;
     const int l = (int)((o / HH) % L);
     const int64_t q = o % HH;
     const float* Wl = raw + (int64_t)H * 4 + (int64_t)l * (HH + H);
-    const float sc = packed[x16_base(H, L) + l];
+    const float sc = s_sc[l];
     const int d = (int)(q & 3), lane = (int)((q >> 2) & 63);
     const int64_t blk = q >> 8;
     const int part = (int)(blk & 1);
@@ -121,6 +128,35 @@
     reinterpret_cast<unsigned*>(packed + x16_off_layer(H, L, 0))[o] =
         part == 0 ? __builtin_bit_cast(unsigned, h) : __builtin_bit_cast(unsigned, lo);
   }
+}
+
+__global__ __launch_bounds__(256) void k_siren_pack_images(const float* __restrict__ raw, float* __restrict__ packed, int H, int L,
+                                                           int g_f16, int g_f32) {
+  const int b = blockIdx.x;
+  if (b >= g_f16 + g_f32) { pack_x3_body(raw, packed, H, L, b - g_f16 - g_f32, gridDim.x - g_f16 - g_f32); return; }
+  if (b >= g_f16) { siren_pack_f32_body(raw, packed, H, L, b - g_f16, g_f32); return; }
+  __shared__ float s_sc[8];
+  constexpr int G = 256 / kWCols;
+  const int l = threadIdx.x / G, g = threadIdx.x % G;
+  if (threadIdx.x < 128) {
+    const bool live = l < L && g < H / kWCols;
+    unsigned mb = live ? g_wstat[0][l][g] : 0u, cb = live ? g_wstat[1][l][g] : 0u;
+#pragma unroll
+    for (int o = G / 2; o > 0; o >>= 1) {
+      mb = max(mb, (unsigned)__shfl_xor((int)mb, o));
+      cb = max(cb, (unsigned)__shfl_xor((int)cb, o));
+    }
+    if (g == 0 && l < L) {
+      const float sc = x3_scale_of_max(__uint_as_float(mb));
+      s_sc[l] = sc;
+      if (b == 0) {
+        packed[x16_base(H, L) + l] = sc;
+        packed[x16_base(H, L) + 8 + l] = __uint_as_float(cb);
+      }
+    }
+  }
+  __syncthreads();
+  pack_f16_body(raw, packed, H, L, s_sc, b, g_f16);
 }
 
 template <int H, int NW, int NB>
@@ -669,12 +705,11 @@
 }
 
 void siren_x3_pack(const float* raw, float* packed, int H, int L, hipStream_t s) {
-  const int64_t words = x16_base(H, L) - x3_base(H, L);
-  hipLaunchKernelGGL(k_siren_pack_x3, dim3(iso_stream_grid(words, 256)), dim3(256), 0, s, raw, packed, H, L);
-  if (L > 0) {
-    hipLaunchKernelGGL(k_siren_wscale, dim3(L), dim3(256), 0, s, raw, packed, H, L);
-    hipLaunchKernelGGL(k_siren_pack_f16, dim3(iso_stream_grid(2 * (int64_t)L * H * H, 256)), dim3(256), 0, s, raw, packed, H, L);
-  }
+  if (L > 0) hipLaunchKernelGGL(k_siren_wscale, dim3(L * (H / kWCols) + 1), dim3(256), 0, s, raw, packed, H, L);
+  const int g_f16 = L > 0 ? iso_stream_grid(2 * (int64_t)L * H * H, 256) : 0;
+  const int g_f32 = iso_stream_grid(off_hidden(H, L), 256);
+  const int g_x3 = iso_stream_grid(x16_base(H, L) - x3_base(H, L), 256);
+  hipLaunchKernelGGL(k_siren_pack_images, dim3(g_f16 + g_f32 + g_x3), dim3(256), 0, s, raw, packed, H, L, g_f16, g_f32);
 }
 
 int siren_x3_tail_blocks() { return 256 * kMinB256; }
diff --git a/iso_points_amd/csrc/splat.hip b/iso_points_amd/csrc/splat.hip
--- a/iso_points_amd/csrc/splat.hip
+++ b/iso_points_amd/csrc/splat.hip
@@ -6,15 +6,21 @@
 #pragma clang fp contract(off)
 
 struct ZScale;
+constexpr int kZParts = 256;
 struct ZRider {
+  int blocks;
   const float* gz; int64_t n;
-  ZScale* zs; int blocks;
-  const long long* acc; float* grad; int terms_log2;
+  unsigned* parts; int nparts;
+  long long* acc;
+  const int64_t* first; const int64_t* num; int n_clouds;
+  const int32_t* idx; int K; int64_t npix;
+  float* grad; int terms_log2;
 };
-__device__ void z_absmax_body(const float* __restrict__ gz, int64_t n, ZScale* __restrict__ zs, int block, int nblocks);
-__device__ void z_finish_body(const long long* __restrict__ acc, const ZScale* __restrict__ zs, const int64_t* __restrict__ first,
-                              const int64_t* __restrict__ num, int n_clouds, float* __restrict__ grad, int terms_log2,
+__device__ void z_absmax_body(const float* __restrict__ gz, int64_t n, ZScale* __restrict__ zs, unsigned* __restrict__ parts,
                               int block, int nblocks);
+__device__ void z_clear_rider(const ZRider& r, int block, int nblocks);
+__device__ void z_scatter_rider(const ZRider& r, int block, int nblocks);
+__device__ void z_finish_rider(const ZRider& r, int block, int nblocks);
 
 namespace {
 
@@ -1544,15 +1550,17 @@
                                                    unsigned long long* __restrict__ pixmask ,
                                                    uint8_t* __restrict__ rowbytes ,
                                                    uint8_t* __restrict__ blk2 ,
-                                                   int32_t* __restrict__ clear_a, int n_clear_a,
-                                                   int32_t* __restrict__ clear_b, int n_clear_b) {
-  if (blockIdx.x == 0) {
-    if ((int)threadIdx.x < n_clear_a) clear_a[threadIdx.x] = 0;
-    if (clear_b && (int)threadIdx.x < n_clear_b) clear_b[threadIdx.x] = 0;
-  }
+                                                   int32_t* __restrict__ clear_a, int n_clear_a, ZRider rider) {
+  if ((int)blockIdx.x < rider.blocks) {
+    if ((int)blockIdx.x < rider.nparts) z_absmax_body(rider.gz, rider.n, nullptr, rider.parts, blockIdx.x, rider.nparts);
+    else z_clear_rider(rider, blockIdx.x - rider.nparts, rider.blocks - rider.nparts);
+    return;
+  }
+  const int own_block = blockIdx.x - rider.blocks, own_blocks = gridDim.x - rider.blocks;
+  if (own_block == 0 && (int)threadIdx.x < n_clear_a) clear_a[threadIdx.x] = 0;
   const int lane = threadIdx.x & 63;
   const int64_t total = (int64_t)N * G.NB2x * G.NB2y;
-  for (int64_t sb = (int64_t)blockIdx.x * 4 + (threadIdx.x >> 6); sb < total; sb += (int64_t)gridDim.x * 4) {
+  for (int64_t sb = (int64_t)own_block * 4 + (threadIdx.x >> 6); sb < total; sb += (int64_t)own_blocks * 4) {
     const int sx = sb % G.NB2x, sy = (sb / G.NB2x) % G.NB2y, n = sb / ((int64_t)G.NB2x * G.NB2y);
     const int bx = sx * 8 + (lane & 7), by = sy * 8 + (lane >> 3);
     unsigned long long m = 0ull;
@@ -1613,19 +1621,19 @@
     const int64_t* __restrict__ first, const int64_t* __restrict__ num,
     const uint8_t* __restrict__ blk2, BlkGeo G, Frame F, int rect_mode, float radii_s,
     int32_t* __restrict__ heavy, int32_t* __restrict__ heavy_count, float* __restrict__ grad,
-    long long* __restrict__ zacc ,
     ZRider rider, int own_blocks) {
-  if ((int)blockIdx.x >= own_blocks) {
-    if (blockIdx.y == 0) z_absmax_body(rider.gz, rider.n, rider.zs, blockIdx.x - own_blocks, rider.blocks);
+  if ((int)blockIdx.x < rider.blocks) {
+    z_scatter_rider(rider, blockIdx.y * rider.blocks + blockIdx.x, rider.blocks * gridDim.y);
     return;
   }
+  const int own_block = blockIdx.x - rider.blocks;
   const int n = blockIdx.y;
   const int64_t len = num[n], base = first[n];
   const float r = rect_mode ? 0.f : rs[n];
   const int lane = threadIdx.x & 63, wv = threadIdx.x >> 6;
   __shared__ int s_wcnt[4][4], s_base;
   const int64_t span = (int64_t)own_blocks * 1024;
-  for (int64_t i0 = (int64_t)blockIdx.x * 1024; i0 < len; i0 += span) {
+  for (int64_t i0 = (int64_t)own_block * 1024; i0 < len; i0 += span) {
     bool is_heavy[4];
     int64_t pp[4];
     unsigned long long bal[4];
@@ -1641,7 +1649,6 @@
         const float rx = radii[p * 2], ry = radii[p * 2 + 1];
         const bool vis = (!visible || visible[p]);
         grad[p * 3] = 0.f; grad[p * 3 + 1] = 0.f; grad[p * 3 + 2] = 0.f;
-        if (zacc) zacc[p] = 0;
         const float sx = rect_mode ? rx * radii_s : r, sy = rect_mode ? ry * radii_s : r;
         if (vis && !(pz < 0.f || fabsf(py) > F.ey || fabsf(px) > F.ex) && sx > 0.f && sy > 0.f) {
           int x0, x1, y0, y1;
@@ -1684,7 +1691,7 @@
     int rect_mode, float radii_s, const int32_t* __restrict__ heavy,
     const int32_t* __restrict__ heavy_count, float* __restrict__ grad, ZRider rider, int own_blocks) {
   if ((int)blockIdx.x >= own_blocks) {
-    z_finish_body(rider.acc, rider.zs, first, num, n_clouds, rider.grad, rider.terms_log2, blockIdx.x - own_blocks, rider.blocks);
+    z_finish_rider(rider, blockIdx.x - own_blocks, rider.blocks);
     return;
   }
   const int count = *heavy_count;
@@ -2534,7 +2541,8 @@
 
 struct ZScale { unsigned max_bits; int exp2; };
 
-__device__ void z_absmax_body(const float* __restrict__ gz, int64_t n, ZScale* __restrict__ zs, int block, int nblocks) {
+__device__ void z_absmax_body(const float* __restrict__ gz, int64_t n, ZScale* __restrict__ zs, unsigned* __restrict__ parts,
+                              int block, int nblocks) {
   __shared__ unsigned sm[4];
   unsigned m = 0u;
   const int64_t n4 = n / 4;
@@ -2562,13 +2570,24 @@
   __syncthreads();
   if (threadIdx.x == 0) {
     m = max(max(sm[0], sm[1]), max(sm[2], sm[3]));
-    if (m) atomicMax(&zs->max_bits, m);
+    if (parts) parts[block] = m;
+    else if (m) atomicMax(&zs->max_bits, m);
   }
 }
 
 __global__ __launch_bounds__(256) void k_z_absmax(const float* __restrict__ gz0, int64_t n, ZScale* __restrict__ zs,
                                                   int64_t view_stride = 0) {
-  z_absmax_body(gz0 + (int64_t)blockIdx.y * view_stride, n, zs, blockIdx.x, gridDim.x);
+  z_absmax_body(gz0 + (int64_t)blockIdx.y * view_stride, n, zs, nullptr, blockIdx.x, gridDim.x);
+}
+
+__device__ unsigned z_parts_max(const unsigned* __restrict__ parts, int nparts) {
+  __shared__ unsigned sm[4];
+  unsigned m = (int)threadIdx.x < nparts ? parts[threadIdx.x] : 0u;
+#pragma unroll
+  for (int o = 32; o > 0; o >>= 1) m = max(m, (unsigned)__shfl_xor((int)m, o));
+  if ((threadIdx.x & 63) == 0) sm[threadIdx.x >> 6] = m;
+  __syncthreads();
+  return max(max(sm[0], sm[1]), max(sm[2], sm[3]));
 }
 
 __device__ __forceinline__ int z_exponent(unsigned max_bits, int terms_log2) {
@@ -2592,17 +2611,13 @@
   atomicAdd(reinterpret_cast<unsigned long long*>(&acc[p]), (unsigned long long)q);
 }
 
-__global__ void k_z_scatter(const int32_t* __restrict__ idx0, const float* __restrict__ gz0, int K, int64_t npix,
-                            const ZScale* __restrict__ zs, long long* __restrict__ acc, int64_t view_stride = 0,
-                            int terms_log2 = -1) {
-  const int32_t* __restrict__ idx = idx0 + (int64_t)blockIdx.y * view_stride * K;
-  const float* __restrict__ gz = gz0 + (int64_t)blockIdx.y * view_stride * K;
-  const int e = terms_log2 >= 0 ? z_exponent(zs->max_bits, terms_log2) : zs->exp2;
+__device__ __forceinline__ void z_scatter_body(const int32_t* __restrict__ idx, const float* __restrict__ gz, int K, int64_t npix,
+                                               int e, long long* __restrict__ acc, int block, int nblocks) {
   if ((K & 3) == 0 && (((uintptr_t)idx | (uintptr_t)gz) & 15) == 0) {
     const int4* __restrict__ idx4 = reinterpret_cast<const int4*>(idx);
     const float4* __restrict__ gz4 = reinterpret_cast<const float4*>(gz);
     const int64_t nq = npix * (K / 4);
-    for (int64_t i = (int64_t)blockIdx.x * blockDim.x + threadIdx.x; i < nq; i += (int64_t)gridDim.x * blockDim.x) {
+    for (int64_t i = (int64_t)block * blockDim.x + threadIdx.x; i < nq; i += (int64_t)nblocks * blockDim.x) {
       const float4 g = gz4[i];
       if (g.x == 0.0f && g.y == 0.0f && g.z == 0.0f && g.w == 0.0f) continue;
       const int4 p = idx4[i];
@@ -2614,13 +2629,33 @@
     }
     return;
   }
-  for (int64_t i = (int64_t)blockIdx.x * blockDim.x + threadIdx.x; i < npix; i += (int64_t)gridDim.x * blockDim.x) {
+  for (int64_t i = (int64_t)block * blockDim.x + threadIdx.x; i < npix; i += (int64_t)nblocks * blockDim.x) {
     for (int k = 0; k < K; ++k) {
       const int p = idx[i * K + k];
       if (p < 0) break;
       z_scatter_one(p, gz[i * K + k], e, acc);
     }
   }
+}
+
+__global__ void k_z_scatter(const int32_t* __restrict__ idx0, const float* __restrict__ gz0, int K, int64_t npix,
+                            const ZScale* __restrict__ zs, long long* __restrict__ acc, int64_t view_stride = 0,
+                            int terms_log2 = -1) {
+  const int e = terms_log2 >= 0 ? z_exponent(zs->max_bits, terms_log2) : zs->exp2;
+  z_scatter_body(idx0 + (int64_t)blockIdx.y * view_stride * K, gz0 + (int64_t)blockIdx.y * view_stride * K, K, npix, e, acc,
+                 blockIdx.x, gridDim.x);
+}
+
+__device__ void z_clear_rider(const ZRider& r, int block, int nblocks) {
+  for (int c = 0; c < r.n_clouds; ++c) {
+    const int64_t len = r.num[c], base = r.first[c];
+    for (int64_t i = (int64_t)block * blockDim.x + threadIdx.x; i < len; i += (int64_t)nblocks * blockDim.x) r.acc[base + i] = 0;
+  }
+}
+
+__device__ void z_scatter_rider(const ZRider& r, int block, int nblocks) {
+  const int e = z_exponent(z_parts_max(r.parts, r.nparts), r.terms_log2);
+  z_scatter_body(r.idx, r.gz, r.K, r.npix, e, r.acc, block, nblocks);
 }
 
 __global__ void k_z_finish(const long long* __restrict__ acc, const ZScale* __restrict__ zs, int64_t n,
@@ -2634,10 +2669,9 @@
   }
 }
 
-__device__ void z_finish_body(const long long* __restrict__ acc, const ZScale* __restrict__ zs, const int64_t* __restrict__ first,
-                              const int64_t* __restrict__ num, int n_clouds, float* __restrict__ grad, int terms_log2,
+__device__ void z_finish_body(const long long* __restrict__ acc, int e, const int64_t* __restrict__ first,
+                              const int64_t* __restrict__ num, int n_clouds, float* __restrict__ grad,
                               int block, int nblocks) {
-  const int e = z_exponent(zs->max_bits, terms_log2);
   for (int c = 0; c < n_clouds; ++c) {
     const int64_t len = num[c], base = first[c];
     for (int64_t i = (int64_t)block * blockDim.x + threadIdx.x; i < len; i += (int64_t)nblocks * blockDim.x) {
@@ -2653,7 +2687,12 @@
 __global__ void k_z_finish_clouds(const long long* __restrict__ acc, const ZScale* __restrict__ zs,
                                   const int64_t* __restrict__ first, const int64_t* __restrict__ num,
                                   float* __restrict__ grad, int terms_log2) {
-  z_finish_body(acc, zs, first + blockIdx.y, num + blockIdx.y, 1, grad, terms_log2, blockIdx.x, gridDim.x);
+  z_finish_body(acc, z_exponent(zs->max_bits, terms_log2), first + blockIdx.y, num + blockIdx.y, 1, grad, blockIdx.x, gridDim.x);
+}
+
+__device__ void z_finish_rider(const ZRider& r, int block, int nblocks) {
+  const int e = z_exponent(z_parts_max(r.parts, r.nparts), r.terms_log2);
+  z_finish_body(r.acc, e, r.first, r.num, r.n_clouds, r.grad, block, nblocks);
 }
 
 static int64_t bwd_maps_bytes(int n_clouds, int image_size, int image_width) {
@@ -2663,7 +2702,8 @@
 extern "C" int64_t iso_splat_backward_workspace_bytes(int n_clouds, int image_size, int image_width,
                                                       int64_t total_points) {
   if (total_points < 0) total_points = 0;
-  return bwd_maps_bytes(n_clouds, image_size, image_width) + 64 + (4 * total_points + 15) / 16 * 16 + 16 + 8 * total_points;
+  return bwd_maps_bytes(n_clouds, image_size, image_width) + 64 + (4 * total_points + 15) / 16 * 16 + 16 + 8 * total_points +
+         4 * kZParts;
 }
 
 extern "C" int iso_splat_backward(const float* points, const float* radii, const uint8_t* visible,
@@ -2691,29 +2731,31 @@
   int32_t* heavy_count = (int32_t*)((uint8_t*)workspace + bwd_maps_bytes(n_clouds, image_size, image_width));
   int32_t* heavy = heavy_count + 16;
   const bool with_z = grad_zbuf && total_points > 0;
-  ZScale* zs = reinterpret_cast<ZScale*>((char*)(heavy_count) + 64 + (4 * total_points + 15) / 16 * 16);
-  long long* zacc = reinterpret_cast<long long*>((char*)zs + 16);
-  {
-    int gmaps = iso_div_up((int64_t)n_clouds * G.NB2x * G.NB2y, 4);
-    hipLaunchKernelGGL(k_grad_maps, dim3(gmaps < 1 ? 1 : gmaps), dim3(256), 0, s, grad_occ, F, G, n_clouds, pixmask, rowbytes, blk2,
-                       heavy_count, 16, with_z ? reinterpret_cast<int32_t*>(zs) : nullptr, 4);
-  }
-  int gx = iso_div_up(max_pts, 1024); if (gx > 8192) gx = 8192;
+  long long* zacc = reinterpret_cast<long long*>((char*)(heavy_count) + 64 + (4 * total_points + 15) / 16 * 16 + 16);
+  unsigned* zparts = reinterpret_cast<unsigned*>(zacc + total_points);
   const int64_t npix = (int64_t)n_clouds * F.H * F.W;
   int terms_log2 = 0;
   while ((1ll << terms_log2) < (int64_t)F.H * F.W) ++terms_log2;
-  ZRider r1{nullptr, 0, zs, 0, nullptr, nullptr, 0}, r2 = r1;
+  ZRider r0{0, grad_zbuf, npix * points_per_pixel, zparts, 0, zacc, first_idx, num_pts, n_clouds, idx, points_per_pixel, npix,
+            grad_points, terms_log2};
+  ZRider r1 = r0, r2 = r0;
   if (with_z) {
-    int gm = iso_div_up(npix * points_per_pixel, 256 * 16); if (gm > 1024) gm = 1024; if (gm < 1) gm = 1;
-    r1 = ZRider{grad_zbuf, npix * points_per_pixel, zs, gm, nullptr, nullptr, 0};
-    r2 = ZRider{nullptr, 0, zs, iso_stream_grid(total_points, 256), zacc, grad_points, terms_log2};
-  }
+    int gm = iso_div_up(npix * points_per_pixel, 256 * 64); if (gm > kZParts) gm = kZParts; if (gm < 1) gm = 1;
+    int gc = iso_div_up(max_pts, 1024); if (gc > 1024) gc = 1024; if (gc < 1) gc = 1;
+    r0.nparts = r1.nparts = r2.nparts = gm;
+    r0.blocks = gm + gc;
+    r1.blocks = iso_div_up(iso_stream_grid(npix, 256), n_clouds);
+    r2.blocks = iso_stream_grid(total_points, 256);
+  }
+  {
+    int gmaps = iso_div_up((int64_t)n_clouds * G.NB2x * G.NB2y, 4);
+    hipLaunchKernelGGL(k_grad_maps, dim3((gmaps < 1 ? 1 : gmaps) + r0.blocks), dim3(256), 0, s, grad_occ, F, G, n_clouds, pixmask,
+                       rowbytes, blk2, heavy_count, 16, r0);
+  }
+  int gx = iso_div_up(max_pts, 1024); if (gx > 8192) gx = 8192;
   hipLaunchKernelGGL(k_splat_backward, dim3(gx + r1.blocks, n_clouds), dim3(256), 0, s, points, radii, visible,
                      search_radius, first_idx, num_pts, blk2, G, F, rect_mode, radii_s, heavy,
-                     heavy_count, grad_points, with_z ? zacc : nullptr, r1, gx);
-  if (with_z)
-    hipLaunchKernelGGL(k_z_scatter, dim3(iso_stream_grid(npix, 256)), dim3(256), 0, s, idx, grad_zbuf,
-                       points_per_pixel, npix, zs, zacc, (int64_t)0, terms_log2);
+                     heavy_count, grad_points, r1, gx);
   constexpr int heavy_grid = 4096;
   hipLaunchKernelGGL(k_splat_backward_heavy, dim3(heavy_grid + r2.blocks), dim3(256), 0, s, points, radii, search_radius,
                      first_idx, num_pts, n_clouds, grad_occ, pixmask, rowbytes, G, F, rect_mode, radii_s,
```

Result: no change. 74.80 (median of 6 runs) (+0.2%).
